# getreu/stringsext

Hardware: AMD Instinct MI355X
Metric: GiB/s scanned (higher is better)
Workload: dtype u8

## Files before the change

stringsext_amd/csrc/sx_api.cpp:

```cpp
#include "sx_ctx.hpp"
#include "sx_print_core.hpp"
#include "sx_select_core.hpp"
#include "sx_selset_build.hpp"
#include "sx_selset_core.hpp"
#include "sx_selre_build.hpp"
#include "sx_selre_core.hpp"
#include "sx_extract_build.hpp"
#include "sx_extract_core.hpp"
#include "sx_seltally_build.hpp"
#include "sx_seltally_core.hpp"
#include "sx_label_build.hpp"
#include "sx_label_core.hpp"

using namespace sx;

struct sx_select_set {
    int device = 0;
    uint8_t* mem = nullptr;
    SelsetDevice dev{};
    sx_select_set_info info{};
};

struct sx_select_regex {
    int device = 0;
    uint8_t* mem = nullptr;
    SelreDevice dev{};
    sx_select_regex_info info{};
};

struct sx_extract_regex {
    int device = 0;
    uint8_t* mem = nullptr;
    ExtractDevice dev{};
    sx_extract_regex_info info{};
};

struct sx_tally_set {
    int device = 0;
    uint8_t* mem = nullptr;
    SeltallyDevice dev{};
    const uint32_t* d_unique_of_pattern = nullptr;
    std::vector<uint32_t> unique_of_pattern;
    sx_tally_set_info info{};
};

struct sx_label_set {
    int device = 0;
    uint8_t* mem = nullptr;
    LabelDevice dev{};
    sx_label_set_info info{};
};

struct sx_labels {
    struct Seg {
        const uint64_t* d = nullptr;
        const void* recs = nullptr;
        uint64_t n = 0;
        std::shared_ptr<std::atomic<uint64_t>> epoch_ref;
        uint64_t epoch = 0;
    };
    int device = 0;
    uint8_t* mem = nullptr;
    std::vector<Seg> segs;
};

namespace sx {
PinnedPool::Block PinnedPool::take(size_t bytes) {
    {
        std::lock_guard<std::mutex> g(mu);
        size_t best = free_blocks.size();
        for (size_t i = 0; i < free_blocks.size(); i++)
            if (free_blocks[i].cap >= bytes && (best == free_blocks.size() || free_blocks[i].cap < free_blocks[best].cap)) best = i;
        if (best < free_blocks.size() && free_blocks[best].cap <= 4 * bytes + (4u << 20)) {
            Block b = free_blocks[best];
            free_blocks.erase(free_blocks.begin() + (long)best);
            return b;
        }
    }
    Block b;
    const size_t cap = bytes + bytes / 8 + (1u << 20);
    if (hipHostMalloc(&b.p, cap, hipHostMallocNonCoherent) != hipSuccess) { b.p = nullptr; return b; }
    b.cap = cap;
    return b;
}
void PinnedPool::give(Block b) {
    if (!b.p) return;
    std::lock_guard<std::mutex> g(mu);
    free_blocks.push_back(b);
    if (free_blocks.size() > 40) {
        size_t m = 0;
        for (size_t i = 1; i < free_blocks.size(); i++) if (free_blocks[i].cap < free_blocks[m].cap) m = i;
        (void)hipHostFree(free_blocks[m].p);
        free_blocks.erase(free_blocks.begin() + (long)m);
    }
}
PinnedPool::~PinnedPool() { for (Block& b : free_blocks) (void)hipHostFree(b.p); }
}

namespace {
std::string g_create_error;
}

namespace sx {

double g_tl_t0 = 0;
int g_tl_on = 0;

double now_ms() {
    using namespace std::chrono;
    return duration<double, std::milli>(steady_clock::now().time_since_epoch()).count();
}


int ensure_pinned(sx_ctx* ctx, uint64_t bytes) {
    if (ctx->h_pin_cap >= bytes) return SX_OK;
    if (ctx->h_pin) HIP_TRY(ctx, hipHostFree(ctx->h_pin));
    ctx->h_pin = nullptr; ctx->h_pin_cap = 0;
    bytes += bytes / 4 + (1u << 20);
    unsigned flags = hipHostMallocNonCoherent;
    if (ctx->sw.pin_flags >= 0) flags = (unsigned)ctx->sw.pin_flags;
    HIP_TRY(ctx, hipHostMalloc((void**)&ctx->h_pin, bytes, flags));
    ctx->h_pin_cap = bytes;
    return SX_OK;
}
int read_back_async(sx_ctx* ctx, hipStream_t s, void* pinned_dst, const void* dev_src, size_t bytes) {
    if (ctx->sw.small_copy && bytes <= (1u << 20) && ((((uintptr_t)pinned_dst | (uintptr_t)dev_src | bytes) & 3) == 0))
        HIP_TRY(ctx, launch_small_copy(pinned_dst, dev_src, bytes, s));
    else HIP_TRY(ctx, hipMemcpyAsync(pinned_dst, dev_src, bytes, hipMemcpyDeviceToHost, s));
    return SX_OK;
}
int read_back_sync(sx_ctx* ctx, MissionDev& d, hipStream_t s, void* host_dst, const void* dev_src, size_t bytes) {
    if (!ctx->sw.small_copy || bytes > kSmallReadBytes || ((((uintptr_t)dev_src | bytes) & 3) != 0)) {
        HIP_TRY(ctx, hipMemcpyAsync(host_dst, dev_src, bytes, hipMemcpyDeviceToHost, s));
        HIP_TRY(ctx, hipStreamSynchronize(s));
        return SX_OK;
    }
    if (!d.h_small) HIP_TRY(ctx, hipHostMalloc((void**)&d.h_small, kSmallReadBytes, hipHostMallocDefault));
    HIP_TRY(ctx, launch_small_copy(d.h_small, dev_src, bytes, s));
    HIP_TRY(ctx, hipStreamSynchronize(s));
    memcpy(host_dst, d.h_small, bytes);
    return SX_OK;
}
int ensure_pinned2(sx_ctx* ctx, uint64_t bytes) {
    if (ctx->h_pin2_cap >= bytes) return SX_OK;
    if (ctx->h_pin2) HIP_TRY(ctx, hipHostFree(ctx->h_pin2));
    ctx->h_pin2 = nullptr; ctx->h_pin2_cap = 0;
    bytes += bytes / 4 + (1u << 20);
    HIP_TRY(ctx, hipHostMalloc((void**)&ctx->h_pin2, bytes, hipHostMallocNonCoherent));
    ctx->h_pin2_cap = bytes;
    return SX_OK;
}
int ensure_scratch(sx_ctx* ctx, uint64_t bytes) {
    std::lock_guard<std::recursive_mutex> g(ctx->grow_mu);
    if (ctx->d_scratch_cap >= bytes) return SX_OK;
    if (ctx->merge_async) { const int rc = merge_drain(ctx); if (rc != SX_OK) return rc; }
    if (ctx->d_scratch) HIP_TRY(ctx, hipFree(ctx->d_scratch));
    ctx->d_scratch = nullptr; ctx->d_scratch_cap = 0;
    bytes += bytes / 4 + (1u << 20);
    HIP_TRY(ctx, hipMalloc((void**)&ctx->d_scratch, bytes));
    ctx->d_scratch_cap = bytes;
    return SX_OK;
}

int ensure_capacity(sx_ctx* ctx, ScanSlot& s, uint32_t cap) {
    if (s.capacity >= cap) return SX_OK;
    if (s.d_recs) HIP_TRY(ctx, hipFree(s.d_recs));
    s.d_recs = nullptr; s.capacity = 0;
    HIP_TRY(ctx, hipMalloc((void**)&s.d_recs, (size_t)cap * sizeof(DevRun)));
    s.capacity = cap;
    return SX_OK;
}

int ensure_cache(sx_ctx* ctx, uint64_t bytes) {
    if (ctx->d_cache_cap >= bytes) return SX_OK;
    if (ctx->d_cache) HIP_TRY(ctx, hipFree(ctx->d_cache));
    ctx->d_cache = nullptr; ctx->d_cache_cap = 0;
    HIP_TRY(ctx, hipMalloc((void**)&ctx->d_cache, bytes));
    ctx->d_cache_cap = bytes;
    return SX_OK;
}
int ensure_rp(sx_ctx* ctx, MissionDev& d, int slot, uint64_t bytes) {
    if (d.d_rp_cap[slot] >= bytes) return SX_OK;
    std::lock_guard<std::recursive_mutex> g(ctx->grow_mu);
    if (ctx->merge_async) { const int rc = merge_drain(ctx); if (rc != SX_OK) return rc; }
    if (d.d_rp[slot]) HIP_TRY(ctx, hipFree(d.d_rp[slot]));
    d.d_rp[slot] = nullptr; d.d_rp_cap[slot] = 0;
    bytes += bytes / 4 + 4096;
    HIP_TRY(ctx, hipMalloc(&d.d_rp[slot], bytes));
    d.d_rp_cap[slot] = bytes;
    return SX_OK;
}


unsigned usable_cpus() {
    unsigned n = std::thread::hardware_concurrency();
    if (n < 1) n = 1;
    if (FILE* f = fopen("/sys/fs/cgroup/cpu.max", "r")) {
        char a[64] = { 0 };
        unsigned long long period = 0;
        if (fscanf(f, "%63s %llu", a, &period) == 2 && strcmp(a, "max") != 0 && period > 0) {
            const unsigned long long quota = strtoull(a, nullptr, 10);
            const unsigned q = (unsigned)((quota + period - 1) / period);
            if (q >= 1 && q < n) n = q;
        }
        fclose(f);
    }
    return n;
}

unsigned replay_threads(const sx_ctx* ctx) {
    unsigned n = ctx->opt.replay_threads ? ctx->opt.replay_threads
                                         : std::min(std::thread::hardware_concurrency(), 4 * usable_cpus());
    if (ctx->sw.replay_threads) n = (unsigned)ctx->sw.replay_threads;
    if (n < 1) n = 1;
    return n > 256 ? 256 : n;
}


void begin_call(sx_ctx* ctx) {
    memset(&ctx->stats, 0, sizeof ctx->stats);
    ctx->err.clear();
    ctx->sharded_call = false;
    ctx->dev_epoch->fetch_add(1);
}

static int fetch_to_host(sx_result* r, MissionFindings& s) {
    if (!s.dev_only) return SX_OK;
    if (!s.keep_on_device || !s.dev_epoch_ref || s.dev_epoch_ref->load() != s.dev_epoch) return SX_E_STATE;
    const size_t bytes = s.ext_nf * s.rec_size() + s.ext_na;
    PinnedPool::Block blk = r->r.pool ? r->r.pool->take(bytes + 64) : PinnedPool::Block{};
    if (!blk.p) return SX_E_NOMEM;
    if (hipMemcpy(blk.p, s.dev_copy, bytes, hipMemcpyDeviceToHost) != hipSuccess) { r->r.pool->give(blk); return SX_E_HIP; }
    s.ext = blk; s.dev_only = false;
    return SX_OK;
}
static int fetch_all_to_host(const sx_result* r) {
    sx_result* w = const_cast<sx_result*>(r);
    for (auto& s : w->r.segs) { const int rc = fetch_to_host(w, s); if (rc != SX_OK) return rc; }
    return SX_OK;
}


}

extern "C" {

int sx_abi_version(void) { return SX_ABI_VERSION; }

const uint16_t* sx_decoder_table(uint32_t encoding, uint64_t* n_words) {
    size_t n = 0;
    const uint16_t* t = decoder_table((int)encoding, &n);
    if (n_words) *n_words = n;
    return t;
}

const uint32_t* sx_wave_pair_codes(const sx_mission* mission, uint32_t* out8192) {
    if (!mission || !out8192) return nullptr;
    Mission m;
    std::string err;
    if (Mission::from_c(*mission, false, Switches{}.wave_same, &m, &err) != SX_OK || m.wave_pairs.size() != 8192) return nullptr;
    memcpy(out8192, m.wave_pairs.data(), 8192 * 4);
    return out8192;
}

const uint32_t* sx_wave_pair_codes2(const sx_mission* mission, uint32_t* out4096) {
    if (!mission || !out4096) return nullptr;
    Mission m;
    std::string err;
    if (Mission::from_c(*mission, false, Switches{}.wave_same, &m, &err) != SX_OK || m.wave_pairs2.size() != 4096) return nullptr;
    memcpy(out4096, m.wave_pairs2.data(), 4096 * 4);
    return out4096;
}

int sx_wave_swar(const sx_mission* mission, uint32_t* out26) {
    if (!mission || !out26) return SX_E_INVALID;
    Mission m;
    std::string err;
    const int rc = Mission::from_c(*mission, false, Switches{}.wave_same, &m, &err);
    if (rc != SX_OK) return rc;
    static_assert(sizeof(WvSwar) == 26 * 4, "sx_wave_swar hands the struct out as 26 words");
    memcpy(out26, &m.wave_swar, sizeof(WvSwar));
    return m.wave_ok && m.wave_swar.cls ? 1 : 0;
}

int sx_scan_classifier(const sx_mission* mission, int generic, uint32_t* out20) {
    if (!mission || !out20) return SX_E_INVALID;
    Mission m;
    std::string err;
    const int rc = Mission::from_c(*mission, generic != 0, Switches{}.wave_same, &m, &err);
    if (rc != SX_OK) return rc;
    const ScanParams& p = m.proto;
    const uint32_t head[7] = { p.a_lo, p.a_hi, p.u_lo, p.u_hi, p.l3_lo, p.l3_hi, p.n_ranges };
    memcpy(out20, head, sizeof head);
    memcpy(out20 + 7, p.rng_c1, 6 * sizeof(uint32_t));
    memcpy(out20 + 13, p.rng_c2, 6 * sizeof(uint32_t));
    out20[19] = 0;
    return (int)m.kind;
}

int sx_wave_classes(const sx_mission* mission, uint8_t* classes) {
    if (!mission || !classes) return SX_E_INVALID;
    Mission m;
    std::string err;
    const int rc = Mission::from_c(*mission, false, Switches{}.wave_same, &m, &err);
    if (rc != SX_OK) return rc;
    if (!m.wave_ok || m.wave_lead_check || (m.wave_lut.size() != 256 && !(m.wave_family == 2 && m.wave_lut.size() == 512))) return 0;
    memcpy(classes, m.wave_lut.data(), m.wave_lut.size());
    return 1 + (int)m.wave_family;
}

int sx_create(sx_ctx** out, const sx_mission* missions, int n_missions, int hip_device, const sx_options* opt) {
    if (!out || !missions || n_missions <= 0 || n_missions > 26) { g_create_error = "bad arguments"; return SX_E_INVALID; }
    sx_ctx* ctx = new sx_ctx();
    ctx->sw = Switches::from_env();
    if (opt) ctx->opt = *opt;
    if (ctx->sw.result_on_device) ctx->opt.flags |= SX_OPT_RESULT_ON_DEVICE;
    ctx->missions.resize((size_t)n_missions);
    ctx->states.resize((size_t)n_missions);
    for (int k = 0; k < n_missions; k++) {
        std::string err;
        int rc = Mission::from_c(missions[k], (ctx->opt.flags & SX_OPT_GENERIC_KERNELS) != 0, ctx->sw.wave_same, &ctx->missions[(size_t)k], &err);
        if (rc != SX_OK) { g_create_error = "mission " + std::to_string(k) + ": " + err; delete ctx; return rc; }
        ctx->states[(size_t)k].reset(ctx->missions[(size_t)k]);
    }
    if (hip_device == SX_HOST_ONLY) { ctx->host_only = true; *out = ctx; return SX_OK; }

    int n_dev = 0;
    hipError_t e = hipGetDeviceCount(&n_dev);
    if (e != hipSuccess || n_dev <= 0 || hip_device < 0 || hip_device >= n_dev) {
        g_create_error = std::string("no usable HIP device (hipGetDeviceCount: ")
                         + (e == hipSuccess ? "ok" : hipGetErrorString(e)) + ", devices=" + std::to_string(n_dev)
                         + ", requested=" + std::to_string(hip_device) + "); the scan only runs on the GPU";
        delete ctx;
        return SX_E_NO_DEVICE;
    }
    ctx->device = hip_device;
    auto fail = [&](const char* what, hipError_t err) {
        g_create_error = std::string(what) + ": " + hipGetErrorString(err);
        sx_destroy(ctx);
        return SX_E_HIP;
    };
    if ((e = hipSetDevice(hip_device)) != hipSuccess) return fail("hipSetDevice", e);
    ctx->dev.resize((size_t)n_missions);
    const uint32_t cap = ctx->opt.record_capacity ? ctx->opt.record_capacity : (1u << 20);
    {
        int cus = 0;
        if (hipDeviceGetAttribute(&cus, hipDeviceAttributeMultiprocessorCount, hip_device) == hipSuccess && cus > 0) ctx->n_cus = (unsigned)cus;
        if (ctx->sw.scan_blocks_per_cu >= 0) ctx->scan_blocks_per_cu = (unsigned)ctx->sw.scan_blocks_per_cu;
        if (ctx->sw.region_cap >= 0) ctx->region_cap = (uint32_t)ctx->sw.region_cap;
        if (ctx->sw.scan_cus) ctx->n_cus = (unsigned)ctx->sw.scan_cus;
    }
    int prio_lo = 0, prio_hi = 0;
    (void)hipDeviceGetStreamPriorityRange(&prio_lo, &prio_hi);
    if (ctx->sw.prio_n >= 0) {
        if (ctx->sw.prio_n >= 1) prio_lo = ctx->sw.prio_scan;
        if (ctx->sw.prio_n >= 2) prio_hi = ctx->sw.prio_post;
        fprintf(stderr, "[sx] stream priorities: scan %d, post %d\n", prio_lo, prio_hi);
    }
    const bool per_mission = (ctx->opt.flags & SX_OPT_MISSION_STREAMS) || ctx->sw.mission_streams;
    if ((e = hipStreamCreateWithPriority(&ctx->post_stream, hipStreamNonBlocking, prio_hi)) != hipSuccess) return fail("hipStreamCreate", e);
    if (!per_mission && (e = hipStreamCreateWithPriority(&ctx->scan_stream, hipStreamNonBlocking, prio_lo)) != hipSuccess)
        return fail("hipStreamCreate", e);
    for (auto& d : ctx->dev) {
        d.stream_b = ctx->post_stream;
        if (per_mission) {
            if ((e = hipStreamCreateWithPriority(&d.stream, hipStreamNonBlocking, prio_lo)) != hipSuccess) return fail("hipStreamCreate", e);
        } else d.stream = ctx->scan_stream;
        for (ScanSlot& s : d.slot) {
            if ((e = hipEventCreate(&s.ev0)) != hipSuccess) return fail("hipEventCreate", e);
            if ((e = hipEventCreate(&s.ev1)) != hipSuccess) return fail("hipEventCreate", e);
            if ((e = hipEventCreateWithFlags(&s.ev_free, hipEventDisableTiming)) != hipSuccess) return fail("hipEventCreate", e);
            if ((e = hipMalloc((void**)&s.d_counters, kCounterWords * sizeof(uint32_t))) != hipSuccess) return fail("hipMalloc", e);
            if ((e = hipMalloc((void**)&s.d_recs, (size_t)cap * sizeof(DevRun))) != hipSuccess) return fail("hipMalloc", e);
            s.capacity = cap;
        }
    }
    for (size_t k = 0; k < ctx->dev.size(); k++) {
        size_t n_words = 0;
        if (const uint16_t* t = decoder_table(ctx->missions[k].c.encoding, &n_words)) {
            if ((e = hipMalloc((void**)&ctx->dev[k].d_table, n_words * 2)) != hipSuccess) return fail("hipMalloc", e);
            if ((e = hipMemcpy(ctx->dev[k].d_table, t, n_words * 2, hipMemcpyHostToDevice)) != hipSuccess) return fail("hipMemcpy", e);
        }
        const std::vector<uint32_t>& pl = ctx->missions[k].pair_lut;
        if (!pl.empty()) {
            if ((e = hipMalloc((void**)&ctx->dev[k].d_pair_lut, pl.size() * 4)) != hipSuccess) return fail("hipMalloc", e);
            if ((e = hipMemcpy(ctx->dev[k].d_pair_lut, pl.data(), pl.size() * 4, hipMemcpyHostToDevice)) != hipSuccess) return fail("hipMemcpy", e);
        }
    }
    *out = ctx;
    return SX_OK;
}

void sx_destroy(sx_ctx* ctx) {
    if (!ctx) return;
    ctx->dev_epoch->fetch_add(1);
    for (auto& e : ctx->select_epoch) e->fetch_add(1);
    if (!ctx->host_only && ctx->device >= 0) {
        (void)hipSetDevice(ctx->device);
        for (auto& d : ctx->dev) {
            if (d.stream) (void)hipStreamSynchronize(d.stream);
            if (d.stream_b) (void)hipStreamSynchronize(d.stream_b);
            for (ScanSlot& s : d.slot) {
                if (s.d_recs) (void)hipFree(s.d_recs);
                if (s.d_cnt) (void)hipFree(s.d_cnt);
                if (s.d_grid) (void)hipFree(s.d_grid);
                if (s.d_packed) (void)hipFree(s.d_packed);
                if (s.d_counters) (void)hipFree(s.d_counters);
                if (s.ev0) (void)hipEventDestroy(s.ev0);
                if (s.ev1) (void)hipEventDestroy(s.ev1);
                if (s.ev_free) (void)hipEventDestroy(s.ev_free);
            }
            if (d.d_table) (void)hipFree(d.d_table);
            if (d.d_pair_lut) (void)hipFree(d.d_pair_lut);
            if (d.d_wave_lut) (void)hipFree(d.d_wave_lut);
            if (d.d_wave_pairs) (void)hipFree(d.d_wave_pairs);
            if (d.d_wave_pairs2) (void)hipFree(d.d_wave_pairs2);
            for (void* q : d.d_rp) if (q) (void)hipFree(q);
            if (d.h_runs) (void)hipHostFree(d.h_runs);
            if (d.ev_runs) (void)hipEventDestroy(d.ev_runs);
            if (d.stream_w) (void)hipStreamDestroy(d.stream_w);
            if (d.h_tot) (void)hipHostFree(d.h_tot);
            if (d.h_small) (void)hipHostFree(d.h_small);
            for (hipEvent_t e : d.wave_ev) if (e) (void)hipEventDestroy(e);
            if (d.stream && d.stream != ctx->scan_stream) (void)hipStreamDestroy(d.stream);
        }
        for (int i = 0; i < 2; i++) {
            if (ctx->ing_pin[i]) (void)hipHostFree(ctx->ing_pin[i]);
            if (ctx->ing_dev[i]) (void)hipFree(ctx->ing_dev[i]);
        }
        if (ctx->copy_stream) (void)hipStreamDestroy(ctx->copy_stream);
        if (ctx->d2h_stream) (void)hipStreamDestroy(ctx->d2h_stream);
        if (ctx->scan_stream) (void)hipStreamDestroy(ctx->scan_stream);
        if (ctx->d_cache) (void)hipFree(ctx->d_cache);
        if (ctx->post_stream) (void)hipStreamDestroy(ctx->post_stream);
        if (ctx->merge_copy_stream) (void)hipStreamDestroy(ctx->merge_copy_stream);
        if (ctx->d_merge) (void)hipFree(ctx->d_merge);
        if (ctx->d_result) (void)hipFree(ctx->d_result);
        if (ctx->d_result_up) (void)hipFree(ctx->d_result_up);
        if (ctx->d_text) (void)hipFree(ctx->d_text);
        if (ctx->d_print_scratch) (void)hipFree(ctx->d_print_scratch);
        if (ctx->d_print_missions) (void)hipFree(ctx->d_print_missions);
        for (uint8_t* p : ctx->d_select) if (p) (void)hipFree(p);
        if (ctx->d_select_scratch) (void)hipFree(ctx->d_select_scratch);
        if (ctx->d_select_scratch2) (void)hipFree(ctx->d_select_scratch2);
        for (hipEvent_t e : ctx->merge_ev) if (e) (void)hipEventDestroy(e);
        for (hipEvent_t e : ctx->slab_ev) if (e) (void)hipEventDestroy(e);
        if (ctx->ev_interleaved) (void)hipEventDestroy(ctx->ev_interleaved);
        if (ctx->d_input) (void)hipFree(ctx->d_input);
        if (ctx->d_scratch) (void)hipFree(ctx->d_scratch);
        if (ctx->h_pin) (void)hipHostFree(ctx->h_pin);
        if (ctx->h_pin2) (void)hipHostFree(ctx->h_pin2);
    }
    delete ctx;
}

const char* sx_last_error(const sx_ctx* ctx) { return ctx ? ctx->err.c_str() : g_create_error.c_str(); }

int sx_reset(sx_ctx* ctx) {
    if (!ctx) return SX_E_INVALID;
    for (size_t k = 0; k < ctx->missions.size(); k++) ctx->states[k].reset(ctx->missions[k]);
    ctx->shard_runs_valid = false;
    return SX_OK;
}


int sx_device_runs(sx_ctx* ctx, int mission_index, const void* device_bytes, uint64_t len, int stream_parity,
                   uint64_t min_chars, sx_run** runs, uint64_t* n_runs) {
    if (!ctx || !runs || !n_runs || mission_index < 0 || (size_t)mission_index >= ctx->missions.size()) return SX_E_INVALID;
    begin_call(ctx);
    ctx->sw.scan_warm = Switches::from_env().scan_warm;
    if (ctx->host_only) { ctx->err = "host-only context: no device scan"; return SX_E_STATE; }
    if ((uintptr_t)device_bytes & 15) { ctx->err = "device_bytes must be 16-byte aligned"; return SX_E_INVALID; }
    if (ctx->missions[(size_t)mission_index].host_sequential()) { ctx->err = "an ISO-2022-JP mission has no stage A (one sequential pass on the host)"; return SX_E_INVALID; }
    HIP_TRY(ctx, hipSetDevice(ctx->device));
    std::vector<RunList> out;
    ctx->shard_runs_valid = false;
    int rc = device_runs(ctx, { mission_index }, (const uint8_t*)device_bytes, len, { (uint32_t)(stream_parity & 1) },
                         { min_chars }, &out);
    if (rc != SX_OK) return rc;
    HIP_TRY(ctx, out[0].wait());
    *n_runs = out[0].size();
    *runs = (sx_run*)malloc(sizeof(sx_run) * (out[0].size() ? out[0].size() : 1));
    if (!*runs) return SX_E_NOMEM;
    memcpy(*runs, out[0].data(), sizeof(sx_run) * out[0].size());
    return SX_OK;
}

int sx_device_runs_multi(sx_ctx* ctx, const int* mission_indices, int n, const void* device_bytes, uint64_t len, int stream_parity,
                         const uint64_t* min_chars, sx_run** runs, uint64_t* n_runs) {
    if (!ctx || !mission_indices || n <= 0 || !min_chars || !runs || !n_runs) return SX_E_INVALID;
    begin_call(ctx);
    if (ctx->host_only) { ctx->err = "host-only context: no device scan"; return SX_E_STATE; }
    if ((uintptr_t)device_bytes & 15) { ctx->err = "device_bytes must be 16-byte aligned"; return SX_E_INVALID; }
    std::vector<int> which; std::vector<uint32_t> par; std::vector<uint64_t> mc;
    for (int i = 0; i < n; i++) {
        const int k = mission_indices[i];
        if (k < 0 || (size_t)k >= ctx->missions.size() || std::find(which.begin(), which.end(), k) != which.end()) { ctx->err = "bad mission index"; return SX_E_INVALID; }
        if (ctx->missions[(size_t)k].host_sequential()) { ctx->err = "an ISO-2022-JP mission has no stage A (one sequential pass on the host)"; return SX_E_INVALID; }
        which.push_back(k); par.push_back((uint32_t)(stream_parity & 1)); mc.push_back(min_chars[i]);
        runs[i] = nullptr; n_runs[i] = 0;
    }
    HIP_TRY(ctx, hipSetDevice(ctx->device));
    std::vector<RunList> out;
    ctx->shard_runs_valid = false;
    int rc = device_runs(ctx, which, (const uint8_t*)device_bytes, len, par, mc, &out);
    if (rc != SX_OK) return rc;
    for (int i = 0; i < n; i++) {
        if (!out[(size_t)i].own.empty()) out[(size_t)i].use_own();
        HIP_TRY(ctx, out[(size_t)i].wait());
        n_runs[i] = out[(size_t)i].size();
        runs[i] = (sx_run*)malloc(sizeof(sx_run) * (n_runs[i] ? n_runs[i] : 1));
        if (!runs[i]) { for (int j = 0; j < i; j++) { free(runs[j]); runs[j] = nullptr; } return SX_E_NOMEM; }
        memcpy(runs[i], out[(size_t)i].data(), sizeof(sx_run) * n_runs[i]);
    }
    return SX_OK;
}

int sx_replay_runs(sx_ctx* ctx, const uint8_t* bytes, uint64_t len, int input_file_id, int is_last_input_buffer,
                   const sx_run* const* runs, const uint64_t* n_runs, sx_result** out) {
    if (!ctx || !out || (!bytes && len) || !runs || !n_runs) return SX_E_INVALID;
    begin_call(ctx);
    std::vector<RunList> r(ctx->missions.size());
    for (size_t k = 0; k < r.size(); k++) r[k].assign(runs[k], runs[k] + n_runs[k]);
    HostBytes view(bytes ? bytes : (const uint8_t*)"");
    ResultHolder res;
    std::vector<uint32_t> entry;
    int rc = set_entry_params(ctx, true, bytes, nullptr, len, 0, &entry);
    if (rc != SX_OK) return rc;
    rc = replay_all(ctx, view, whole_chunk_job(ctx, len, input_file_id, is_last_input_buffer != 0), r, &res.r->r, nullptr);
    if (rc == SX_OK) *out = res.release();
    return rc;
}


int sx_scan_shard_device(sx_ctx* ctx, const void* device_bytes, uint64_t buf_off, uint64_t buf_len, uint64_t own_lo,
                         uint64_t own_hi, const uint64_t* start_at, uint64_t file_stream_off, int input_file_id,
                         int reuse_runs, sx_result** out, uint64_t* end_pos) {
    if (!ctx || (!device_bytes && buf_len)) return SX_E_INVALID;
    begin_call(ctx);
    if (ctx->host_only) { ctx->err = "host-only context: no device scan"; return SX_E_STATE; }
    if ((uintptr_t)device_bytes & 15) { ctx->err = "device_bytes must be 16-byte aligned"; return SX_E_INVALID; }
    HIP_TRY(ctx, hipSetDevice(ctx->device));
    return shard_common(ctx, nullptr, (const uint8_t*)device_bytes, nullptr, nullptr, buf_off, buf_len, own_lo, own_hi, start_at,
                        file_stream_off, input_file_id, reuse_runs, out, end_pos);
}

int sx_scan_shard(sx_ctx* ctx, const uint8_t* bytes, uint64_t buf_off, uint64_t buf_len, uint64_t own_lo, uint64_t own_hi,
                  const uint64_t* start_at, uint64_t file_stream_off, int input_file_id, int reuse_runs, sx_result** out,
                  uint64_t* end_pos) {
    if (!ctx || (!bytes && buf_len)) return SX_E_INVALID;
    begin_call(ctx);
    if (ctx->host_only) { ctx->err = "host-only context: no device scan"; return SX_E_STATE; }
    HIP_TRY(ctx, hipSetDevice(ctx->device));
    if (!(reuse_runs && ctx->shard_runs_valid && ctx->shard_runs_off == buf_off && ctx->shard_runs_len == buf_len && ctx->shard_runs_ptr == (const void*)ctx->d_input)) {
        if (buf_len > ctx->d_input_cap) {
            if (ctx->d_input) HIP_TRY(ctx, hipFree(ctx->d_input));
            ctx->d_input = nullptr; ctx->d_input_cap = 0;
            HIP_TRY(ctx, hipMalloc((void**)&ctx->d_input, buf_len));
            ctx->d_input_cap = buf_len;
        }
        if (buf_len) HIP_TRY(ctx, hipMemcpy(ctx->d_input, bytes, buf_len, hipMemcpyHostToDevice));
    }
    return shard_common(ctx, bytes ? bytes : (const uint8_t*)"", ctx->d_input, nullptr, nullptr, buf_off, buf_len, own_lo, own_hi,
                        start_at, file_stream_off, input_file_id, reuse_runs, out, end_pos);
}

int sx_replay_shard_runs(sx_ctx* ctx, const uint8_t* bytes, uint64_t buf_off, uint64_t buf_len, uint64_t own_lo,
                         uint64_t own_hi, const uint64_t* start_at, uint64_t file_stream_off, int input_file_id,
                         const sx_run* const* runs, const uint64_t* n_runs, sx_result** out, uint64_t* end_pos) {
    if (!ctx || (!bytes && buf_len) || !runs || !n_runs) return SX_E_INVALID;
    begin_call(ctx);
    return shard_common(ctx, bytes ? bytes : (const uint8_t*)"", nullptr, runs, n_runs, buf_off, buf_len, own_lo, own_hi, start_at,
                        file_stream_off, input_file_id, 0, out, end_pos);
}

uint64_t sx_result_count(const sx_result* r) { return r ? r->r.count() : 0; }
uint64_t sx_result_segments(const sx_result* r) { return r ? r->r.segs.size() : 0; }
int sx_result_segment(const sx_result* r, uint64_t i, const sx_finding** findings, uint64_t* n_findings,
                      const uint8_t** arena, uint64_t* arena_len) {
    if (!r || i >= r->r.segs.size()) return SX_E_INVALID;
    { const int rc = fetch_to_host(const_cast<sx_result*>(r), const_cast<sx_result*>(r)->r.segs[(size_t)i]); if (rc != SX_OK) return rc; }
    const MissionFindings& s = r->r.segs[(size_t)i];
    if (findings) *findings = s.data();
    if (n_findings) *n_findings = s.count();
    if (arena) *arena = (const uint8_t*)s.strings();
    if (arena_len) *arena_len = s.strings_len();
    return SX_OK;
}
int sx_result_segment_packed(const sx_result* r, uint64_t i, const void** findings, uint64_t* n_findings, const uint8_t** arena,
                             uint64_t* arena_len, int* packed, sx_segment_info* info) {
    if (!r || i >= r->r.segs.size()) return SX_E_INVALID;
    { const int rc = fetch_to_host(const_cast<sx_result*>(r), const_cast<sx_result*>(r)->r.segs[(size_t)i]); if (rc != SX_OK) return rc; }
    const MissionFindings& s = r->r.segs[(size_t)i];
    if (findings) *findings = s.packed ? (const void*)s.data16() : (const void*)s.data();
    if (n_findings) *n_findings = s.count();
    if (arena) *arena = (const uint8_t*)s.strings();
    if (arena_len) *arena_len = s.strings_len();
    if (packed) *packed = s.packed ? 1 : 0;
    if (info) {
        memset(info, 0, sizeof *info);
        info->packed = s.packed ? 1 : 0;
        info->input_file_id = -1;
        if (s.packed && s.info) {
            info->input_file_id = s.info->file_id; info->slice_base = s.info->slice_base;
            memcpy(info->position0, s.info->pos0, sizeof info->position0);
        }
    }
    return SX_OK;
}
int sx_result_segment_device(const sx_result* r, uint64_t i, const void** d_records, uint64_t* n_findings, const uint8_t** d_arena,
                             uint64_t* arena_len, int* packed, sx_segment_info* info) {
    if (!r || i >= r->r.segs.size()) return SX_E_INVALID;
    const MissionFindings& s = r->r.segs[(size_t)i];
    if (d_records) *d_records = nullptr;
    if (d_arena) *d_arena = nullptr;
    if (n_findings) *n_findings = s.count();
    if (arena_len) *arena_len = s.strings_len();
    if (packed) *packed = s.packed ? 1 : 0;
    if (info) {
        memset(info, 0, sizeof *info);
        info->packed = s.packed ? 1 : 0;
        info->input_file_id = -1;
        if (s.packed && s.info) {
            info->input_file_id = s.info->file_id; info->slice_base = s.info->slice_base;
            memcpy(info->position0, s.info->pos0, sizeof info->position0);
        }
    }
    if (!s.dev_only) return SX_OK;
    if (!s.keep_on_device || !s.dev_epoch_ref || s.dev_epoch_ref->load() != s.dev_epoch) return SX_E_STATE;
    if (d_records) *d_records = s.dev_copy;
    if (d_arena) *d_arena = (const uint8_t*)s.dev_copy + s.ext_nf * s.rec_size();
    return SX_OK;
}
const sx_finding* sx_result_findings(const sx_result* r) {
    if (!r || fetch_all_to_host(r) != SX_OK || !const_cast<sx_result*>(r)->r.flatten(nullptr) || r->r.segs.empty()) return nullptr;
    return r->r.segs[0].data();
}
const uint8_t* sx_result_arena(const sx_result* r, uint64_t* len) {
    if (len) *len = 0;
    if (!r || fetch_all_to_host(r) != SX_OK || !const_cast<sx_result*>(r)->r.flatten(nullptr) || r->r.segs.empty()) return nullptr;
    if (len) *len = r->r.segs[0].strings_len();
    return (const uint8_t*)r->r.segs[0].strings();
}
void sx_result_free(sx_result* r) { delete r; }

int sx_print_findings(const sx_ctx* ctx, const sx_result* r, int n_inputs, int radix, int no_metadata, uint8_t** out,
                      uint64_t* out_len) {
    if (!ctx || !r || !out || !out_len) return SX_E_INVALID;
    if (radix != 0 && radix != 'x' && radix != 'd' && radix != 'o') return SX_E_INVALID;
    { const int rc = fetch_all_to_host(r); if (rc != SX_OK) return rc; }
    std::string s;
    print_findings(ctx->missions, r->r, n_inputs, radix, no_metadata != 0, &s);
    *out = (uint8_t*)malloc(s.size() ? s.size() : 1);
    if (!*out) return SX_E_NOMEM;
    memcpy(*out, s.data(), s.size());
    *out_len = s.size();
    return SX_OK;
}

static int result_on_device(sx_ctx* ctx, const sx_result* r, const char* host_call) {
    const std::string in_host = std::string("the result is in host memory: ") + host_call;
    if (r->r.segs.empty()) { ctx->set_err(in_host); return SX_E_STATE; }
    for (const MissionFindings& s : r->r.segs) {
        if (!s.dev_only || !s.keep_on_device || s.ext_nf == 0) { ctx->set_err(in_host); return SX_E_STATE; }
        const bool ours = s.dev_epoch_ref && (s.dev_epoch_ref == ctx->dev_epoch || s.dev_epoch_ref == ctx->select_epoch[0] || s.dev_epoch_ref == ctx->select_epoch[1]);
        if (!ours || s.dev_epoch_ref->load() != s.dev_epoch) {
            ctx->set_err("a later scan or selection has reused the result's device memory");
            return SX_E_STATE;
        }
    }
    return SX_OK;
}

int sx_print_findings_device(sx_ctx* ctx, const sx_result* r, int n_inputs, int radix, int no_metadata, const uint8_t** d_text,
                             uint64_t* text_len) {
    if (d_text) *d_text = nullptr;
    if (text_len) *text_len = 0;
    if (!ctx || !r || !d_text || !text_len) return SX_E_INVALID;
    if (radix != 0 && radix != 'x' && radix != 'd' && radix != 'o') { ctx->set_err("radix must be 0, 'x', 'd' or 'o'"); return SX_E_INVALID; }
    if (ctx->host_only) { ctx->set_err("host-only context: no device print"); return SX_E_STATE; }
    { const int rc = result_on_device(ctx, r, "sx_print_findings"); if (rc != SX_OK) return rc; }
    HIP_TRY(ctx, hipSetDevice(ctx->device));
    hipStream_t st = ctx->post_stream;
    if (!ctx->d_print_missions) {
        std::vector<PrintMission> tab(256);
        memset(tab.data(), 0, tab.size() * sizeof(PrintMission));
        for (size_t k = ctx->missions.size(); k-- > 0;) {
            const Mission& m = ctx->missions[k];
            const char* name = m.c.print_encoding_as_ascii ? "ascii" : m.encoding_name();
            const std::string label = name ? name : "";
            PrintMission& t = tab[m.c.mission_id];
            if (label.size() > sizeof t.label) { ctx->set_err("encoding label longer than 14 bytes"); return SX_E_STATE; }
            t.present = 1; t.len = (uint8_t)label.size();
            memcpy(t.label, label.data(), label.size());
        }
        uint8_t* p = nullptr;
        if (hipMalloc((void**)&p, tab.size() * sizeof(PrintMission)) != hipSuccess) { (void)hipGetLastError(); ctx->set_err("device print: no memory for the Mission table"); return SX_E_NOMEM; }
        const hipError_t e = hipMemcpy(p, tab.data(), tab.size() * sizeof(PrintMission), hipMemcpyHostToDevice);
        if (e != hipSuccess) { (void)hipFree(p); ctx->set_err(std::string("hipMemcpy: ") + hipGetErrorString(e)); return SX_E_HIP; }
        ctx->d_print_missions = p;
    }
    const size_t ns = r->r.segs.size();
    uint64_t scratch = 0;
    for (const MissionFindings& s : r->r.segs) scratch += print_scratch_bytes(s.ext_nf);
    if (scratch > ctx->d_print_scratch_cap) {
        if (ctx->d_print_scratch) (void)hipFree(ctx->d_print_scratch);
        ctx->d_print_scratch = nullptr; ctx->d_print_scratch_cap = 0;
        if (hipMalloc((void**)&ctx->d_print_scratch, scratch) != hipSuccess) { (void)hipGetLastError(); ctx->d_print_scratch = nullptr; ctx->set_err("device print: no memory for the offsets"); return SX_E_NOMEM; }
        ctx->d_print_scratch_cap = scratch;
    }
    std::vector<PrintParams> P(ns);
    std::vector<const uint64_t*> d_total(ns);
    uint64_t at = 0;
    for (size_t i = 0; i < ns; i++) {
        const MissionFindings& s = r->r.segs[i];
        PrintParams& p = P[i];
        memset(&p, 0, sizeof p);
        p.recs = s.dev_copy; p.arena = (const uint8_t*)s.dev_copy + s.ext_nf * s.rec_size(); p.n = s.ext_nf; p.packed = s.packed ? 1u : 0u;
        p.file_id = s.packed && s.info ? s.info->file_id : -1;
        p.several_inputs = n_inputs > 1; p.radix = (uint32_t)radix; p.no_metadata = no_metadata != 0; p.several_missions = ctx->missions.size() > 1;
        p.missions = (const PrintMission*)ctx->d_print_missions;
        const size_t bytes = print_scratch_bytes(s.ext_nf);
        HIP_TRY(ctx, print_measure(p, ctx->d_print_scratch + at, bytes, st, &p.wbase, &d_total[i]));
        at += bytes;
    }
    HIP_TRY(ctx, hipStreamSynchronize(st));
    uint64_t total = 0;
    for (size_t i = 0; i < ns; i++) {
        uint64_t t = 0;
        HIP_TRY(ctx, hipMemcpy(&t, d_total[i], sizeof t, hipMemcpyDeviceToHost));
        P[i].base = total;
        total += t;
    }
    if (total > ctx->d_text_cap) {
        if (ctx->d_text) (void)hipFree(ctx->d_text);
        ctx->d_text = nullptr; ctx->d_text_cap = 0;
        if (hipMalloc((void**)&ctx->d_text, total) != hipSuccess) {
            (void)hipGetLastError();
            ctx->d_text = nullptr;
            ctx->set_err("device print: no memory for " + std::to_string(total) + " bytes of text");
            return SX_E_NOMEM;
        }
        ctx->d_text_cap = total;
    }
    for (size_t i = 0; i < ns; i++) {
        P[i].text = ctx->d_text;
        HIP_TRY(ctx, print_write(P[i], st));
    }
    HIP_TRY(ctx, hipStreamSynchronize(st));
    *d_text = ctx->d_text;
    *text_len = total;
    return SX_OK;
}

static int grow_device(sx_ctx* ctx, uint8_t** p, uint64_t* cap, uint64_t bytes, const char* what) {
    if (bytes <= *cap) return SX_OK;
    if (*p) (void)hipFree(*p);
    *p = nullptr; *cap = 0;
    if (hipMalloc((void**)p, bytes) != hipSuccess) {
        (void)hipGetLastError();
        *p = nullptr;
        ctx->set_err(std::string("device select: no memory for ") + std::to_string(bytes) + " bytes of " + what);
        return SX_E_NOMEM;
    }
    *cap = bytes;
    return SX_OK;
}

static int select_on_device(sx_ctx* ctx, const sx_result* r, const sx_pattern* patterns, int n_patterns, const SelsetDevice* set, const SelreDevice* re, const ExtractDevice* ex, uint32_t flags, sx_result** out,
                            const sx_labels* labels = nullptr, const uint64_t* masks = nullptr) {
    if (ctx->host_only) { ctx->set_err("host-only context: no device selection"); return SX_E_STATE; }
    { const int rc = result_on_device(ctx, r, "filter on the host"); if (rc != SX_OK) return rc; }
    if (labels) {
        bool same = labels->segs.size() == r->r.segs.size();
        for (size_t i = 0; same && i < labels->segs.size(); i++) {
            const sx_labels::Seg& l = labels->segs[i];
            const MissionFindings& s = r->r.segs[i];
            same = l.recs == s.dev_copy && l.n == s.ext_nf && l.epoch_ref == s.dev_epoch_ref && l.epoch == s.dev_epoch;
        }
        if (!same) { ctx->set_err("the labels were not made from this result"); return SX_E_INVALID; }
    }
    const int slot = (int)(ctx->select_calls & 1u);
    for (const MissionFindings& s : r->r.segs)
        if (s.dev_epoch_ref == ctx->select_epoch[slot]) { ctx->set_err("this selection reuses the source's device memory: it was selected two calls ago"); return SX_E_STATE; }
    HIP_TRY(ctx, hipSetDevice(ctx->device));
    hipStream_t st = ctx->post_stream;
    const size_t ns = r->r.segs.size();
    uint64_t scratch = 0;
    for (const MissionFindings& s : r->r.segs) scratch += ex ? extract_scratch_bytes(s.ext_nf) : select_scratch_bytes(s.ext_nf);
    { const int rc = grow_device(ctx, &ctx->d_select_scratch, &ctx->d_select_scratch_cap, scratch, "wavefront tables"); if (rc != SX_OK) return rc; }
    std::vector<SelectParams> P(ex ? 0 : ns);
    std::vector<ExtractParams> X(ex ? ns : 0);
    std::vector<const uint32_t*> d_count(ns);
    std::vector<const uint64_t*> d_count64(ns), d_bytes(ns);
    uint64_t at = 0;
    for (size_t i = 0; i < ns; i++) {
        const MissionFindings& s = r->r.segs[i];
        if (ex) {
            ExtractParams& x = X[i];
            memset(&x, 0, sizeof x);
            x.recs = s.dev_copy; x.arena = (const uint8_t*)s.dev_copy + s.ext_nf * s.rec_size(); x.n = s.ext_nf; x.packed = s.packed ? 1u : 0u;
            x.ex = *ex;
            const size_t bytes = extract_scratch_bytes(s.ext_nf);
            HIP_TRY(ctx, extract_measure(&x, ctx->d_select_scratch + at, bytes, st, &d_count64[i], &d_bytes[i]));
            at += bytes;
            continue;
        }
        SelectParams& p = P[i];
        memset(&p, 0, sizeof p);
        p.recs = s.dev_copy; p.arena = (const uint8_t*)s.dev_copy + s.ext_nf * s.rec_size(); p.n = s.ext_nf; p.packed = s.packed ? 1u : 0u;
        if (set || re) p.pat.invert = (flags & SX_SELECT_INVERT) ? 1u : 0u;
        else select_fill_patterns(&p.pat, patterns, n_patterns, flags);
        const size_t bytes = select_scratch_bytes(s.ext_nf);
        LabelPick pick{ nullptr, 0, 0, 0 };
        if (labels) pick = LabelPick{ labels->segs[i].d, masks[0], masks[1], masks[2] };
        HIP_TRY(ctx, select_measure(&p, set, re, ctx->d_select_scratch + at, bytes, st, &d_count[i], &d_bytes[i], labels ? &pick : nullptr));
        at += bytes;
    }
    HIP_TRY(ctx, hipStreamSynchronize(st));
    std::vector<uint64_t> n_sel(ns), b_sel(ns), base(ns);
    uint64_t block = 0, scratch2 = 0;
    for (size_t i = 0; i < ns; i++) {
        uint64_t c = 0;
        if (ex) HIP_TRY(ctx, hipMemcpy(&c, d_count64[i], sizeof c, hipMemcpyDeviceToHost));
        else { uint32_t c32 = 0; HIP_TRY(ctx, hipMemcpy(&c32, d_count[i], sizeof c32, hipMemcpyDeviceToHost)); c = c32; }
        HIP_TRY(ctx, hipMemcpy(&b_sel[i], d_bytes[i], sizeof(uint64_t), hipMemcpyDeviceToHost));
        if (c >= 0xFFFFFFFFull) {
            ctx->set_err("segment " + std::to_string(i) + " has " + std::to_string(c) + " matches: more than the 32-bit counters of a segment hold");
            return SX_E_INVALID;
        }
        n_sel[i] = c;
        if (!c) continue;
        base[i] = block;
        block += (c * r->r.segs[i].rec_size() + b_sel[i] + 255) / 256 * 256;
        scratch2 = std::max<uint64_t>(scratch2, ex ? extract_place_scratch_bytes(c) : select_place_scratch_bytes(c));
    }
    ctx->select_epoch[slot]->fetch_add(1);
    ctx->select_calls++;
    ResultHolder res;
    res.r->r.pool = ctx->pool;
    if (block) {
        { const int rc = grow_device(ctx, &ctx->d_select[slot], &ctx->d_select_cap[slot], block, "selected findings"); if (rc != SX_OK) return rc; }
        { const int rc = grow_device(ctx, &ctx->d_select_scratch2, &ctx->d_select_scratch2_cap, scratch2, "string offsets"); if (rc != SX_OK) return rc; }
        for (size_t i = 0; i < ns; i++) {
            if (!n_sel[i]) continue;
            const MissionFindings& s = r->r.segs[i];
            uint8_t* recs = ctx->d_select[slot] + base[i];
            if (ex) HIP_TRY(ctx, extract_place(X[i], recs, n_sel[i], recs + n_sel[i] * s.rec_size(), ctx->d_select_scratch2, extract_place_scratch_bytes(n_sel[i]), st));
            else HIP_TRY(ctx, select_place(P[i], recs, n_sel[i], recs + n_sel[i] * s.rec_size(), ctx->d_select_scratch2, select_place_scratch_bytes(n_sel[i]), st));
            MissionFindings o;
            o.ext_nf = n_sel[i]; o.ext_na = b_sel[i]; o.dev_copy = recs; o.dev_only = true; o.keep_on_device = true;
            o.dev_epoch_ref = ctx->select_epoch[slot]; o.dev_epoch = ctx->select_epoch[slot]->load();
            o.packed = s.packed; o.info = s.info;
            res.r->r.segs.push_back(std::move(o));
        }
        HIP_TRY(ctx, hipStreamSynchronize(st));
    }
    *out = res.release();
    return SX_OK;
}

int sx_result_select_device(sx_ctx* ctx, const sx_result* r, const sx_pattern* patterns, int n_patterns, uint32_t flags, sx_result** out) {
    if (out) *out = nullptr;
    if (!ctx || !r || !patterns || !out) return SX_E_INVALID;
    if (n_patterns < 1 || n_patterns > SX_SELECT_MAX_PATTERNS) { ctx->set_err("n_patterns must be 1..16"); return SX_E_INVALID; }
    if (flags & ~(uint32_t)(SX_SELECT_ASCII_NOCASE | SX_SELECT_INVERT)) { ctx->set_err("unknown selection flags"); return SX_E_INVALID; }
    for (int p = 0; p < n_patterns; p++)
        if (!patterns[p].bytes || patterns[p].len < 1 || patterns[p].len > SX_SELECT_MAX_PATTERN_BYTES) { ctx->set_err("a pattern must have 1..64 bytes"); return SX_E_INVALID; }
    return select_on_device(ctx, r, patterns, n_patterns, nullptr, nullptr, nullptr, flags, out);
}

int sx_select_set_create(sx_ctx* ctx, const sx_pattern* patterns, uint32_t n_patterns, uint32_t flags, sx_select_set** out) {
    if (out) *out = nullptr;
    if (!ctx || !patterns || !out) return SX_E_INVALID;
    SelsetTable T;
    std::string err;
    { const int rc = selset_build(patterns, n_patterns, flags, &T, &err); if (rc != SX_OK) { ctx->set_err("pattern set: " + err); return rc; } }
    if (ctx->host_only) { ctx->set_err("host-only context: no device for the pattern set"); return SX_E_STATE; }
    HIP_TRY(ctx, hipSetDevice(ctx->device));
    const size_t table = (T.next.size() + 15) / 16 * 16;
    uint8_t* mem = nullptr;
    if (hipMalloc((void**)&mem, sizeof T.map + table) != hipSuccess) {
        (void)hipGetLastError();
        ctx->set_err("pattern set: no device memory for " + std::to_string(sizeof T.map + table) + " bytes of table");
        return SX_E_NOMEM;
    }
    hipError_t e = hipMemcpy(mem, T.map, sizeof T.map, hipMemcpyHostToDevice);
    if (e == hipSuccess) e = hipMemcpy(mem + sizeof T.map, T.next.data(), T.next.size(), hipMemcpyHostToDevice);
    if (e != hipSuccess) { (void)hipFree(mem); ctx->set_err(std::string("hipMemcpy: ") + hipGetErrorString(e)); return SX_E_HIP; }
    sx_select_set* set = new (std::nothrow) sx_select_set;
    if (!set) { (void)hipFree(mem); return SX_E_NOMEM; }
    set->device = ctx->device; set->mem = mem;
    set->dev = SelsetDevice{ mem, mem + sizeof T.map, T.states, T.classes, T.lds_states, T.matched, T.entry_bytes, 0 };
    set->info = sx_select_set_info{ T.n_patterns, T.states, T.classes, T.nocase, (uint64_t)T.next.size(), T.lds_states, 0 };
    *out = set;
    return SX_OK;
}

int sx_select_set_info_get(const sx_select_set* set, sx_select_set_info* out) {
    if (!set || !out) return SX_E_INVALID;
    *out = set->info;
    return SX_OK;
}

void sx_select_set_free(sx_select_set* set) {
    if (!set) return;
    (void)hipFree(set->mem);
    delete set;
}

int sx_result_select_set_device(sx_ctx* ctx, const sx_result* r, const sx_select_set* set, uint32_t flags, sx_result** out) {
    if (out) *out = nullptr;
    if (!ctx || !r || !set || !out) return SX_E_INVALID;
    if (flags & ~(uint32_t)SX_SELECT_INVERT) { ctx->set_err("a pattern set is selected with SX_SELECT_INVERT or no flag: the fold is compiled into the set"); return SX_E_INVALID; }
    if (ctx->host_only) { ctx->set_err("host-only context: no device selection"); return SX_E_STATE; }
    if (set->device != ctx->device) { ctx->set_err("the pattern set lies on another device"); return SX_E_INVALID; }
    return select_on_device(ctx, r, nullptr, 0, &set->dev, nullptr, nullptr, flags, out);
}

int sx_select_regex_create(sx_ctx* ctx, const sx_pattern* patterns, uint32_t n_patterns, uint32_t flags, sx_select_regex** out) {
    if (out) *out = nullptr;
    if (!ctx || !patterns || !out) return SX_E_INVALID;
    SelreTable T;
    std::string err;
    { const int rc = selre_build(patterns, n_patterns, flags, &T, &err); if (rc != SX_OK) { ctx->set_err("regex set: " + err); return rc; } }
    if (ctx->host_only) { ctx->set_err("host-only context: no device for the regex set"); return SX_E_STATE; }
    HIP_TRY(ctx, hipSetDevice(ctx->device));
    const size_t bytes = T.next.size() * sizeof(uint16_t), table = (bytes + 15) / 16 * 16;
    uint8_t* mem = nullptr;
    if (hipMalloc((void**)&mem, sizeof T.map + table) != hipSuccess) {
        (void)hipGetLastError();
        ctx->set_err("regex set: no device memory for " + std::to_string(sizeof T.map + table) + " bytes of table");
        return SX_E_NOMEM;
    }
    hipError_t e = hipMemcpy(mem, T.map, sizeof T.map, hipMemcpyHostToDevice);
    if (e == hipSuccess) e = hipMemcpy(mem + sizeof T.map, T.next.data(), bytes, hipMemcpyHostToDevice);
    if (e != hipSuccess) { (void)hipFree(mem); ctx->set_err(std::string("hipMemcpy: ") + hipGetErrorString(e)); return SX_E_HIP; }
    sx_select_regex* re = new (std::nothrow) sx_select_regex;
    if (!re) { (void)hipFree(mem); return SX_E_NOMEM; }
    re->device = ctx->device; re->mem = mem;
    re->dev = SelreDevice{ mem, (const uint16_t*)(mem + sizeof T.map), T.states, T.classes, T.lds_states, T.end_first, T.stop_first, T.matched, T.root_end, 0 };
    re->info = sx_select_regex_info{ T.n_patterns, T.states, T.classes, T.nocase, (uint64_t)bytes, T.lds_states, T.end_states };
    *out = re;
    return SX_OK;
}

int sx_select_regex_info_get(const sx_select_regex* re, sx_select_regex_info* out) {
    if (!re || !out) return SX_E_INVALID;
    *out = re->info;
    return SX_OK;
}

void sx_select_regex_free(sx_select_regex* re) {
    if (!re) return;
    (void)hipFree(re->mem);
    delete re;
}

int sx_result_select_regex_device(sx_ctx* ctx, const sx_result* r, const sx_select_regex* re, uint32_t flags, sx_result** out) {
    if (out) *out = nullptr;
    if (!ctx || !r || !re || !out) return SX_E_INVALID;
    if (flags & ~(uint32_t)SX_SELECT_INVERT) { ctx->set_err("a regex set is selected with SX_SELECT_INVERT or no flag: the fold is compiled into the set"); return SX_E_INVALID; }
    if (ctx->host_only) { ctx->set_err("host-only context: no device selection"); return SX_E_STATE; }
    if (re->device != ctx->device) { ctx->set_err("the regex set lies on another device"); return SX_E_INVALID; }
    return select_on_device(ctx, r, nullptr, 0, nullptr, &re->dev, nullptr, flags, out);
}

int sx_extract_regex_create(sx_ctx* ctx, const sx_pattern* patterns, uint32_t n_patterns, uint32_t flags, sx_extract_regex** out) {
    if (out) *out = nullptr;
    if (!ctx || !patterns || !out) return SX_E_INVALID;
    ExtractTable T;
    std::string err;
    { const int rc = extract_build(patterns, n_patterns, flags, &T, &err); if (rc != SX_OK) { ctx->set_err("extract set: " + err); return rc; } }
    if (ctx->host_only) { ctx->set_err("host-only context: no device for the extract set"); return SX_E_STATE; }
    HIP_TRY(ctx, hipSetDevice(ctx->device));
    const size_t bytes = T.next.size() * sizeof(uint16_t), table = (bytes + 15) / 16 * 16;
    uint8_t* mem = nullptr;
    if (hipMalloc((void**)&mem, sizeof T.map + table) != hipSuccess) {
        (void)hipGetLastError();
        ctx->set_err("extract set: no device memory for " + std::to_string(sizeof T.map + table) + " bytes of table");
        return SX_E_NOMEM;
    }
    hipError_t e = hipMemcpy(mem, T.map, sizeof T.map, hipMemcpyHostToDevice);
    if (e == hipSuccess) e = hipMemcpy(mem + sizeof T.map, T.next.data(), bytes, hipMemcpyHostToDevice);
    if (e != hipSuccess) { (void)hipFree(mem); ctx->set_err(std::string("hipMemcpy: ") + hipGetErrorString(e)); return SX_E_HIP; }
    sx_extract_regex* ex = new (std::nothrow) sx_extract_regex;
    if (!ex) { (void)hipFree(mem); return SX_E_NOMEM; }
    ex->device = ctx->device; ex->mem = mem;
    ex->dev = ExtractDevice{ mem, (const uint16_t*)(mem + sizeof T.map), T.states, T.classes, T.lds_states, T.end_first, T.here_first, T.dead_first, T.start0, T.start1 };
    ex->info = sx_extract_regex_info{ T.n_patterns, T.states, T.classes, T.nocase, (uint64_t)bytes, T.lds_states, 0 };
    *out = ex;
    return SX_OK;
}

int sx_extract_regex_info_get(const sx_extract_regex* ex, sx_extract_regex_info* out) {
    if (!ex || !out) return SX_E_INVALID;
    *out = ex->info;
    return SX_OK;
}

void sx_extract_regex_free(sx_extract_regex* ex) {
    if (!ex) return;
    (void)hipFree(ex->mem);
    delete ex;
}

int sx_result_extract_regex_device(sx_ctx* ctx, const sx_result* r, const sx_extract_regex* ex, uint32_t flags, sx_result** out) {
    if (out) *out = nullptr;
    if (!ctx || !r || !ex || !out) return SX_E_INVALID;
    if (flags) { ctx->set_err("an extraction takes no flag: the fold is compiled into the set"); return SX_E_INVALID; }
    if (ctx->host_only) { ctx->set_err("host-only context: no device extraction"); return SX_E_STATE; }
    if (ex->device != ctx->device) { ctx->set_err("the extract set lies on another device"); return SX_E_INVALID; }
    return select_on_device(ctx, r, nullptr, 0, nullptr, nullptr, &ex->dev, flags, out);
}

int sx_tally_set_reset(sx_tally_set* set) {
    if (!set) return SX_E_INVALID;
    if (hipSetDevice(set->device) != hipSuccess) { (void)hipGetLastError(); return SX_E_HIP; }
    hipError_t e = hipMemset(set->dev.hits, 0, (size_t)set->dev.unique * sizeof(uint64_t));
    if (e == hipSuccess) e = hipMemset(set->dev.first, 0xFF, (size_t)set->dev.unique * sizeof(uint64_t));
    if (e == hipSuccess) e = hipStreamSynchronize(nullptr);
    if (e != hipSuccess) { (void)hipGetLastError(); return SX_E_HIP; }
    return SX_OK;
}

int sx_tally_set_create(sx_ctx* ctx, const sx_pattern* patterns, uint32_t n_patterns, uint32_t flags, sx_tally_set** out) {
    if (out) *out = nullptr;
    if (!ctx || !patterns || !out) return SX_E_INVALID;
    SeltallyTable T;
    std::string err;
    { const int rc = seltally_build(patterns, n_patterns, flags, &T, &err); if (rc != SX_OK) { ctx->set_err("tally set: " + err); return rc; } }
    if (ctx->host_only) { ctx->set_err("host-only context: no device for the tally set"); return SX_E_STATE; }
    HIP_TRY(ctx, hipSetDevice(ctx->device));
    const size_t table = (T.next.size() + 15) / 16 * 16;
    const size_t per_state = (size_t)T.states * sizeof(uint32_t), map_words = (((size_t)T.n_patterns + 1) & ~(size_t)1) * sizeof(uint32_t);
    const size_t counters = (size_t)T.unique * sizeof(uint64_t);
    const size_t at_own = sizeof T.map + table, at_dict = at_own + per_state, at_map = at_dict + per_state;
    const size_t at_hits = (at_map + map_words + 7) / 8 * 8, bytes = at_hits + 2 * counters;
    uint8_t* mem = nullptr;
    if (hipMalloc((void**)&mem, bytes) != hipSuccess) {
        (void)hipGetLastError();
        ctx->set_err("tally set: no device memory for " + std::to_string(bytes) + " bytes of tables and counters");
        return SX_E_NOMEM;
    }
    hipError_t e = hipMemcpy(mem, T.map, sizeof T.map, hipMemcpyHostToDevice);
    if (e == hipSuccess) e = hipMemcpy(mem + sizeof T.map, T.next.data(), T.next.size(), hipMemcpyHostToDevice);
    if (e == hipSuccess) e = hipMemcpy(mem + at_own, T.own.data(), per_state, hipMemcpyHostToDevice);
    if (e == hipSuccess) e = hipMemcpy(mem + at_dict, T.dict.data(), per_state, hipMemcpyHostToDevice);
    if (e == hipSuccess) e = hipMemcpy(mem + at_map, T.unique_of_pattern.data(), (size_t)T.n_patterns * sizeof(uint32_t), hipMemcpyHostToDevice);
    if (e != hipSuccess) { (void)hipFree(mem); ctx->set_err(std::string("hipMemcpy: ") + hipGetErrorString(e)); return SX_E_HIP; }
    sx_tally_set* set = new (std::nothrow) sx_tally_set;
    if (!set) { (void)hipFree(mem); return SX_E_NOMEM; }
    set->device = ctx->device; set->mem = mem;
    set->dev = SeltallyDevice{ mem, mem + sizeof T.map, (const uint32_t*)(mem + at_own), (const uint32_t*)(mem + at_dict),
                               (uint64_t*)(mem + at_hits), (uint64_t*)(mem + at_hits + counters),
                               T.states, T.classes, T.lds_states, T.entry_bytes, T.unique, T.unique < kSeltallyLdsIds ? T.unique : kSeltallyLdsIds };
    set->d_unique_of_pattern = (const uint32_t*)(mem + at_map);
    set->info = sx_tally_set_info{ T.n_patterns, T.unique, T.states, T.classes, T.nocase, T.entry_bytes,
                                   (uint64_t)(sizeof T.map + T.next.size() + 2 * per_state + (size_t)T.n_patterns * sizeof(uint32_t)), T.lds_states, 0 };
    set->unique_of_pattern = std::move(T.unique_of_pattern);
    if (sx_tally_set_reset(set) != SX_OK) { ctx->set_err("tally set: the counters could not be reset"); sx_tally_set_free(set); return SX_E_HIP; }
    *out = set;
    return SX_OK;
}

int sx_tally_set_info_get(const sx_tally_set* set, sx_tally_set_info* out) {
    if (!set || !out) return SX_E_INVALID;
    *out = set->info;
    return SX_OK;
}

void sx_tally_set_free(sx_tally_set* set) {
    if (!set) return;
    (void)hipFree(set->mem);
    delete set;
}

int sx_result_tally_device(sx_ctx* ctx, const sx_result* r, sx_tally_set* set, uint64_t ordinal_base, uint64_t* n_findings) {
    if (n_findings) *n_findings = 0;
    if (!ctx || !r || !set) return SX_E_INVALID;
    if (ctx->host_only) { ctx->set_err("host-only context: no device tally"); return SX_E_STATE; }
    if (set->device != ctx->device) { ctx->set_err("the tally set lies on another device"); return SX_E_INVALID; }
    { const int rc = result_on_device(ctx, r, "count on the host"); if (rc != SX_OK) return rc; }
    HIP_TRY(ctx, hipSetDevice(ctx->device));
    hipStream_t st = ctx->post_stream;
    uint64_t walked = 0;
    for (const MissionFindings& s : r->r.segs) {
        SeltallyParams p;
        memset(&p, 0, sizeof p);
        p.recs = s.dev_copy; p.arena = (const uint8_t*)s.dev_copy + s.ext_nf * s.rec_size(); p.n = s.ext_nf; p.packed = s.packed ? 1u : 0u;
        p.ordinal = ordinal_base + walked;
        p.set = set->dev;
        HIP_TRY(ctx, seltally_launch(p, st));
        walked += s.ext_nf;
    }
    HIP_TRY(ctx, hipStreamSynchronize(st));
    if (n_findings) *n_findings = walked;
    return SX_OK;
}

int sx_tally_set_read(const sx_tally_set* set, uint64_t* hits, uint64_t* first, uint32_t n_patterns) {
    if (!set || n_patterns != set->info.n_patterns) return SX_E_INVALID;
    if (hipSetDevice(set->device) != hipSuccess) { (void)hipGetLastError(); return SX_E_HIP; }
    std::vector<uint64_t> u(set->dev.unique);
    for (int k = 0; k < 2; k++) {
        uint64_t* out = k ? first : hits;
        if (!out) continue;
        if (hipMemcpy(u.data(), k ? set->dev.first : set->dev.hits, u.size() * sizeof(uint64_t), hipMemcpyDeviceToHost) != hipSuccess) { (void)hipGetLastError(); return SX_E_HIP; }
        for (uint32_t p = 0; p < n_patterns; p++) out[p] = u[set->unique_of_pattern[p]];
    }
    return SX_OK;
}

int sx_tally_set_counters_device(const sx_tally_set* set, const uint64_t** d_hits, const uint64_t** d_first,
                                 const uint32_t** d_unique_of_pattern, uint32_t* unique) {
    if (!set) return SX_E_INVALID;
    if (d_hits) *d_hits = set->dev.hits;
    if (d_first) *d_first = set->dev.first;
    if (d_unique_of_pattern) *d_unique_of_pattern = set->d_unique_of_pattern;
    if (unique) *unique = set->dev.unique;
    return SX_OK;
}

int sx_label_set_reset(sx_label_set* set) {
    if (!set) return SX_E_INVALID;
    if (hipSetDevice(set->device) != hipSuccess) { (void)hipGetLastError(); return SX_E_HIP; }
    hipError_t e = hipMemset(set->dev.findings, 0, kLabelBits * sizeof(uint64_t));
    if (e == hipSuccess) e = hipMemset(set->dev.first, 0xFF, kLabelBits * sizeof(uint64_t));
    if (e == hipSuccess) e = hipStreamSynchronize(nullptr);
    if (e != hipSuccess) { (void)hipGetLastError(); return SX_E_HIP; }
    return SX_OK;
}

int sx_label_set_create(sx_ctx* ctx, const sx_pattern* patterns, uint32_t n_patterns, uint32_t flags, sx_label_set** out) {
    if (out) *out = nullptr;
    if (!ctx || !patterns || !out) return SX_E_INVALID;
    LabelTable T;
    std::string err;
    { const int rc = label_build(patterns, n_patterns, flags, &T, &err); if (rc != SX_OK) { ctx->set_err("label set: " + err); return rc; } }
    if (ctx->host_only) { ctx->set_err("host-only context: no device for the label set"); return SX_E_STATE; }
    HIP_TRY(ctx, hipSetDevice(ctx->device));
    const size_t next_bytes = T.next.size() * sizeof(uint16_t), table = (next_bytes + 15) / 16 * 16;
    const size_t here_bytes = T.here.size() * sizeof(uint64_t), end_bytes = T.end.size() * sizeof(uint64_t), counters = kLabelBits * sizeof(uint64_t);
    const size_t at_here = sizeof T.map + table, at_end = at_here + here_bytes, at_findings = at_end + end_bytes, bytes = at_findings + 2 * counters;
    uint8_t* mem = nullptr;
    if (hipMalloc((void**)&mem, bytes) != hipSuccess) {
        (void)hipGetLastError();
        ctx->set_err("label set: no device memory for " + std::to_string(bytes) + " bytes of tables and counters");
        return SX_E_NOMEM;
    }
    hipError_t e = hipMemcpy(mem, T.map, sizeof T.map, hipMemcpyHostToDevice);
    if (e == hipSuccess) e = hipMemcpy(mem + sizeof T.map, T.next.data(), next_bytes, hipMemcpyHostToDevice);
    if (e == hipSuccess && here_bytes) e = hipMemcpy(mem + at_here, T.here.data(), here_bytes, hipMemcpyHostToDevice);
    if (e == hipSuccess) e = hipMemcpy(mem + at_end, T.end.data(), end_bytes, hipMemcpyHostToDevice);
    if (e != hipSuccess) { (void)hipFree(mem); ctx->set_err(std::string("hipMemcpy: ") + hipGetErrorString(e)); return SX_E_HIP; }
    sx_label_set* set = new (std::nothrow) sx_label_set;
    if (!set) { (void)hipFree(mem); return SX_E_NOMEM; }
    set->device = ctx->device; set->mem = mem;
    set->dev = LabelDevice{ mem, (const uint16_t*)(mem + sizeof T.map), (const uint64_t*)(mem + at_here), (const uint64_t*)(mem + at_end),
                            (uint64_t*)(mem + at_findings), (uint64_t*)(mem + at_findings + counters), T.root_here, T.all,
                            T.states, T.classes, T.lds_states, T.here_first, T.dead, T.n_patterns };
    set->info = sx_label_set_info{ T.n_patterns, T.states, T.classes, T.nocase, (uint64_t)(sizeof T.map + next_bytes + here_bytes + end_bytes), T.lds_states, (uint32_t)T.here.size() };
    if (sx_label_set_reset(set) != SX_OK) { ctx->set_err("label set: the counters could not be reset"); sx_label_set_free(set); return SX_E_HIP; }
    *out = set;
    return SX_OK;
}

int sx_label_set_info_get(const sx_label_set* set, sx_label_set_info* out) {
    if (!set || !out) return SX_E_INVALID;
    *out = set->info;
    return SX_OK;
}

void sx_label_set_free(sx_label_set* set) {
    if (!set) return;
    (void)hipFree(set->mem);
    delete set;
}

int sx_label_set_read(const sx_label_set* set, uint64_t* findings, uint64_t* first, uint32_t n_patterns) {
    if (!set || n_patterns != set->info.n_patterns) return SX_E_INVALID;
    if (hipSetDevice(set->device) != hipSuccess) { (void)hipGetLastError(); return SX_E_HIP; }
    for (int k = 0; k < 2; k++) {
        uint64_t* out = k ? first : findings;
        if (!out) continue;
        if (hipMemcpy(out, k ? set->dev.first : set->dev.findings, (size_t)n_patterns * sizeof(uint64_t), hipMemcpyDeviceToHost) != hipSuccess) { (void)hipGetLastError(); return SX_E_HIP; }
    }
    return SX_OK;
}

int sx_label_set_counters_device(const sx_label_set* set, const uint64_t** d_findings, const uint64_t** d_first) {
    if (!set) return SX_E_INVALID;
    if (d_findings) *d_findings = set->dev.findings;
    if (d_first) *d_first = set->dev.first;
    return SX_OK;
}

int sx_result_label_device(sx_ctx* ctx, const sx_result* r, sx_label_set* set, uint64_t ordinal_base, sx_labels** out) {
    if (out) *out = nullptr;
    if (!ctx || !r || !set || !out) return SX_E_INVALID;
    if (ctx->host_only) { ctx->set_err("host-only context: no device labels"); return SX_E_STATE; }
    if (set->device != ctx->device) { ctx->set_err("the label set lies on another device"); return SX_E_INVALID; }
    { const int rc = result_on_device(ctx, r, "label on the host"); if (rc != SX_OK) return rc; }
    HIP_TRY(ctx, hipSetDevice(ctx->device));
    hipStream_t st = ctx->post_stream;
    sx_labels* lab = new (std::nothrow) sx_labels;
    if (!lab) return SX_E_NOMEM;
    lab->device = ctx->device;
    uint64_t bytes = 0;
    for (const MissionFindings& s : r->r.segs) bytes += ((uint64_t)s.ext_nf * sizeof(uint64_t) + 255) / 256 * 256;
    if (hipMalloc((void**)&lab->mem, bytes ? bytes : 256) != hipSuccess) {
        (void)hipGetLastError();
        delete lab;
        ctx->set_err("device labels: no memory for " + std::to_string(bytes) + " bytes of labels");
        return SX_E_NOMEM;
    }
    uint64_t walked = 0, at = 0;
    hipError_t e = hipSuccess;
    for (const MissionFindings& s : r->r.segs) {
        sx_labels::Seg seg;
        seg.d = (const uint64_t*)(lab->mem + at); seg.recs = s.dev_copy; seg.n = s.ext_nf; seg.epoch_ref = s.dev_epoch_ref; seg.epoch = s.dev_epoch;
        lab->segs.push_back(seg);
        LabelParams p;
        memset(&p, 0, sizeof p);
        p.recs = s.dev_copy; p.arena = (const uint8_t*)s.dev_copy + s.ext_nf * s.rec_size(); p.n = s.ext_nf; p.packed = s.packed ? 1u : 0u;
        p.ordinal = ordinal_base + walked;
        p.labels = (uint64_t*)(lab->mem + at);
        p.set = set->dev;
        e = label_launch(p, st);
        if (e != hipSuccess) break;
        walked += s.ext_nf;
        at += ((uint64_t)s.ext_nf * sizeof(uint64_t) + 255) / 256 * 256;
    }
    const hipError_t e2 = hipStreamSynchronize(st);
    if (e == hipSuccess) e = e2;
    if (e != hipSuccess) {
        sx_labels_free(lab);
        ctx->set_err(std::string("device labels: ") + hipGetErrorString(e));
        return SX_E_HIP;
    }
    *out = lab;
    return SX_OK;
}

uint64_t sx_labels_segments(const sx_labels* labels) { return labels ? labels->segs.size() : 0; }

int sx_labels_segment_device(const sx_labels* labels, uint64_t segment, const uint64_t** d_labels, uint64_t* n_findings) {
    if (d_labels) *d_labels = nullptr;
    if (n_findings) *n_findings = 0;
    if (!labels || segment >= labels->segs.size()) return SX_E_INVALID;
    if (d_labels) *d_labels = labels->segs[segment].d;
    if (n_findings) *n_findings = labels->segs[segment].n;
    return SX_OK;
}

void sx_labels_free(sx_labels* labels) {
    if (!labels) return;
    (void)hipFree(labels->mem);
    delete labels;
}

int sx_result_select_labels_device(sx_ctx* ctx, const sx_result* r, const sx_labels* labels, uint64_t any, uint64_t all, uint64_t none, sx_result** out) {
    if (out) *out = nullptr;
    if (!ctx || !r || !labels || !out) return SX_E_INVALID;
    if (ctx->host_only) { ctx->set_err("host-only context: no device selection"); return SX_E_STATE; }
    if (labels->device != ctx->device) { ctx->set_err("the labels lie on another device"); return SX_E_INVALID; }
    const uint64_t masks[3] = { any, all, none };
    return select_on_device(ctx, r, nullptr, 0, nullptr, nullptr, nullptr, 0, out, labels, masks);
}

int sx_get_stats(const sx_ctx* ctx, sx_stats* out) {
    if (!ctx || !out) return SX_E_INVALID;
    *out = ctx->stats;
    return SX_OK;
}

void sx_free(void* p) { free(p); }

int sx_fill_background_device(sx_ctx* ctx, void* device_bytes, uint64_t first_byte_index, uint64_t len, uint64_t seed) {
    if (!ctx || ctx->host_only) return SX_E_STATE;
    HIP_TRY(ctx, hipSetDevice(ctx->device));
    HIP_TRY(ctx, launch_fill_background((uint8_t*)device_bytes, first_byte_index, len, seed, ctx->dev[0].stream_b));
    HIP_TRY(ctx, hipStreamSynchronize(ctx->dev[0].stream_b));
    return SX_OK;
}

int sx_device_alloc(sx_ctx* ctx, uint64_t bytes, void** device_ptr) {
    if (!ctx || ctx->host_only || !device_ptr) return SX_E_STATE;
    HIP_TRY(ctx, hipSetDevice(ctx->device));
    HIP_TRY(ctx, hipMalloc(device_ptr, bytes ? bytes : 1));
    return SX_OK;
}
int sx_device_free(sx_ctx* ctx, void* device_ptr) {
    if (!ctx || ctx->host_only) return SX_E_STATE;
    HIP_TRY(ctx, hipFree(device_ptr));
    return SX_OK;
}
int sx_device_upload(sx_ctx* ctx, void* device_dst, const void* host_src, uint64_t bytes) {
    if (!ctx || ctx->host_only) return SX_E_STATE;
    HIP_TRY(ctx, hipSetDevice(ctx->device));
    HIP_TRY(ctx, hipMemcpy(device_dst, host_src, bytes, hipMemcpyHostToDevice));
    return SX_OK;
}
int sx_device_download(sx_ctx* ctx, void* host_dst, const void* device_src, uint64_t bytes) {
    if (!ctx || ctx->host_only) return SX_E_STATE;
    HIP_TRY(ctx, hipSetDevice(ctx->device));
    HIP_TRY(ctx, hipMemcpy(host_dst, device_src, bytes, hipMemcpyDeviceToHost));
    return SX_OK;
}

int sx_device_read_bandwidth(sx_ctx* ctx, const void* device_bytes, uint64_t len, int repeats, double* gbytes_per_s) {
    if (!ctx || ctx->host_only || !gbytes_per_s || repeats == 0) return SX_E_STATE;
    HIP_TRY(ctx, hipSetDevice(ctx->device));
    MissionDev& d = ctx->dev[0];
    uint64_t* d_out = nullptr;
    HIP_TRY(ctx, hipMalloc((void**)&d_out, 8));
    HIP_TRY(ctx, hipMemsetAsync(d_out, 0, 8, d.stream));
    const uint32_t sub = repeats < 0 ? (ctx->opt.subchunk_bytes ? ctx->opt.subchunk_bytes : 256u * 1024u) : 0u;
    if (repeats < 0) repeats = -repeats;
    HIP_TRY(ctx, launch_read_sum((const uint8_t*)device_bytes, len, d_out, d.stream, sub, ctx->sw.probe_rot));
    float best = 1e30f;
    for (int i = 0; i < repeats; i++) {
        HIP_TRY(ctx, hipEventRecord(d.slot[0].ev0, d.stream));
        HIP_TRY(ctx, launch_read_sum((const uint8_t*)device_bytes, len, d_out, d.stream, sub, ctx->sw.probe_rot));
        HIP_TRY(ctx, hipEventRecord(d.slot[0].ev1, d.stream));
        HIP_TRY(ctx, hipStreamSynchronize(d.stream));
        float ms = 0;
        HIP_TRY(ctx, hipEventElapsedTime(&ms, d.slot[0].ev0, d.slot[0].ev1));
        if (ms < best) best = ms;
    }
    (void)hipFree(d_out);
    *gbytes_per_s = (double)(len / 16 * 16) / (best * 1e-3) / 1e9;
    return SX_OK;
}

}
```

stringsext_amd/csrc/sx_ctx.hpp:

```cpp
#pragma once
#include <hip/hip_runtime_api.h>
#include <stdio.h>
#include <stdlib.h>
#include <string.h>
#include <errno.h>
#include <fcntl.h>
#include <sys/mman.h>
#include <sys/stat.h>
#include <unistd.h>

#include <algorithm>
#include <atomic>
#include <chrono>
#include <condition_variable>
#include <deque>
#include <functional>
#include <mutex>
#include <string>
#include <thread>
#include <unordered_map>
#include <vector>

#include "sx_host.hpp"
#include "sx_switches.hpp"

namespace sx {

double now_ms();
constexpr size_t kSmallReadBytes = 4096;
extern double g_tl_t0;
extern int g_tl_on;
#define SX_TL(...) do { if (sx::g_tl_on) { fprintf(stderr, "[tl %+8.3f] ", sx::now_ms() - sx::g_tl_t0); fprintf(stderr, __VA_ARGS__); fputc('\n', stderr); } } while (0)

struct RunList {
    std::vector<sx_run> own;
    const sx_run* p = nullptr;
    size_t n = 0;
    bool on_device = false;
    bool skipped = false;
    const sx_run* dev_ptr = nullptr;
    const void* dev_src = nullptr; size_t copy_bytes = 0;
    hipStream_t copy_stream = nullptr; hipEvent_t ready = nullptr;
    mutable bool issued = false;
    hipError_t start_copy() const {
        if (!dev_src || issued || !copy_bytes) return hipSuccess;
        hipError_t e = hipMemcpyAsync(const_cast<sx_run*>(p), dev_src, copy_bytes, hipMemcpyDeviceToHost, copy_stream);
        if (e == hipSuccess) e = hipEventRecord(ready, copy_stream);
        issued = true;
        return e;
    }
    mutable bool complete = false, edges_done = false;
    bool full() const { return !dev_src || !copy_bytes || complete; }
    hipError_t fetch_edges(size_t edge) const {
        if (full() || issued) return wait();
        if (n <= 2 * edge) return wait();
        if (edges_done) return hipSuccess;
        edges_done = true;
        hipError_t e = hipMemcpyAsync(const_cast<sx_run*>(p), dev_src, edge * sizeof(sx_run), hipMemcpyDeviceToHost, copy_stream);
        if (e == hipSuccess)
            e = hipMemcpyAsync(const_cast<sx_run*>(p) + (n - edge), (const sx_run*)dev_src + (n - edge), edge * sizeof(sx_run),
                               hipMemcpyDeviceToHost, copy_stream);
        if (e == hipSuccess) e = hipStreamSynchronize(copy_stream);
        return e;
    }
    hipError_t wait() const {
        hipError_t e = start_copy();
        if (e == hipSuccess && dev_src && copy_bytes) e = hipEventSynchronize(ready);
        if (e == hipSuccess) complete = true;
        return e;
    }
    void use_own() { p = own.data(); n = own.size(); on_device = false; dev_src = nullptr; copy_bytes = 0; complete = true; }
    void assign(const sx_run* b, const sx_run* e) { own.assign(b, e); use_own(); }
    const sx_run* data() const { return p; }
    size_t size() const { return n; }
    const sx_run& operator[](size_t i) const { return p[i]; }
};

struct ScanSlot {
    DevRun* d_recs = nullptr;
    uint32_t capacity = 0;
    uint32_t* d_counters = nullptr;
    hipEvent_t ev0 = nullptr, ev1 = nullptr;
    hipEvent_t ev_free = nullptr;
    bool free_pending = false;
    uint32_t* d_cnt = nullptr;  uint64_t cnt_cap = 0;
    uint32_t* d_grid = nullptr; uint64_t grid_cap = 0;
    DevRun* d_packed = nullptr; uint64_t packed_cap = 0;
    uint32_t region_cap = 0;
    uint64_t n_regions = 0;
    bool fused = false, fused_first = false;
};
struct MissionDev {
    hipStream_t stream = nullptr;
    hipStream_t stream_b = nullptr;
    ScanSlot slot[2];
    uint16_t* d_table = nullptr;
    uint32_t* d_pair_lut = nullptr;
    uint32_t* d_wave_pairs = nullptr;
    uint32_t* d_wave_pairs2 = nullptr;
    uint8_t* d_wave_lut = nullptr;
    sx_run* h_runs = nullptr; uint64_t h_runs_cap = 0;
    hipEvent_t ev_runs = nullptr;
    void* d_rp[12] = { nullptr, nullptr, nullptr, nullptr, nullptr, nullptr, nullptr, nullptr, nullptr, nullptr, nullptr, nullptr };
    uint64_t d_rp_cap[12] = { 0, 0, 0, 0, 0, 0, 0, 0, 0, 0, 0, 0 };
    hipStream_t stream_w = nullptr;
    uint64_t* h_tot = nullptr;
    const uint32_t* grid_of_scan = nullptr; uint32_t grid_sub = 0; const uint8_t* grid_data = nullptr; uint64_t grid_len = 0;
    uint8_t* h_small = nullptr;
    std::vector<hipEvent_t> wave_ev;
    uint64_t last_out_runs = 0, last_out_bytes = 0;
};


}

struct sx_result {
    sx::Result r;
};

struct sx_ctx {
    std::shared_ptr<sx::PinnedPool> pool = std::make_shared<sx::PinnedPool>();
    std::shared_ptr<std::atomic<uint64_t>> dev_epoch = std::make_shared<std::atomic<uint64_t>>(0);
    std::vector<sx::Mission> missions;
    std::vector<sx::ScannerState> states;
    std::vector<sx::MissionDev> dev;
    bool host_only = false;
    bool sharded_call = false, single_piece = true;
    int device = -1;
    sx_options opt{};
    sx::Switches sw;
    std::string err;
    sx_stats stats{};
    hipStream_t scan_stream = nullptr, post_stream = nullptr;
    uint8_t* d_cache = nullptr;
    uint64_t d_cache_cap = 0;
    hipStream_t merge_copy_stream = nullptr;
    hipEvent_t merge_ev[3] = { nullptr, nullptr, nullptr };
    hipEvent_t slab_ev[3] = { nullptr, nullptr, nullptr };
    std::atomic<bool> slab_copy_pending{ false };
    uint8_t* d_merge = nullptr; uint64_t d_merge_cap = 0, merge_out_room = 0, merge_n_out = 0;
    uint8_t* d_result = nullptr; uint64_t d_result_cap = 0;
    uint8_t* d_result_up = nullptr; uint64_t d_result_up_cap = 0;
    uint8_t* d_text = nullptr; uint64_t d_text_cap = 0;
    uint8_t* d_print_scratch = nullptr; uint64_t d_print_scratch_cap = 0;
    uint8_t* d_print_missions = nullptr;
    uint8_t* d_select[2] = { nullptr, nullptr }; uint64_t d_select_cap[2] = { 0, 0 };
    std::shared_ptr<std::atomic<uint64_t>> select_epoch[2] = { std::make_shared<std::atomic<uint64_t>>(0), std::make_shared<std::atomic<uint64_t>>(0) };
    uint64_t select_calls = 0;
    uint8_t* d_select_scratch = nullptr; uint64_t d_select_scratch_cap = 0;
    uint8_t* d_select_scratch2 = nullptr; uint64_t d_select_scratch2_cap = 0;
    bool merge_async = false;
    bool merge_copy_pending[2] = { false, false };
    uint64_t merge_parts = 0;
    uint64_t merged_out_bytes = 0;
    double out_density = 0;
    hipEvent_t ev_interleaved = nullptr;
    std::atomic<bool> interleave_pending{ false };
    std::mutex mu;
    std::mutex err_mu;
    std::recursive_mutex grow_mu;
    void set_err(std::string text) { std::lock_guard<std::mutex> g(err_mu); err = std::move(text); }
    unsigned n_cus = 256, scan_blocks_per_cu = 8;
    hipStream_t copy_stream = nullptr;
    hipStream_t d2h_stream = nullptr;
    uint8_t* ing_pin[2] = { nullptr, nullptr };
    uint8_t* ing_dev[2] = { nullptr, nullptr };
    uint64_t ing_cap = 0, ing_dev_cap = 0;
    uint32_t region_cap = 64;
    std::vector<uint32_t> dense;
    uint8_t* d_input = nullptr;
    uint64_t d_input_cap = 0;
    uint64_t ondemand_fetches = 0;
    std::vector<uint64_t> last_runs;
    std::vector<char> wave_pred;
    std::vector<double> wave_density;
    std::vector<char> wave_off;
    std::vector<sx::RunList> shard_runs;
    bool shard_runs_valid = false;
    uint64_t shard_runs_off = 0, shard_runs_len = 0;
    const void* shard_runs_ptr = nullptr;
    uint8_t* h_pin = nullptr;   uint64_t h_pin_cap = 0;
    uint8_t* h_pin2 = nullptr;  uint64_t h_pin2_cap = 0;
    uint8_t* d_scratch = nullptr; uint64_t d_scratch_cap = 0;
};

#define HIP_TRY(ctx, expr)                                                                     \
    do {                                                                                       \
        hipError_t e_ = (expr);                                                                \
        if (e_ != hipSuccess) {                                                                \
            (ctx)->set_err(std::string(#expr) + ": " + hipGetErrorString(e_));                 \
            return SX_E_HIP;                                                                   \
        }                                                                                      \
    } while (0)

namespace sx {

class SparseDeviceBytes : public ByteView {
public:
    SparseDeviceBytes(sx_ctx* ctx, const uint8_t* d_base, uint64_t len = 0) : ctx_(ctx), d_base_(d_base), len_(len) {}
    void add(uint64_t lo, uint64_t hi, const uint8_t* p) { segs_.push_back({ lo, hi, p }); }
    void add_copy(uint64_t lo, uint64_t hi, const uint8_t* p) {
        owned_.emplace_back(p, p + (hi - lo));
        segs_.push_back({ lo, hi, owned_.back().data() });
    }
    bool empty() const { return segs_.empty(); }
    const uint8_t* span(uint64_t off, size_t n, size_t* hint) override {
        size_t a = *hint < segs_.size() ? *hint : 0;
        if (!(a < segs_.size() && segs_[a].lo <= off)) a = 0;
        size_t steps = 0;
        while (a < segs_.size() && segs_[a].hi <= off && steps < 8) { a++; steps++; }
        if (!(a < segs_.size() && segs_[a].lo <= off && off < segs_[a].hi)) {
            size_t lo = 0, hi = segs_.size();
            while (lo < hi) {
                size_t mid = (lo + hi) / 2;
                if (segs_[mid].hi <= off) lo = mid + 1; else hi = mid;
            }
            a = lo;
        }
        if (a < segs_.size() && segs_[a].lo <= off && off + n <= segs_[a].hi) { *hint = a; return segs_[a].p + (off - segs_[a].lo); }
        std::lock_guard<std::mutex> g(mu_);
        if (len_) {
            const uint64_t b = off / kBlock;
            if (off + n <= std::min<uint64_t>(len_, (b + 1) * kBlock)) {
                auto it = blocks_.find(b);
                if (it == blocks_.end()) {
                    const uint64_t lo = b * kBlock, hi = std::min<uint64_t>(len_, lo + kBlock);
                    std::vector<uint8_t> v((size_t)(hi - lo));
                    if (hipMemcpy(v.data(), d_base_ + lo, (size_t)(hi - lo), hipMemcpyDeviceToHost) != hipSuccess) memset(v.data(), 0, v.size());
                    ctx_->ondemand_fetches++;
                    it = blocks_.emplace(b, std::move(v)).first;
                }
                return it->second.data() + (off - b * kBlock);
            }
        }
        extra_.emplace_back(n);
        if (hipMemcpy(extra_.back().data(), d_base_ + off, n, hipMemcpyDeviceToHost) != hipSuccess)
            memset(extra_.back().data(), 0, n);
        ctx_->ondemand_fetches++;
        return extra_.back().data();
    }

private:
    struct Seg { uint64_t lo, hi; const uint8_t* p; };
    sx_ctx* ctx_;
    const uint8_t* d_base_;
    uint64_t len_ = 0;
    static constexpr uint64_t kBlock = 65536;
    std::unordered_map<uint64_t, std::vector<uint8_t>> blocks_;
    std::vector<Seg> segs_;
    std::deque<std::vector<uint8_t>> extra_, owned_;
    std::mutex mu_;
};

int ensure_pinned(sx_ctx* ctx, uint64_t bytes);
int ensure_pinned2(sx_ctx* ctx, uint64_t bytes);
int read_back_sync(sx_ctx* ctx, sx::MissionDev& d, hipStream_t s, void* host_dst, const void* dev_src, size_t bytes);
int read_back_async(sx_ctx* ctx, hipStream_t s, void* pinned_dst, const void* dev_src, size_t bytes);
int ensure_scratch(sx_ctx* ctx, uint64_t bytes);
int ensure_capacity(sx_ctx* ctx, ScanSlot& s, uint32_t cap);
int ensure_rp(sx_ctx* ctx, MissionDev& d, int slot, uint64_t bytes);
int ensure_cache(sx_ctx* ctx, uint64_t bytes);
unsigned usable_cpus();
unsigned replay_threads(const sx_ctx* ctx);
void begin_call(sx_ctx* ctx);

ScanParams scan_params(const sx_ctx* ctx, int mission, const ScanSlot& s, const uint8_t* d_bytes, uint64_t len,
                       uint32_t parity, uint64_t min_chars);
int stage_a_launch(sx_ctx* ctx, const std::vector<int>& which, const uint8_t* d_bytes, uint64_t len,
                   const std::vector<uint32_t>& parity, const std::vector<uint64_t>& min_chars, int si);
struct ReplayJob;
int ensure_copy_stream(sx_ctx* ctx);
bool result_stays_on_device(const sx_ctx* ctx, const ReplayJob& job);
int merge_drain(sx_ctx* ctx);
int slab_copy_drain(sx_ctx* ctx);
int stage_a_finish(sx_ctx* ctx, const std::vector<int>& which, const uint8_t* d_bytes, uint64_t len,
                   const std::vector<uint32_t>& parity, const std::vector<uint64_t>& min_chars, int si,
                   std::vector<RunList>* out, bool cut_into_pieces = false, const ReplayJob* wave_job = nullptr);
int device_runs(sx_ctx* ctx, const std::vector<int>& which, const uint8_t* d_bytes, uint64_t len,
                const std::vector<uint32_t>& parity, const std::vector<uint64_t>& min_chars,
                std::vector<RunList>* out);

struct ReplayJob {
    uint64_t len = 0;
    int file_id = -1;
    bool is_last = false;
    std::vector<uint64_t> lo;
    uint64_t hi = 0;
    std::vector<char> entry_exact;
    std::vector<uint64_t> consumed0, stream0;
    bool commit_state = true;
    uint32_t slice_base = 0;
    const uint8_t* d_bytes = nullptr;
};




struct PreReplayed {
    std::vector<char> done;
    std::vector<MissionFindings> per;
    std::vector<uint64_t> ends;
    explicit PreReplayed(size_t nm) : done(nm, 0), per(nm), ends(nm, 0) {}
};


constexpr int SX_WAVE_FALLBACK = 1001;
constexpr int SX_NEED_RUNS = 1002;
bool wave_replay_wanted(const sx_ctx* ctx, const ReplayJob& job, size_t k, size_t n_runs, uint64_t heavy_tiles = 0);
int wave_replay_mission(sx_ctx* ctx, size_t k, ByteView& view, const ReplayJob& job, MissionFindings* out, uint64_t* end_pos,
                        uint64_t defer_min_bytes, bool own_stream = false);
bool device_replay_wanted(const sx_ctx* ctx, const ReplayJob& job, size_t k, size_t n_runs);
int device_replay_mission(sx_ctx* ctx, size_t k, ByteView& view, const ReplayJob& job, const RunList& runs,
                          MissionFindings* out, uint64_t* end_pos, uint64_t defer_min_bytes);
int replay_all(sx_ctx* ctx, ByteView& bytes, const ReplayJob& job, const std::vector<RunList>& runs,
               Result* into, uint64_t* end_pos, PreReplayed* pre = nullptr);
ReplayJob whole_chunk_job(sx_ctx* ctx, uint64_t len, int file_id, bool is_last);
int download_for_replay(sx_ctx* ctx, const uint8_t* d_bytes, uint64_t len,
                        const std::vector<RunList>* runs_opt, SparseDeviceBytes* view,
                        const ReplayJob& job, const std::vector<char>* skip = nullptr,
                        bool* used_base = nullptr);

struct ResultHolder {
    sx_result* r = new sx_result();
    ~ResultHolder() { delete r; }
    sx_result* release() { sx_result* x = r; r = nullptr; return x; }
};

int set_entry_params(sx_ctx* ctx, bool carried_state_is_entry, const uint8_t* host_bytes, const uint8_t* d_bytes, uint64_t len,
                     uint64_t stream_off, std::vector<uint32_t>* parity);
int scan_common(sx_ctx* ctx, const uint8_t* host_bytes, const uint8_t* d_bytes, uint64_t len, int file_id,
                int is_last, sx_result** out, uint32_t slice_base0 = 0, sx_result* append_to = nullptr);
int shard_common(sx_ctx* ctx, const uint8_t* host_bytes, const uint8_t* d_bytes,
                 const sx_run* const* given_runs, const uint64_t* given_n, uint64_t buf_off, uint64_t buf_len,
                 uint64_t own_lo, uint64_t own_hi, const uint64_t* start_at, uint64_t file_stream_off, int file_id,
                 int reuse_runs, sx_result** out, uint64_t* end_pos);
int stream_core(sx_ctx* ctx, sx_read_fn read, void* read_user, uint64_t chunk_bytes, int input_file_id,
                sx_result_fn sink, void* sink_user, sx_result* accumulate, int is_last_at_eof,
                const uint8_t* direct = nullptr, uint64_t direct_len = 0);

}
```

stringsext_amd/csrc/sx_replay_core.hpp:

```cpp
#pragma once
#include <stdint.h>

#include "sx_device.hpp"
#include "sx_codec_core.hpp"

namespace sx {


constexpr u32 kSliceLen = 4096;

SXD u64 win_start(u64 p, u32 W) { const u64 s = p / kSliceLen * kSliceLen; return s + (p - s) / W * W; }
SXD u64 next_win_start(u64 p, u32 W) {
    const u64 s = p / kSliceLen * kSliceLen;
    const u64 e = s + (p - s) / W * W + W;
    return e < s + kSliceLen ? e : s + kSliceLen;
}

SXD bool regions_may_touch(const ReplayParams& P) { return P.grep_char < 0; }
SXD bool run_is_chained(const ReplayParams& P, u64 i, u64 want) {
    if (i == 0) return false;
    return regions_may_touch(P) ? want < P.runs[i - 1].end : want <= next_win_start(P.runs[i - 1].end - 1, P.W);
}

struct NearBytes {
    const u8* p = nullptr;
    u64 lo = 0, hi = 0;
};
struct ByteReader {
    const u8* far;
    NearBytes nr;
    SXD u8 operator[](u64 pos) const { return pos - nr.lo < nr.hi - nr.lo ? nr.p[pos - nr.lo] : far[pos]; }
    SXD const u8* span(u64 pos, u64 n) const { return (pos >= nr.lo && pos + n <= nr.hi) ? nr.p + (pos - nr.lo) : far + pos; }
};

template <int ENC>
SXD u64 call_start_before(const ReplayParams& P, u64 p, u64 rs, NearBytes nr = NearBytes{}) {
    const ByteReader bytes{ P.data, nr };
    u64 b = rs;
    if (ENC == 1) {
        while (b > p) {
            const u8 x = bytes[b - 1];
            if (x < 0x80) { b--; continue; }
            if (x >= 0xC0) break;
            u32 k = 1;
            u64 j = b - 1;
            bool found = false;
            while (j > p && k <= 3) {
                j--;
                const u8 y = bytes[j];
                if ((y & 0xC0) == 0x80) { k++; continue; }
                found = true;
                break;
            }
            if (!found) break;
            const u8 lead = bytes[j];
            u32 need = 0;
            u8 lo = 0x80, hi = 0xBF;
            if (lead >= 0xC2 && lead <= 0xDF) need = 1;
            else if (lead >= 0xE0 && lead <= 0xEF) { need = 2; if (lead == 0xE0) lo = 0xA0; if (lead == 0xED) hi = 0x9F; }
            else if (lead >= 0xF0 && lead <= 0xF4) { need = 3; if (lead == 0xF0) lo = 0x90; if (lead == 0xF4) hi = 0x8F; }
            if (need != k) break;
            const u8 second = bytes[j + 1];
            if (second < lo || second > hi) break;
            b = j;
        }
        return b;
    }
    if (ENC == 2 || ENC == 3) {
        constexpr bool be = ENC == 3;
        if ((rs - p) & 1) return p;
        while (b >= p + 2) {
            const u32 u = be ? ((u32)bytes[b - 2] << 8) | bytes[b - 1] : ((u32)bytes[b - 1] << 8) | bytes[b - 2];
            if ((u & 0xF800) != 0xD800) { b -= 2; continue; }
            if ((u & 0xFC00) == 0xDC00) {
                if (b >= p + 4) {
                    const u32 h = be ? ((u32)bytes[b - 4] << 8) | bytes[b - 3] : ((u32)bytes[b - 3] << 8) | bytes[b - 4];
                    if ((h & 0xFC00) == 0xD800) { b -= 4; continue; }
                }
                break;
            }
            b -= 2;
            break;
        }
        return b;
    }
    if (ENC == 4 || ENC == 5) {
        DDecoder dd;
        ddec_reset(dd, (int)P.encoding, P.table);
        u8 sink[48];
        u64 at = p, vs = p;
        while (at < rs) {
            const u32 n = (u32)(rs - at < 12 ? rs - at : 12);
            const DStep r = ddecode<ENC>(dd, P.data + at, n, sink, sizeof sink, false);
            at += r.read;
            if (r.result == RES_MALFORMED && dd.rq_n == 0) vs = at;
        }
        return vs;
    }
    if (!P.table) return p;
    while (b > p) {
        const u8 x = bytes[b - 1];
        if (x >= 0x80 && P.table[x - 0x80] == 0) break;
        b--;
    }
    return b;
}

constexpr u64 kPieceCont = 1ull << 63;

SXD bool mission_splittable(const ReplayParams& P) {
    return P.grep_char < 0 && !P.same_block && P.chars_min_nb >= 1 && P.chars_min_nb <= P.q;
}
SXD u64 win_starts_below(u64 x, u32 W) { const u64 wps = (kSliceLen + W - 1) / W; return x / kSliceLen * wps + (x % kSliceLen + W - 1) / W; }
SXD u64 win_start_no(u64 idx, u32 W) { const u64 wps = (kSliceLen + W - 1) / W; return idx / wps * kSliceLen + idx % wps * W; }

template <int ENC>
SXD bool valid_char_before(const ReplayParams& P, u64 rs) {
    const u8* bytes = P.data;
    if (rs == 0) return false;
    const u8 x = bytes[rs - 1];
    if (ENC == 1) {
        if (x < 0x80) return true;
        if (x >= 0xC0) return false;
        u32 k = 1;
        u64 j = rs - 1;
        bool found = false;
        while (j > 0 && k <= 3) {
            j--;
            if ((bytes[j] & 0xC0) == 0x80) { k++; continue; }
            found = true;
            break;
        }
        if (!found) return false;
        const u8 lead = bytes[j];
        u32 need = 0;
        u8 lo = 0x80, hi = 0xBF;
        if (lead >= 0xC2 && lead <= 0xDF) need = 1;
        else if (lead >= 0xE0 && lead <= 0xEF) { need = 2; if (lead == 0xE0) lo = 0xA0; if (lead == 0xED) hi = 0x9F; }
        else if (lead >= 0xF0 && lead <= 0xF4) { need = 3; if (lead == 0xF0) lo = 0x90; if (lead == 0xF4) hi = 0x8F; }
        if (need != k) return false;
        const u8 second = bytes[j + 1];
        return second >= lo && second <= hi;
    }
    if (ENC == 2 || ENC == 3) {
        constexpr bool be = ENC == 3;
        if (rs < 2) return false;
        const u32 u = be ? ((u32)bytes[rs - 2] << 8) | bytes[rs - 1] : ((u32)bytes[rs - 1] << 8) | bytes[rs - 2];
        if ((u & 0xF800) != 0xD800) return true;
        if ((u & 0xFC00) != 0xDC00 || rs < 4) return false;
        const u32 h = be ? ((u32)bytes[rs - 4] << 8) | bytes[rs - 3] : ((u32)bytes[rs - 3] << 8) | bytes[rs - 4];
        return (h & 0xFC00) == 0xD800;
    }
    if (ENC == 4 || ENC == 5) return x < 0x80;
    return x < 0x80 || !P.table || P.table[x - 0x80] != 0;
}

template <int ENC>
SXD u32 char_len_at(const ReplayParams& P, u64 rs) {
    const u8* b = P.data + rs;
    if (ENC == 1) return b[0] < 0x80 ? 1u : b[0] < 0xE0 ? 2u : b[0] < 0xF0 ? 3u : 4u;
    if (ENC == 2) return (b[1] & 0xFC) == 0xD8 ? 4u : 2u;
    if (ENC == 3) return (b[0] & 0xFC) == 0xD8 ? 4u : 2u;
    if (ENC == 4 || ENC == 5) return dbcs_token_len<(ENC == 4 || ENC == 5) ? ENC : 4>(b, P.len - rs, (int)P.encoding);
    return 1;
}

constexpr u64 kGbVerifyMax = 2048;
SXD bool gb_run_is_exact(const ReplayParams& P, u64 rs, u64 re) {
    if (rs == 0 || re - rs > kGbVerifyMax) return false;
    const u8 x = P.data[rs - 1];
    if (x >= 0x80 || gb_digit(x)) return false;
    DDecoder d;
    ddec_reset(d, (int)P.encoding, P.table);
    u8 sink[48];
    u64 at = rs;
    while (at < re) {
        const u32 n = (u32)(re - at < 12 ? re - at : 12);
        const DStep r = ddec_gb18030(d, P.data + at, n, sink, sizeof sink, false);
        if (r.result != RES_INPUT_EMPTY) return false;
        for (u32 w = 0; w < r.written;) {
            const u8 lead = sink[w];
            if (!pass_lead(P, lead)) return false;
            w += lead < 0x80 ? 1 : lead < 0xE0 ? 2 : lead < 0xF0 ? 3 : 4;
        }
        at += r.read;
    }
    return d.dlead == 0 && d.gb2 == 0 && d.rq_n == 0;
}

template <int ENC>
SXD u64 split_count(const ReplayParams& P, u64 i) {
    if (!mission_splittable(P)) return 1;
    const u64 rs = P.runs[i].start, re = P.runs[i].end;
    const u64 inside = win_starts_below(re, P.W) - win_starts_below(rs + 1, P.W);
    if (inside == 0) return 1;
    const u64 fe = rs + char_len_at<ENC>(P, rs) - 1;
    if (fe >= re || win_start(fe, P.W) >= rs) return 1;
    if (ENC == 4 && enc_is_gb((int)P.encoding)) return gb_run_is_exact(P, rs, re) ? inside + 1 : 1;
    return valid_char_before<ENC>(P, rs) ? inside + 1 : 1;
}
SXD sx_run split_piece(const ReplayParams& P, u64 i, u64 k, u64 count) {
    const sx_run r = P.runs[i];
    if (count <= 1) return r;
    const u64 first = win_starts_below(r.start + 1, P.W);
    sx_run o;
    o.start = k == 0 ? r.start : win_start_no(first + k - 1, P.W);
    o.end = k + 1 == count ? r.end : win_start_no(first + k, P.W);
    o.chars = k == 0 ? r.chars : (kPieceCont | (o.start - r.start));
    return o;
}
template <int ENC> SXD bool run_is_piece(const sx_run& r) { return (r.chars & kPieceCont) != 0; }

template <int ENC>
SXD u32 derive_in_run(u32 q, u32 encoding, const uint16_t* table, const u8* from, u32 delta, DDecoder& dec, u8* ob, u32 ob_cap,
                      bool* cut_pending) {
    ddec_reset(dec, (int)encoding, table);
    u32 w = 0, k = 0;
    while (k < delta) {
        const DStep r = ddecode<ENC>(dec, from + k, delta - k, ob + w, ob_cap - w, false);
        k += r.read; w += r.written;
        if (r.result != RES_MALFORMED) break;
    }
    u32 chars = 0;
    for (u32 t = 0; t < w; t++) chars += (ob[t] & 0xC0) != 0x80;
    *cut_pending = chars >= q;
    return chars >= q ? 0u : w;
}

template <int ENC>
SXD u64 dbcs_sync_before(const u8* bytes, u64 len, u64 at, u64 floor, u32 skip0, u64 lim, int enc, const u32* grid = nullptr, u32 grid_sub = 0) {
    if (grid && grid_sub) {
        const u64 sub = lim / grid_sub, s0 = sub * grid_sub;
        if (s0 > floor) { const u32 v = grid[sub]; if (v & 1u) { floor = s0; skip0 = (v >> 1) & 3u; } }
    }
    u64 r = lim;
    while (r >= floor + 4) {
        u32 x;
        __builtin_memcpy(&x, bytes + r - 4, 4);
        if (!dbcs_may_be_pending_after<ENC>((u8)(x >> 24), enc)) break;
        if (!dbcs_may_be_pending_after<ENC>((u8)(x >> 16), enc)) { r -= 1; break; }
        if (!dbcs_may_be_pending_after<ENC>((u8)(x >> 8), enc)) { r -= 2; break; }
        if (!dbcs_may_be_pending_after<ENC>((u8)x, enc)) { r -= 3; break; }
        r -= 4;
    }
    while (r > floor && dbcs_may_be_pending_after<ENC>(bytes[r - 1], enc)) r--;
    if (r == floor) r += skip0;
    while (r < lim) r += dbcs_token_len<ENC>(bytes + r, len - r, enc);
    return r < at ? r : at;
}

template <int ENC>
SXD_NOINLINE u32 derive_at(const ReplayParams& P, u64 at, u64 floor, DDecoder& dec, u8* ob, NearBytes nr = NearBytes{}) {
    const u8* bytes = P.data;
    const ByteReader rd{ P.data, nr };
    ddec_reset(dec, (int)P.encoding, P.table);
    const u64 back = P.same_block ? 4ull * P.long_run + 8 : 8;
    u64 p = at >= back ? at - back : 0;
    if ((ENC == 2 || ENC == 3) && ((P.stream0 + p) & 1)) p = p ? p - 1 : p + 1;
    if (p < floor) p = floor;
    if (p > at) p = at;
    if (ENC == 4 || ENC == 5) p = dbcs_sync_before<ENC>(bytes, P.len, at, floor, floor == 0 ? P.entry_skip : 0u, p, (int)P.encoding, P.grid_flags, P.grid_sub);
    u8 sink[40], last[4], mb[4];
    u32 last_len = 0, mb_len = 0;
    while (p < at) {
        const u32 n = (u32)(at - p < 12 ? at - p : 12);
        const u8* src = rd.span(p, n);
        u32 k = 0;
        for (;;) {
            const DStep r = ddecode<ENC>(dec, src + k, n - k, sink, sizeof sink, false);
            k += r.read;
            for (u32 w = 0; w < r.written;) {
                const u8 lead = sink[w];
                const u32 cl = lead < 0x80 ? 1 : lead < 0xE0 ? 2 : lead < 0xF0 ? 3 : 4;
                if (pass_lead(P, lead)) {
                    for (u32 t = 0; t < cl; t++) last[t] = sink[w + t];
                    last_len = cl;
                    if (cl > 1) { for (u32 t = 0; t < cl; t++) mb[t] = sink[w + t]; mb_len = cl; }
                } else { last_len = 0; mb_len = 0; }
                w += cl;
            }
            if (r.result == RES_INPUT_EMPTY) break;
            if (r.result == RES_MALFORMED) { last_len = 0; mb_len = 0; }
        }
        p += n;
    }
    u32 out = 0;
    if (last_len) {
        if (P.same_block && mb_len && last_len == 1) { for (u32 t = 0; t < mb_len; t++) ob[out++] = mb[t]; }
        for (u32 t = 0; t < last_len; t++) ob[out++] = last[t];
    }
    return out;
}

constexpr u32 kObCap = 4 * 64 + 3 * 128 + 16;
constexpr u32 kMaxWindow = 128;
constexpr u32 kObCapBig = 4 * 255 + 3 * 510 + 16, kMaxWindowBig = 512;
constexpr u32 kBackBytes = 16;

SXD void stage_window(const u8* src, u32 n, u8* win) {
    u32 k = 0;
    if (((uintptr_t)src & 15) == 0) {
        for (; k + 16 <= n; k += 16) *(uint4*)(win + k) = *(const uint4*)(src + k);
    } else if (((uintptr_t)src & 3) == 0) {
        for (; k + 4 <= n; k += 4) *(u32*)(win + k) = *(const u32*)(src + k);
    }
    for (; k < n; k++) win[k] = src[k];
}

SXD void stage_window_words(const u8* src, u32 n, u8* win) {
    u32 k = 0;
    if (((uintptr_t)src & 15) == 0) {
        for (; k + 16 <= n; k += 16) {
            const uint4 v = *(const uint4*)(src + k);
            u32* w = (u32*)(win + k);
            w[0] = v.x; w[1] = v.y; w[2] = v.z; w[3] = v.w;
        }
    } else if (((uintptr_t)src & 3) == 0) {
        for (; k + 4 <= n; k += 4) *(u32*)(win + k) = *(const u32*)(src + k);
    }
    for (; k < n; k++) win[k] = src[k];
}

struct CacheGeom { u32 slot_bytes, cap_f, cap_b; };
SXD CacheGeom cache_geom(u64 arena_bytes, u64 n_heads) {
    u64 sb = n_heads ? arena_bytes / n_heads : 4096;
    if (sb > 4096) sb = 4096;
    if (sb < 160) sb = 160;
    sb &= ~15ull;
    CacheGeom g;
    g.slot_bytes = (u32)sb;
    g.cap_f = (u32)(sb / 96);
    if (g.cap_f < 2) g.cap_f = 2;
    g.cap_b = g.slot_bytes - g.cap_f * (u32)sizeof(sx_finding);
    return g;
}
template <int MODE, int ENC, bool EXT_WIN = false, bool QBIG = false>
SXD void replay_region(const ReplayParams& P, u64 i, ReplayRegionOut& o, sx_finding* fout, u8* aout, u64 abase,
                       u32 cap_f = 0, u32 cap_b = 0, u8* win_ext = nullptr) {
    const u8* bytes = P.data;
    const u64 len = P.len;
    const u32 W = P.W;
    const u64 want = win_start(P.runs[i].start, W);
    constexpr u32 kOb = QBIG ? kObCapBig : kObCap, kWinMax = QBIG ? kMaxWindowBig : kMaxWindow;
    u8 ob[kOb];
    alignas(16) u8 win_own[EXT_WIN ? 16 : kWinMax + kBackBytes];
    u8* const row = EXT_WIN ? win_ext : win_own;
    u8* const win = row + kBackBytes;
    u64 staged = ~0ull;
    NearBytes near;
    DDecoder dec;

    if (want >= kBackBytes) {
        if (EXT_WIN) stage_window_words(bytes + want - kBackBytes, kBackBytes, row);
        else stage_window(bytes + want - kBackBytes, kBackBytes, row);
        near.p = row; near.lo = want - kBackBytes; near.hi = want;
    }
    u32 leftover_len;
    bool maybe_cut = false;
    if (P.runs[i].chars & kPieceCont) {
        const u64 delta = P.runs[i].chars & ~kPieceCont;
        if (delta < 4ull * P.q) leftover_len = derive_in_run<ENC>(P.q, P.encoding, P.table, bytes + (want - delta), (u32)delta, dec, ob, kOb, &maybe_cut);
        else { (void)derive_at<ENC>(P, want, 0, dec, ob, near); leftover_len = 0; maybe_cut = true; }
    } else leftover_len = derive_at<ENC>(P, want, 0, dec, ob, near);

    u64 ri = i;
    u32 n_find = 0, n_bytes = 0, windows = 0;
    u32 status = kRegionOk;
    u64 pos = want;
    bool cached = MODE == 2;

    const u64 n_look = P.n_look ? P.n_look : P.n_runs;
    auto piece_at = [&](u64 p) -> bool {
        while (ri < n_look && P.runs[ri].end <= p) ri++;
        return ri < n_look && P.runs[ri].start == p && (P.runs[ri].chars & kPieceCont);
    };
    auto region_over = [&](u64 p) -> bool {
        while (ri < n_look && P.runs[ri].end <= p) ri++;
        if (ri < n_look && (regions_may_touch(P) ? P.runs[ri].start < p : win_start(P.runs[ri].start, W) <= p)) return false;
        return true;
    };
    auto may_drop = [&](const u8* lo, u32 n) -> bool {
        if (n == 0) return true;
        if (n < P.long_run) return true;
        u32 chars = 0;
        for (u32 k = 0; k < n; k++) chars += (lo[k] & 0xC0) != 0x80;
        return chars < P.long_run;
    };

    bool done = false;
    while (!done && pos < len) {
        const u64 soff = pos / kSliceLen * kSliceLen;
        const u32 slen = (u32)(len - soff < kSliceLen ? len - soff : kSliceLen);
        const u64 consumed = P.consumed0 + soff;
        const u32 slice_index = (u32)(soff / kSliceLen) + P.slice_base;
        u32 din = (u32)(pos - soff);
        bool is_last_window = false;
        while (din < slen) {
            u32 dend;
            if (din + W < slen) dend = din + W; else { is_last_window = true; dend = slen; }
            if (++windows > P.max_windows) { status = kRegionTooLong; done = true; break; }
            const u32 wb = din;
            u32 dout = leftover_len;
            for (;;) {
                if (staged != soff + wb) {
                    if (EXT_WIN) stage_window_words(bytes + soff + wb, dend - wb, win);
                    else stage_window(bytes + soff + wb, dend - wb, win);
                    staged = soff + wb;
                    if (near.p == row && staged == want) near.hi = soff + dend;
                    else { near.p = win; near.lo = staged; near.hi = soff + dend; }
                }
                if (P.skip && leftover_len == 0 && !maybe_cut && din < dend && ddec_idle<ENC>(dec)) {
                    const u64 p = soff + din, wend = soff + dend;
                    while (ri < n_look && P.runs[ri].end <= p) ri++;
                    const u64 rs = ri < n_look ? P.runs[ri].start : ~0ull;
                    if (rs >= wend) {
                        if (regions_may_touch(P) || (P.long_run > 1 && (ri >= n_look || win_start(rs, W) > wend))) {
                            leftover_len = 0; dout = 0; din = dend;
                            ddec_reset(dec, (int)P.encoding, P.table);
                            break;
                        }
                        leftover_len = derive_at<ENC>(P, wend, p, dec, ob, near);
                        dout = leftover_len;
                        din = dend;
                        break;
                    }
                    if (rs > p) {
                        const u64 vs = call_start_before<ENC>(P, p, rs, near);
                        if (vs > p) din = (u32)(vs - soff);
                    }
                }
                const DStep r = ddecode<ENC>(dec, win + (din - wb), dend - din, ob + dout, kOb - dout, false);
                if (r.result == RES_OUTPUT_FULL) { status = kRegionTooLong; done = true; break; }
                u8 precision = SX_PRECISION_EXACT;
                if (r.written > 0 && din == 0 && (ob[dout] & 0x80)) {
                    DDecoder fresh;
                    ddec_reset(fresh, (int)P.encoding, P.table);
                    u8 probe[8] = { 0, 0, 0, 0, 0, 0, 0, 0 };
                    const u32 pn = slen < 32 ? slen : 32;
                    const DStep pr = ddecode<ENC>(fresh, bytes + soff, pn, probe, 8, true);
                    const u32 filled = dout + r.written < 8 ? dout + r.written : 8;
                    bool same = pr.written != 0;
                    for (u32 t = 0; t < pr.written && same; t++) same = (t < filled ? ob[t] : 0) == probe[t];
                    if (!same) precision = SX_PRECISION_BEFORE;
                }
                u32 split_start = dout;
                const u32 split_end = dout + r.written;
                if (leftover_len > 0) { split_start -= leftover_len; leftover_len = 0; precision = SX_PRECISION_BEFORE; }
                const bool invalid_after = r.result == RES_MALFORMED;
                const bool continue_str = maybe_cut;
                maybe_cut = false;
                const bool may_yield = continue_str || !invalid_after || split_end - split_start >= P.chars_min_nb;
                if (split_end > split_start && may_yield) {
                    DSplit it{ ob + split_start, ob + split_end, ob + split_start, continue_str, invalid_after };
                    DChunk ch;
                    while (dsplit_next(P, it, ch)) {
                        if (!ch.again) {
                            bool put = MODE != 0;
                            if (MODE == 2) { put = n_find < cap_f && n_bytes + ch.len <= cap_b; cached = cached && put; }
                            if (put) {
                                sx_finding f;
                                f.position = consumed + din;
                                f.str_off = (u32)(abase + n_bytes);
                                f.str_len = ch.len;
                                f.precision = precision;
                                f.completes_previous = ch.completes ? 1 : 0;
                                f.mission_id = (u8)P.mission_id;
                                f.reserved = 0;
                                f.input_file_id = (int16_t)P.file_id;
                                f.reserved2 = 0;
                                f.slice_index = slice_index;
                                fout[n_find] = f;
                                for (u32 t = 0; t < ch.len; t++) aout[n_bytes + t] = ch.s[t];
                            }
                            n_find++; n_bytes += ch.len;
                            leftover_len = 0;
                            maybe_cut = ch.maybe_cut;
                        } else {
                            leftover_len = ch.len;
                            maybe_cut = false;
                        }
                        precision = SX_PRECISION_AFTER;
                    }
                }
                dout += r.written;
                din += r.read;
                if (r.result == RES_INPUT_EMPTY) break;
            }
            if (done) break;
            if (leftover_len) {
                const u32 from = dout - leftover_len;
                if (from) for (u32 t = 0; t < leftover_len; t++) ob[t] = ob[from + t];
            }
            const bool digit_pending = (ENC == 4) && enc_is_gb((int)P.encoding) && dec.gb2 != 0;
            if (piece_at(soff + din) || (!maybe_cut && !digit_pending && may_drop(ob, leftover_len) && region_over(soff + din))) { done = true; break; }
        }
        pos = soff + din;
        (void)is_last_window;
    }
    o.end = pos;
    o.n_find = n_find;
    o.n_bytes = n_bytes;
    o.status = status;
    o.pad = cached ? 1u : 0u;
}

template <int MODE>
SXD void replay_region_any(const ReplayParams& P, u64 i, ReplayRegionOut& o, sx_finding* fout, u8* aout, u64 abase,
                           u32 cap_f = 0, u32 cap_b = 0) {
#define SX_RR(E)                                                                                  \
    do {                                                                                          \
        if (P.q > 64) replay_region<MODE, E, false, true>(P, i, o, fout, aout, abase, cap_f, cap_b); \
        else replay_region<MODE, E>(P, i, o, fout, aout, abase, cap_f, cap_b);                     \
    } while (0)
    switch (enc_family(P.encoding)) {
        case 1: SX_RR(1); break;
        case 2: SX_RR(2); break;
        case 3: SX_RR(3); break;
        case 4: SX_RR(4); break;
        case 5: SX_RR(5); break;
        default: SX_RR(0); break;
    }
#undef SX_RR
}


}
```

stringsext_amd/csrc/sx_sort.hip:

```cpp
#include <hip/hip_runtime.h>
#include <cstring>
#include <cstdio>
#include <cstdlib>
#include <ctime>
#include <rocprim/device/device_radix_sort.hpp>
#include <rocprim/device/device_scan.hpp>
#include <rocprim/iterator/counting_iterator.hpp>
#include <rocprim/iterator/transform_iterator.hpp>

#include "sx_device.hpp"

namespace sx {

__global__ __launch_bounds__(256) void split_records_kernel(const DevRun* recs, uint32_t n, uint64_t* keys, uint64_t* vals) {
    const uint32_t i = blockIdx.x * 256u + threadIdx.x;
    if (i >= n) return;
    const DevRun r = recs[i];
    const bool invalid = r.len == kRecInvalidLen && r.chars_flags == kRecInvalidFlags;
    keys[i] = invalid ? ~0ull : r.start;
    vals[i] = ((uint64_t)r.chars_flags << 32) | r.len;
}
__global__ __launch_bounds__(256) void join_records_kernel(const uint64_t* keys, const uint64_t* vals, uint32_t n, DevRun* out) {
    const uint32_t i = blockIdx.x * 256u + threadIdx.x;
    if (i >= n) return;
    DevRun r;
    r.start = keys[i]; r.len = (uint32_t)vals[i]; r.chars_flags = (uint32_t)(vals[i] >> 32);
    out[i] = r;
}

size_t sort_scratch_bytes(uint32_t n) {
    size_t tmp = 0;
    uint64_t* nul = nullptr;
    (void)rocprim::radix_sort_pairs(nullptr, tmp, nul, nul, nul, nul, (size_t)n, 0, 64, (hipStream_t)0);
    return (size_t)n * 8 * 4 + tmp + 1024;
}

hipError_t sort_records(DevRun* recs, uint32_t n, uint64_t max_key, void* scratch, size_t scratch_bytes, hipStream_t stream, bool dbg) {
    if (n == 0) return hipSuccess;
    uint64_t* k0 = (uint64_t*)scratch;
    uint64_t* v0 = k0 + n;
    uint64_t* k1 = v0 + n;
    uint64_t* v1 = k1 + n;
    uint8_t* tmp = (uint8_t*)(((uintptr_t)(v1 + n) + 255) & ~(uintptr_t)255);
    size_t tmp_bytes = scratch_bytes - (size_t)(tmp - (uint8_t*)scratch);
    const unsigned blocks = (n + 255) / 256;
    auto stamp = [&](const char* what) {
        if (!dbg) return;
        (void)hipStreamSynchronize(stream);
        timespec ts; clock_gettime(CLOCK_MONOTONIC, &ts);
        fprintf(stderr, "[sx]     %s at %.3f ms\n", what, ts.tv_sec * 1e3 + ts.tv_nsec * 1e-6);
    };
    stamp("sort: begin");
    hipLaunchKernelGGL(split_records_kernel, dim3(blocks), dim3(256), 0, stream, recs, n, k0, v0);
    stamp("sort: split done");
    unsigned end_bit = 1;
    while (end_bit < 63 && (max_key >> end_bit)) end_bit++;
    end_bit++;
    hipError_t e = rocprim::radix_sort_pairs(tmp, tmp_bytes, k0, k1, v0, v1, (size_t)n, 0, end_bit, stream);
    if (e != hipSuccess) return e;
    stamp("sort: radix done");
    hipLaunchKernelGGL(join_records_kernel, dim3(blocks), dim3(256), 0, stream, k1, v1, n, recs);
    return hipGetLastError();
}


constexpr uint32_t kScanPerBlock = 1024;
__global__ __launch_bounds__(256) void region_block_scan_kernel(const uint32_t* counts, uint64_t n, uint32_t* local_off,
                                                                uint32_t* block_sum) {
    __shared__ uint32_t wsum[4];
    const uint64_t i0 = ((uint64_t)blockIdx.x * 256 + threadIdx.x) * 4;
    uint32_t c[4], t = 0;
    for (int j = 0; j < 4; j++) { c[j] = i0 + j < n ? counts[i0 + j] : 0u; t += c[j]; }
    uint32_t inc = t;
    const uint32_t lane = threadIdx.x & 63;
    for (int o = 1; o < 64; o <<= 1) { const uint32_t v = __shfl_up(inc, o); if ((int)lane >= o) inc += v; }
    if (lane == 63) wsum[threadIdx.x >> 6] = inc;
    __syncthreads();
    uint32_t before = 0;
    for (uint32_t w = 0; w < (threadIdx.x >> 6); w++) before += wsum[w];
    uint32_t run = before + inc - t;
    for (int j = 0; j < 4; j++) { if (i0 + j < n) local_off[i0 + j] = run; run += c[j]; }
    if (threadIdx.x == 255) block_sum[blockIdx.x] = before + inc;
}
__global__ __launch_bounds__(256) void region_sum_scan_kernel(uint32_t* block_sum, uint32_t n_blocks, uint32_t* total) {
    __shared__ uint32_t wsum[4];
    __shared__ uint32_t carry_s;
    if (threadIdx.x == 0) carry_s = 0;
    __syncthreads();
    for (uint32_t base = 0; base < n_blocks; base += 256) {
        const uint32_t i = base + threadIdx.x;
        const uint32_t v = i < n_blocks ? block_sum[i] : 0u;
        uint32_t inc = v;
        const uint32_t lane = threadIdx.x & 63;
        for (int o = 1; o < 64; o <<= 1) { const uint32_t u = __shfl_up(inc, o); if ((int)lane >= o) inc += u; }
        if (lane == 63) wsum[threadIdx.x >> 6] = inc;
        __syncthreads();
        uint32_t before = carry_s;
        for (uint32_t w = 0; w < (threadIdx.x >> 6); w++) before += wsum[w];
        if (i < n_blocks) block_sum[i] = before + inc - v;
        __syncthreads();
        if (threadIdx.x == 255) carry_s = before + inc;
        __syncthreads();
    }
    if (threadIdx.x == 0) *total = carry_s;
}
constexpr uint32_t kPackLanes = 16;
__global__ __launch_bounds__(256) void region_pack_kernel(const DevRun* recs, const uint32_t* counts, const uint32_t* local_off,
                                                          const uint32_t* block_off, uint64_t n_regions, uint32_t region_cap,
                                                          DevRun* out) {
    const uint64_t t = (uint64_t)blockIdx.x * 256 + threadIdx.x;
    const uint64_t w = t / kPackLanes;
    if (w >= n_regions) return;
    const uint32_t n = counts[w];
    const DevRun* reg = recs + w * region_cap;
    const uint64_t base = (uint64_t)block_off[w / kScanPerBlock] + local_off[w];
    for (uint32_t j = (uint32_t)(t % kPackLanes); j < n; j += kPackLanes) {
        const DevRun r = reg[j];
        uint32_t rank = 0;
        for (uint32_t i = 0; i < n; i++) rank += reg[i].start < r.start ? 1u : 0u;
        out[base + rank] = r;
    }
}
__global__ __launch_bounds__(256) void region_invalidate_kernel(DevRun* recs, const uint32_t* counts, uint64_t n_regions,
                                                                uint32_t region_cap) {
    const uint64_t s = (uint64_t)blockIdx.x * 256 + threadIdx.x;
    const uint64_t w = s / region_cap;
    if (w >= n_regions) return;
    if ((uint32_t)(s - w * region_cap) >= counts[w]) {
        DevRun r; r.start = 0; r.len = kRecInvalidLen; r.chars_flags = kRecInvalidFlags;
        recs[s] = r;
    }
}
hipError_t invalidate_region_slack(DevRun* recs, const uint32_t* counts, uint64_t n_regions, uint32_t region_cap, hipStream_t stream) {
    const uint64_t slots = n_regions * region_cap;
    if (slots == 0) return hipSuccess;
    hipLaunchKernelGGL(region_invalidate_kernel, dim3((unsigned)((slots + 255) / 256)), dim3(256), 0, stream, recs, counts, n_regions,
                       region_cap);
    return hipGetLastError();
}
size_t compact_scratch_bytes(uint64_t n_regions) {
    return n_regions * 4 + ((n_regions + kScanPerBlock - 1) / kScanPerBlock) * 4 + 1024;
}
hipError_t compact_regions(const DevRun* recs, const uint32_t* counts, uint64_t n_regions, uint32_t region_cap, DevRun* out,
                           uint32_t* total, void* scratch, size_t scratch_bytes, hipStream_t stream) {
    if (n_regions == 0) return hipMemsetAsync(total, 0, 4, stream);
    const uint32_t n_blocks = (uint32_t)((n_regions + kScanPerBlock - 1) / kScanPerBlock);
    if (scratch_bytes < compact_scratch_bytes(n_regions)) return hipErrorInvalidValue;
    uint32_t* local_off = (uint32_t*)scratch;
    uint32_t* block_sum = local_off + n_regions;
    hipLaunchKernelGGL(region_block_scan_kernel, dim3(n_blocks), dim3(256), 0, stream, counts, n_regions, local_off, block_sum);
    hipLaunchKernelGGL(region_sum_scan_kernel, dim3(1), dim3(256), 0, stream, block_sum, n_blocks, total);
    const uint64_t threads = n_regions * kPackLanes;
    hipLaunchKernelGGL(region_pack_kernel, dim3((unsigned)((threads + 255) / 256)), dim3(256), 0, stream, recs, counts, local_off,
                       block_sum, n_regions, region_cap, out);
    return hipGetLastError();
}

struct RecIsHead {
    const DevRun* v;
    __device__ uint32_t operator()(uint32_t i) const {
        const DevRun r = v[i];
        if (r.start == ~0ull) return 0u;
        if (i == 0 || !(r.chars_flags & kRecStartOpen)) return 1u;
        const DevRun p = v[i - 1];
        return ((p.chars_flags & kRecEndOpen) && p.start + p.len == r.start) ? 0u : 1u;
    }
};
__global__ __launch_bounds__(256) void accumulate_runs_kernel(const DevRun* v, uint32_t n, const uint32_t* rid, sx_run* tmp) {
    const uint32_t i = blockIdx.x * 256u + threadIdx.x;
    if (i >= n) return;
    const DevRun r = v[i];
    if (r.start == ~0ull) return;
    const uint32_t id = rid[i] - 1u;
    const bool head = i == 0 || rid[i - 1] != rid[i];
    const bool tail = i + 1 >= n || rid[i + 1] != rid[i] || v[i + 1].start == ~0ull;
    const unsigned long long chars = r.chars_flags & kRecCharsMask, end = r.start + r.len;
    if (head && tail) { sx_run o; o.start = r.start; o.end = end; o.chars = chars; tmp[id] = o; return; }
    if (head) tmp[id].start = r.start;
    atomicAdd((unsigned long long*)&tmp[id].chars, chars);
    atomicMax((unsigned long long*)&tmp[id].end, end);
}

struct RunLongFlag {
    const sx_run* t; uint64_t min_chars;
    __device__ uint32_t operator()(uint32_t i) const { return t[i].chars >= min_chars ? 1u : 0u; }
};
__global__ __launch_bounds__(256) void scatter_long_runs_kernel(const sx_run* tmp, uint32_t n, uint64_t min_chars, const uint32_t* pos,
                                                                sx_run* out, uint32_t* out_count) {
    const uint32_t i = blockIdx.x * 256u + threadIdx.x;
    if (i >= n) return;
    const sx_run r = tmp[i];
    const bool keep = r.chars >= min_chars;
    if (keep) out[pos[i]] = r;
    if (i == n - 1) *out_count = pos[i] + (keep ? 1u : 0u);
}
static size_t merge_tmp_bytes(uint32_t n) {
    size_t a = 0, b = 0;
    auto heads = rocprim::make_transform_iterator(rocprim::counting_iterator<uint32_t>(0), RecIsHead{ nullptr });
    (void)rocprim::inclusive_scan(nullptr, a, heads, (uint32_t*)nullptr, (size_t)n, rocprim::plus<uint32_t>(), (hipStream_t)0);
    auto flags = rocprim::make_transform_iterator(rocprim::counting_iterator<uint32_t>(0), RunLongFlag{ nullptr, 1 });
    (void)rocprim::exclusive_scan(nullptr, b, flags, (uint32_t*)nullptr, 0u, (size_t)n, rocprim::plus<uint32_t>(), (hipStream_t)0);
    return (a > b ? a : b) + 256;
}
size_t merge_scratch_bytes(uint32_t n) {
    return ((size_t)n * 4 + 255) / 256 * 256 + ((size_t)n * sizeof(sx_run) + 511) / 256 * 256 + merge_tmp_bytes(n);
}

hipError_t merge_sorted_records(const DevRun* recs, uint32_t n, uint64_t min_chars, void* scratch, size_t scratch_bytes,
                                sx_run* out, uint32_t* out_count, hipStream_t stream) {
    if (n == 0) return hipMemsetAsync(out_count, 0, 4, stream);
    uint8_t* base = (uint8_t*)scratch;
    uint32_t* rid = (uint32_t*)base;
    const size_t rid_bytes = ((size_t)n * 4 + 255) / 256 * 256;
    sx_run* tmp = (sx_run*)(base + rid_bytes);
    const size_t run_bytes = ((size_t)n * sizeof(sx_run) + 511) / 256 * 256;
    void* rp_tmp = base + rid_bytes + run_bytes;
    size_t rp_bytes = scratch_bytes - rid_bytes - run_bytes;
    auto heads = rocprim::make_transform_iterator(rocprim::counting_iterator<uint32_t>(0), RecIsHead{ recs });
    hipError_t e = rocprim::inclusive_scan(rp_tmp, rp_bytes, heads, rid, (size_t)n, rocprim::plus<uint32_t>(), stream);
    if (e != hipSuccess) return e;
    e = hipMemsetAsync(tmp, 0, (size_t)n * sizeof(sx_run), stream);
    if (e != hipSuccess) return e;
    hipLaunchKernelGGL(accumulate_runs_kernel, dim3((n + 255) / 256), dim3(256), 0, stream, recs, n, rid, tmp);
    const uint64_t minc = min_chars ? min_chars : 1;
    auto flags = rocprim::make_transform_iterator(rocprim::counting_iterator<uint32_t>(0), RunLongFlag{ tmp, minc });
    rp_bytes = scratch_bytes - rid_bytes - run_bytes;
    uint32_t* pos = rid;
    e = rocprim::exclusive_scan(rp_tmp, rp_bytes, flags, pos, 0u, (size_t)n, rocprim::plus<uint32_t>(), stream);
    if (e != hipSuccess) return e;
    hipLaunchKernelGGL(scatter_long_runs_kernel, dim3((n + 255) / 256), dim3(256), 0, stream, tmp, n, minc, pos, out, out_count);
    return hipGetLastError();
}


constexpr int kMergeLists = 16;
struct MergeLists {
    const sx_finding* f[kMergeLists];
    uint64_t nf[kMergeLists];
    uint64_t out_base[kMergeLists];
    uint32_t arena_adj[kMergeLists];
    const uint8_t* a[kMergeLists];
    uint32_t off0[kMergeLists];
    int n;
};
struct MergeRange { uint64_t base; uint32_t shift, pad; };

__global__ void merge_range_kernel(MergeLists L, uint32_t T, MergeRange* out) {
    if (threadIdx.x || blockIdx.x) return;
    uint64_t lo = ~0ull, hi = 0;
    for (int m = 0; m < L.n; m++)
        if (L.nf[m]) {
            const uint64_t a = L.f[m][0].position, b = L.f[m][L.nf[m] - 1].position;
            lo = a < lo ? a : lo; hi = b > hi ? b : hi;
        }
    if (lo > hi) { lo = 0; hi = 0; }
    const uint64_t span = hi - lo;
    uint32_t s = 0;
    while (s < 63 && (span >> s) + 1 > (uint64_t)T) s++;
    out->base = lo; out->shift = s; out->pad = 0;
}
__device__ __forceinline__ uint64_t merge_lower(const sx_finding* f, uint64_t lo, uint64_t hi, uint64_t p) {
    while (lo < hi) {
        const uint64_t mid = lo + (hi - lo) / 2;
        if (f[mid].position < p) lo = mid + 1; else hi = mid;
    }
    return lo;
}
__device__ __forceinline__ uint64_t merge_upper(const sx_finding* f, uint64_t lo, uint64_t hi, uint64_t p) {
    while (lo < hi) {
        const uint64_t mid = lo + (hi - lo) / 2;
        if (f[mid].position <= p) lo = mid + 1; else hi = mid;
    }
    return lo;
}
__global__ __launch_bounds__(256) void merge_bounds_kernel(MergeLists L, uint32_t T, const MergeRange* rg, uint32_t* bounds) {
    const uint64_t i = (uint64_t)blockIdx.x * 256 + threadIdx.x;
    const uint64_t per = (uint64_t)T + 1;
    if (i >= per * (uint64_t)L.n) return;
    const int m = (int)(i / per);
    const uint32_t t = (uint32_t)(i % per);
    uint64_t v;
    if (t == 0) v = 0;
    else if (t == T) v = L.nf[m];
    else v = merge_lower(L.f[m], 0, L.nf[m], rg->base + ((uint64_t)t << rg->shift));
    bounds[i] = (uint32_t)v;
}
__global__ __launch_bounds__(256) void merge_place_kernel(MergeLists L, int m, uint32_t T, const MergeRange* rg, const uint32_t* bounds,
                                                          void* out, int packed, uint64_t* src) {
    const uint64_t i = (uint64_t)blockIdx.x * 256 + threadIdx.x;
    if (i >= L.nf[m]) return;
    sx_finding f = L.f[m][i];
    const uint64_t p = f.position, base = rg->base;
    uint64_t t = p <= base ? 0 : (p - base) >> rg->shift;
    if (t > (uint64_t)T - 1) t = (uint64_t)T - 1;
    uint64_t rank = i;
    for (int o = 0; o < L.n; o++) {
        if (o == m || !L.nf[o]) continue;
        const uint32_t* b = bounds + (uint64_t)o * ((uint64_t)T + 1) + t;
        const uint64_t lo = b[0], hi = b[1];
        rank += o < m ? merge_upper(L.f[o], lo, hi, p) : merge_lower(L.f[o], lo, hi, p);
    }
    if (src) src[rank] = (uint64_t)(uintptr_t)(L.a[m] + (uint32_t)(f.str_off - L.off0[m]));
    f.str_off += L.arena_adj[m];
    if (packed) {
        sx_finding16 p;
        p.position = f.position; p.str_off = f.str_off; p.str_len = (uint16_t)f.str_len;
        p.flags = (uint8_t)((f.precision & 3u) | (f.completes_previous ? 4u : 0u)); p.mission_id = f.mission_id;
        ((sx_finding16*)out)[rank] = p;
    } else ((sx_finding*)out)[rank] = f;
}
static uint32_t merge_tiles(uint64_t n) {
    const uint64_t t = n / 64;
    return (uint32_t)(t < 1 ? 1 : t > (1u << 22) ? (1u << 22) : t);
}

__global__ __launch_bounds__(256) void merge_gather_in_kernel(const sx_finding* src, uint64_t n, uint32_t arena_base, uint64_t out_base,
                                                              sx_finding* all, uint64_t* keys, uint64_t* vals) {
    const uint64_t i = (uint64_t)blockIdx.x * 256 + threadIdx.x;
    if (i >= n) return;
    sx_finding f = src[i];
    f.str_off += arena_base;
    all[out_base + i] = f;
    keys[out_base + i] = f.position;
    vals[out_base + i] = out_base + i;
}
__global__ __launch_bounds__(256) void merge_gather_out_kernel(const sx_finding* all, const uint64_t* order, uint64_t n, sx_finding* out) {
    const uint64_t i = (uint64_t)blockIdx.x * 256 + threadIdx.x;
    if (i < n) out[i] = all[order[i]];
}
static size_t merge_sort_scratch_bytes(uint64_t n) {
    size_t tmp = 0;
    uint64_t* nul = nullptr;
    (void)rocprim::radix_sort_pairs(nullptr, tmp, nul, nul, nul, nul, (size_t)n, 0, 64, (hipStream_t)0);
    return n * sizeof(sx_finding) + 4 * n * 8 + tmp + 2048;
}
bool merge_part_can_pack(uint64_t n, int n_missions) { return n_missions <= kMergeLists && n < 0xFFFFFFFFull; }
static size_t merge_tables_bytes(uint64_t n, int n_missions) { return (256 + ((size_t)merge_tiles(n) + 1) * 4 * (size_t)n_missions + 255) / 256 * 256; }
size_t merge_findings_scratch_bytes(uint64_t n, int n_missions, int ordered) {
    if (n_missions > kMergeLists || n >= 0xFFFFFFFFull) return merge_sort_scratch_bytes(n);
    if (ordered) return 512 + merge_tables_bytes(n, n_missions) + ((size_t)n * 8 + 255) / 256 * 256 + order_strings_scratch_bytes(n);
    return 512 + ((size_t)merge_tiles(n) + 1) * 4 * (size_t)n_missions + 256;
}
hipError_t merge_findings_device_part(const sx_finding* const* f, const uint8_t* const* a, const uint64_t* nf, const uint64_t* nb,
                                      const uint32_t* off0, int n_missions, void* out, void* scratch, size_t scratch_bytes,
                                      hipStream_t stream, int packed, int ordered) {
    uint64_t n = 0;
    for (int m = 0; m < n_missions; m++) n += nf[m];
    if (n == 0) return hipSuccess;
    if (scratch_bytes < merge_findings_scratch_bytes(n, n_missions, ordered)) return hipErrorInvalidValue;
    if (ordered && !(n_missions <= kMergeLists && n < 0xFFFFFFFFull)) return hipErrorInvalidValue;
    uint8_t* base = (uint8_t*)(((uintptr_t)scratch + 255) & ~(uintptr_t)255);
    if (packed && !(n_missions <= kMergeLists && n < 0xFFFFFFFFull)) return hipErrorInvalidValue;
    sx_finding* out_f = (sx_finding*)out;
    uint8_t* out_a = (uint8_t*)out + n * (packed ? sizeof(sx_finding16) : sizeof(sx_finding));
    if (n_missions <= kMergeLists && n < 0xFFFFFFFFull) {
        MergeLists L{};
        L.n = n_missions;
        uint64_t ab = 0;
        for (int m = 0; m < n_missions; m++) {
            L.f[m] = f[m]; L.nf[m] = nf[m]; L.arena_adj[m] = (uint32_t)ab - off0[m];
            L.a[m] = a[m]; L.off0[m] = off0[m];
            if (nf[m] && nb[m] && !ordered) {
                hipError_t e = hipMemcpyAsync(out_a + ab, a[m], nb[m], hipMemcpyDeviceToDevice, stream);
                if (e != hipSuccess) return e;
            }
            ab += nb[m];
        }
        const uint32_t T = merge_tiles(n);
        MergeRange* rg = (MergeRange*)base;
        uint32_t* bounds = (uint32_t*)(base + 256);
        uint64_t* src = ordered ? (uint64_t*)(base + merge_tables_bytes(n, n_missions)) : nullptr;
        hipLaunchKernelGGL(merge_range_kernel, dim3(1), dim3(64), 0, stream, L, T, rg);
        const uint64_t nb_threads = ((uint64_t)T + 1) * (uint64_t)n_missions;
        hipLaunchKernelGGL(merge_bounds_kernel, dim3((unsigned)((nb_threads + 255) / 256)), dim3(256), 0, stream, L, T, rg, bounds);
        for (int m = 0; m < n_missions; m++)
            if (nf[m])
                hipLaunchKernelGGL(merge_place_kernel, dim3((unsigned)((nf[m] + 255) / 256)), dim3(256), 0, stream, L, m, T, rg, bounds, (void*)out_f, packed, src);
        if (ordered) {
            uint8_t* rest = (uint8_t*)src + ((size_t)n * 8 + 255) / 256 * 256;
            return order_part_strings(out, n, packed, src, out_a, rest, scratch_bytes - (size_t)(rest - (uint8_t*)scratch), stream);
        }
        return hipGetLastError();
    }
    sx_finding* all = (sx_finding*)base;
    uint64_t* k0 = (uint64_t*)(base + ((n * sizeof(sx_finding) + 255) & ~(size_t)255));
    uint64_t* v0 = k0 + n;
    uint64_t* k1 = v0 + n;
    uint64_t* v1 = k1 + n;
    uint8_t* tmp = (uint8_t*)(((uintptr_t)(v1 + n) + 255) & ~(uintptr_t)255);
    size_t tmp_bytes = scratch_bytes - (size_t)(tmp - (uint8_t*)scratch);
    uint64_t fb = 0, ab = 0;
    for (int m = 0; m < n_missions; m++) {
        if (nf[m]) {
            hipLaunchKernelGGL(merge_gather_in_kernel, dim3((unsigned)((nf[m] + 255) / 256)), dim3(256), 0, stream, f[m], nf[m],
                               (uint32_t)ab - off0[m], fb, all, k0, v0);
            hipError_t e = hipMemcpyAsync(out_a + ab, a[m], nb[m], hipMemcpyDeviceToDevice, stream);
            if (e != hipSuccess) return e;
        }
        fb += nf[m]; ab += nb[m];
    }
    hipError_t e = rocprim::radix_sort_pairs(tmp, tmp_bytes, k0, k1, v0, v1, (size_t)n, 0, 64, stream);
    if (e != hipSuccess) return e;
    hipLaunchKernelGGL(merge_gather_out_kernel, dim3((unsigned)((n + 255) / 256)), dim3(256), 0, stream, all, v1, n, out_f);
    return hipGetLastError();
}

typedef unsigned int copy_v4u __attribute__((ext_vector_type(4)));
template <bool NT>
__global__ __launch_bounds__(1024) void copy_bytes_kernel(copy_v4u* __restrict__ dst, const copy_v4u* __restrict__ src, uint64_t n16,
                                                          uint8_t* dst_tail, const uint8_t* src_tail, uint32_t n_tail) {
    const uint64_t per = (n16 + gridDim.x - 1) / gridDim.x;
    const uint64_t begin = per * blockIdx.x, end = begin + per < n16 ? begin + per : n16;
    const uint64_t stride = blockDim.x;
    uint64_t i = begin + threadIdx.x;
    n16 = end;
    for (; i + 3 * stride < n16; i += 4 * stride) {
        const copy_v4u a = __builtin_nontemporal_load(src + i), b = __builtin_nontemporal_load(src + i + stride);
        const copy_v4u c = __builtin_nontemporal_load(src + i + 2 * stride), d = __builtin_nontemporal_load(src + i + 3 * stride);
        if (NT) {
            __builtin_nontemporal_store(a, dst + i); __builtin_nontemporal_store(b, dst + i + stride);
            __builtin_nontemporal_store(c, dst + i + 2 * stride); __builtin_nontemporal_store(d, dst + i + 3 * stride);
        } else { dst[i] = a; dst[i + stride] = b; dst[i + 2 * stride] = c; dst[i + 3 * stride] = d; }
    }
    for (; i < n16; i += stride) dst[i] = src[i];
    if (blockIdx.x == 0 && threadIdx.x < n_tail) dst_tail[threadIdx.x] = src_tail[threadIdx.x];
}
__global__ __launch_bounds__(64) void small_copy_kernel(uint32_t* dst, const uint32_t* src, uint32_t n_words) {
    const uint32_t t = blockIdx.x * 64 + threadIdx.x, nt = gridDim.x * 64;
    if ((((uintptr_t)dst | (uintptr_t)src) & 15) == 0) {
        const uint32_t n4 = n_words / 4;
        for (uint32_t i = t; i < n4; i += nt) ((uint4*)dst)[i] = ((const uint4*)src)[i];
        for (uint32_t i = n4 * 4 + t; i < n_words; i += nt) dst[i] = src[i];
    } else for (uint32_t i = t; i < n_words; i += nt) dst[i] = src[i];
}
hipError_t launch_small_copy(void* pinned_dst, const void* dev_src, size_t bytes, hipStream_t stream) {
    if (!bytes) return hipSuccess;
    if ((((uintptr_t)pinned_dst | (uintptr_t)dev_src | bytes) & 3) != 0 || bytes > (1u << 20)) return hipErrorInvalidValue;
    const unsigned blocks = bytes <= 16384 ? 1u : (bytes <= 131072 ? 2u : 4u);
    hipLaunchKernelGGL(small_copy_kernel, dim3(blocks), dim3(64), 0, stream, (uint32_t*)pinned_dst, (const uint32_t*)dev_src, (uint32_t)(bytes / 4));
    return hipGetLastError();
}
hipError_t launch_copy_bytes(void* dst, const void* src, uint64_t bytes, uint32_t workgroups, hipStream_t stream, int threads, bool nt) {
    if (!bytes) return hipSuccess;
    if ((((uintptr_t)dst | (uintptr_t)src) & 15) != 0) return hipErrorInvalidValue;
    const uint64_t n16 = bytes / 16;
    if (nt)
        hipLaunchKernelGGL(copy_bytes_kernel<true>, dim3(workgroups ? workgroups : 2), dim3((unsigned)threads), 0, stream, (copy_v4u*)dst, (const copy_v4u*)src, n16,
                           (uint8_t*)dst + n16 * 16, (const uint8_t*)src + n16 * 16, (uint32_t)(bytes - n16 * 16));
    else
        hipLaunchKernelGGL(copy_bytes_kernel<false>, dim3(workgroups ? workgroups : 2), dim3((unsigned)threads), 0, stream, (copy_v4u*)dst, (const copy_v4u*)src, n16,
                           (uint8_t*)dst + n16 * 16, (const uint8_t*)src + n16 * 16, (uint32_t)(bytes - n16 * 16));
    return hipGetLastError();
}

__global__ __launch_bounds__(64) void merge_cuts_kernel(const sx_finding* f, uint64_t n, uint64_t nb, const uint64_t* cuts, uint32_t n_cuts,
                                                        uint64_t* idx, uint64_t* off) {
    const uint32_t j = blockIdx.x * 64u + threadIdx.x;
    if (j >= n_cuts) return;
    const uint64_t c = cuts[j];
    uint64_t lo = 0, hi = n;
    while (lo < hi) {
        const uint64_t mid = lo + (hi - lo) / 2;
        if (f[mid].position < c) lo = mid + 1; else hi = mid;
    }
    idx[j] = lo;
    off[j] = lo < n ? f[lo].str_off : nb;
}
hipError_t launch_merge_cuts(const sx_finding* f, uint64_t n, uint64_t nb, const uint64_t* cuts, uint32_t n_cuts, uint64_t* idx,
                             uint64_t* off, hipStream_t stream) {
    if (n_cuts == 0) return hipSuccess;
    hipLaunchKernelGGL(merge_cuts_kernel, dim3((n_cuts + 63) / 64), dim3(64), 0, stream, f, n, nb, cuts, n_cuts, idx, off);
    return hipGetLastError();
}

}
```

stringsext_amd/csrc/sx_stage_a.cpp:

```cpp
#include "sx_ctx.hpp"

using namespace sx;

namespace sx {

static bool large_regions_fit(uint64_t len, uint64_t n_regions, uint32_t cap) {
    const uint64_t slots = n_regions * cap;
    return slots < (1ull << 31) && slots * sizeof(DevRun) <= std::max<uint64_t>(256ull << 20, len / 2);
}

static uint32_t subchunk_bytes(const sx_ctx* ctx) {
    const uint32_t sub = ctx->opt.subchunk_bytes ? ctx->opt.subchunk_bytes : 256u * 1024u;
    return std::max<uint32_t>(kTileBytes, sub / kTileBytes * kTileBytes);
}

static bool fusion_allowed(const sx_ctx* ctx) {
    return !(ctx->opt.flags & (SX_OPT_NO_FUSED_SCAN | SX_OPT_MISSION_STREAMS)) && !ctx->sw.mission_streams && ctx->sw.fused && ctx->sw.scan_warm < 0;
}

ScanParams scan_params(const sx_ctx* ctx, int mission, const ScanSlot& s, const uint8_t* d_bytes, uint64_t len,
                       uint32_t parity, uint64_t min_chars) {
    const Mission& m = ctx->missions[(size_t)mission];
    ScanParams p = m.proto;
    p.data = d_bytes; p.len = len; p.subchunk = subchunk_bytes(ctx); p.parity = parity;
    p.pair_lut = ctx->dev[(size_t)mission].d_pair_lut;
    if (p.gb4) {
        p.gb_ranges = ctx->dev[(size_t)mission].d_table ? ctx->dev[(size_t)mission].d_table + kGbN : nullptr;
        p.ubf = m.c.ubf;
        if (!p.gb_ranges) p.gb4 = 0;
    }
    p.wave_prio = ctx->sw.scan_prio;
    p.min_chars = (uint32_t)std::min<uint64_t>(min_chars, kRecCharsMask);
    if (p.min_chars == 0) p.min_chars = 1;
    p.cand_bytes = std::min<uint32_t>(p.min_chars * (m.is_utf16() ? 2u : 1u), 14u);
    {
        uint32_t have = 1;
        for (int i = 0; i < 5; i++) {
            const uint32_t sh = have < p.cand_bytes ? std::min(have, p.cand_bytes - have) : 0;
            p.cand_sh[i] = sh;
            have += sh;
        }
    }
    p.capacity = s.capacity; p.recs = s.d_recs; p.counters = s.d_counters;
    p.region_cap = s.region_cap; p.region_counts = s.d_cnt; p.grid_flags = s.d_grid;
    unsigned occ = ctx->scan_blocks_per_cu;
    p.persistent = (occ >= 1 && occ < 8) ? occ * ctx->n_cus : 0u;
    return p;
}

int stage_a_launch(sx_ctx* ctx, const std::vector<int>& which, const uint8_t* d_bytes, uint64_t len,
                   const std::vector<uint32_t>& parity, const std::vector<uint64_t>& min_chars, int si) {
    if (len == 0) return SX_OK;
    for (size_t k = 0; k < which.size(); k++) {
        MissionDev& d = ctx->dev[(size_t)which[k]];
        ScanSlot& s = d.slot[si];
        if (s.free_pending) { HIP_TRY(ctx, hipStreamWaitEvent(d.stream, s.ev_free, 0)); s.free_pending = false; }
        {
            const uint32_t sub = subchunk_bytes(ctx);
            const uint64_t n_regions = (len + sub - 1) / sub;
            if (ctx->dense.size() != ctx->missions.size()) ctx->dense.assign(ctx->missions.size(), 0);
            s.region_cap = 0; s.n_regions = n_regions;
            const uint32_t dn = ctx->dense[(size_t)which[k]];
            const uint32_t want_cap = dn > 1 ? dn : (dn == 0 ? ctx->region_cap : 0u);
            if (ctx->region_cap && want_cap &&
                (dn > 1 ? large_regions_fit(len, n_regions, want_cap) : n_regions * want_cap < (1ull << 28))) {
                s.region_cap = want_cap;
                int rc = ensure_capacity(ctx, s, (uint32_t)(n_regions * s.region_cap));
                if (rc != SX_OK && dn > 1) {
                    (void)hipGetLastError();
                    ctx->dense[(size_t)which[k]] = 1;
                    s.region_cap = 0;
                    rc = SX_OK;
                }
                if (rc != SX_OK) return rc;
                if (s.region_cap == 0) goto launch;
                if (s.cnt_cap < n_regions) {
                    if (s.d_cnt) HIP_TRY(ctx, hipFree(s.d_cnt));
                    s.d_cnt = nullptr; s.cnt_cap = 0;
                    HIP_TRY(ctx, hipMalloc((void**)&s.d_cnt, (n_regions + n_regions / 4 + 64) * 4));
                    s.cnt_cap = n_regions + n_regions / 4 + 64;
                }
            }
        }
    launch:
        const bool dbcs = ctx->missions[(size_t)which[k]].is_dbcs();
        if (dbcs) {
            const uint32_t sub = subchunk_bytes(ctx);
            const uint64_t n_sub = (len + sub - 1) / sub;
            if (s.grid_cap < n_sub) {
                if (s.d_grid) HIP_TRY(ctx, hipFree(s.d_grid));
                s.d_grid = nullptr; s.grid_cap = 0;
                HIP_TRY(ctx, hipMalloc((void**)&s.d_grid, (n_sub + n_sub / 4 + 64) * 4));
                s.grid_cap = n_sub + n_sub / 4 + 64;
            }
        }
    }
    std::vector<char> fused(which.size(), 0);
    std::vector<ScanParams> params(which.size());
    for (size_t k = 0; k < which.size(); k++)
        params[k] = scan_params(ctx, which[k], ctx->dev[(size_t)which[k]].slot[si], d_bytes, len, parity[k], min_chars[k]);
    if (fusion_allowed(ctx)) {
        FusedParams fp{};
        uint32_t used = 0;
        size_t member[kFusedMax] = { 0, 0, 0 };
        for (size_t k = 0; k < which.size(); k++) {
            if (params[k].persistent) continue;
            const int sl = fused_slot_of(ctx->missions[(size_t)which[k]].kind, params[k]);
            if (sl < 0 || (used >> sl) & 1u) continue;
            if (sl >= 1 && (used & 6u) && ((fp.m[(used & 2u) ? 1 : 2].parity ^ params[k].parity) & 1u)) continue;
            used |= 1u << sl; fp.m[sl] = params[k]; member[sl] = k;
        }
        if (__builtin_popcount(used) >= 2 || used == 1u) {
            hipStream_t st = nullptr;
            for (int sl = 0; sl < kFusedMax; sl++) if ((used >> sl) & 1u) {
                MissionDev& d = ctx->dev[(size_t)which[member[sl]]];
                if (!st) st = d.stream;
                HIP_TRY(ctx, hipMemsetAsync(d.slot[si].d_counters, 0, kCounterWords * sizeof(uint32_t), st));
            }
            for (int sl = 0; sl < kFusedMax; sl++) if ((used >> sl) & 1u) HIP_TRY(ctx, hipEventRecord(ctx->dev[(size_t)which[member[sl]]].slot[si].ev0, st));
            HIP_TRY(ctx, launch_scan_fused(fp, used, st, ctx->sw.fused_prefilter));
            bool first = true;
            for (int sl = 0; sl < kFusedMax; sl++) if ((used >> sl) & 1u) {
                ScanSlot& s = ctx->dev[(size_t)which[member[sl]]].slot[si];
                HIP_TRY(ctx, hipEventRecord(s.ev1, st));
                s.fused = true; s.fused_first = first; first = false;
                fused[member[sl]] = 1;
            }
            ctx->stats.fused_launches++;
        }
    }
    for (size_t k = 0; k < which.size(); k++) {
        if (fused[k]) continue;
        MissionDev& d = ctx->dev[(size_t)which[k]];
        ScanSlot& s = d.slot[si];
        s.fused = false; s.fused_first = false;
        const bool dbcs = ctx->missions[(size_t)which[k]].is_dbcs();
        const ScanParams& p = params[k];
        const uint64_t n_sub = (len + p.subchunk - 1) / p.subchunk;
        for (int w = ctx->sw.scan_warm; w > 0; w--) {
            if (dbcs) HIP_TRY(ctx, hipMemsetAsync(s.d_grid, 0, n_sub * 4, d.stream));
            HIP_TRY(ctx, hipMemsetAsync(s.d_counters, 0, kCounterWords * sizeof(uint32_t), d.stream));
            HIP_TRY(ctx, launch_scan(ctx->missions[(size_t)which[k]].kind, p, d.stream));
        }
        if (dbcs) HIP_TRY(ctx, hipMemsetAsync(s.d_grid, 0, n_sub * 4, d.stream));
        HIP_TRY(ctx, hipMemsetAsync(s.d_counters, 0, kCounterWords * sizeof(uint32_t), d.stream));
        HIP_TRY(ctx, hipEventRecord(s.ev0, d.stream));
        HIP_TRY(ctx, launch_scan(ctx->missions[(size_t)which[k]].kind, p, d.stream));
        HIP_TRY(ctx, hipEventRecord(s.ev1, d.stream));
        if (dbcs) { d.grid_of_scan = s.d_grid; d.grid_sub = p.subchunk; d.grid_data = d_bytes; d.grid_len = len; }
    }
    return SX_OK;
}

int stage_a_finish(sx_ctx* ctx, const std::vector<int>& which, const uint8_t* d_bytes, uint64_t len,
                   const std::vector<uint32_t>& parity, const std::vector<uint64_t>& min_chars, int si,
                   std::vector<RunList>* out, bool cut_into_pieces, const ReplayJob* wave_job) {
    out->assign(which.size(), RunList{});
    if (len == 0) return SX_OK;
    const double t0 = now_ms();
    for (size_t k = 0; k < which.size(); k++) {
        MissionDev& d = ctx->dev[(size_t)which[k]];
        ScanSlot& s = d.slot[si];
        HIP_TRY(ctx, hipEventSynchronize(s.ev1));
        const double t_ev = now_ms();
        SX_TL("mission %d: scan kernel done", which[k]);
        float ms = 0;
        HIP_TRY(ctx, hipEventElapsedTime(&ms, s.ev0, s.ev1));
        if (which[k] < 16) ctx->stats.kernel_ms[which[k]] += ms;
        if (s.fused && s.fused_first) ctx->stats.fused_ms += ms;
        if (which[k] < 64) { if (s.fused) ctx->stats.fused_mask |= 1ull << which[k]; else ctx->stats.fused_mask &= ~(1ull << which[k]); }
        uint32_t counters[4] = { 0, 0, 0, 0 };
        std::vector<uint32_t> hc(kCounterWords);
        bool skip_runs = false;
        for (int round = 0;; round++) {
            { const int rb = read_back_sync(ctx, d, d.stream_b, hc.data(), s.d_counters, kCounterWords * sizeof(uint32_t)); if (rb != SX_OK) return rb; }
            counters[0] = hc[0]; counters[3] = hc[3];
            {
                uint64_t heavy = 0, recs = 0;
                for (uint32_t sh = 0; sh < kStatShards; sh++) { heavy += hc[kStatBase + sh * kStatStride]; recs += hc[kStatBase + sh * kStatStride + 1]; }
                counters[1] = (uint32_t)std::min<uint64_t>(heavy, 0xFFFFFFFFull); counters[2] = (uint32_t)std::min<uint64_t>(recs, 0xFFFFFFFFull);
            }
            if (round == 0 && wave_job) {
                const uint64_t total = s.region_cap ? counters[2] : counters[0];
                if (wave_replay_wanted(ctx, *wave_job, (size_t)which[k], total, counters[1])) {
                    RunList& rl = (*out)[k];
                    rl.n = wave_replay_wanted(ctx, *wave_job, (size_t)which[k], total) ? total : std::max<uint64_t>(total, len / 16);
                    rl.p = nullptr; rl.skipped = true; rl.complete = true;
                    skip_runs = true;
                    break;
                }
            }
            if (s.region_cap) {
                if (counters[0] == 0) break;
                const uint32_t big = (counters[3] + counters[3] / 4 + 127) / 64 * 64;
                if (s.region_cap == ctx->region_cap && counters[3] && large_regions_fit(len, s.n_regions, big) && !ctx->sw.no_large_regions) {
                    ctx->dense[(size_t)which[k]] = big;
                    s.region_cap = big;
                    if (ensure_capacity(ctx, s, (uint32_t)(s.n_regions * big)) != SX_OK) {
                        (void)hipGetLastError();
                        ctx->dense[(size_t)which[k]] = 1;
                        s.region_cap = 0;
                    }
                } else {
                    ctx->dense[(size_t)which[k]] = 1;
                    s.region_cap = 0;
                }
            } else {
                if (counters[0] <= s.capacity) break;
                if (round >= 8) { ctx->err = "device run-record buffer kept overflowing"; return SX_E_NOMEM; }
                int rc = ensure_capacity(ctx, s, counters[0] + counters[0] / 8 + 1024);
                if (rc != SX_OK) return rc;
            }
            const ScanParams p = scan_params(ctx, which[k], s, d_bytes, len, parity[k], min_chars[k]);
            const double tr0 = now_ms();
            if (p.grid_flags) HIP_TRY(ctx, hipMemsetAsync(p.grid_flags, 0, ((len + p.subchunk - 1) / p.subchunk) * 4, d.stream_b));
            HIP_TRY(ctx, hipMemsetAsync(s.d_counters, 0, kCounterWords * sizeof(uint32_t), d.stream_b));
            HIP_TRY(ctx, launch_scan(ctx->missions[(size_t)which[k]].kind, p, d.stream_b));
            if (p.grid_flags) { d.grid_of_scan = p.grid_flags; d.grid_sub = p.subchunk; d.grid_data = d_bytes; d.grid_len = len; }
            HIP_TRY(ctx, hipStreamSynchronize(d.stream_b));
            ctx->stats.rescans++;
            ctx->stats.rescan_ms += now_ms() - tr0;
        }
        const double tc0 = now_ms();
        SX_TL("mission %d: counters read (%u records)", which[k], s.region_cap ? counters[2] : counters[0]);
        if (ctx->sw.timing2) fprintf(stderr, "[sx]   mission %d: kernel done at +%.2f ms, counters at +%.2f ms\n", which[k], t_ev - t0, tc0 - t0);
        if (skip_runs) {
            HIP_TRY(ctx, hipEventRecord(s.ev_free, d.stream_b));
            s.free_pending = true;
            if (ctx->sw.timing) fprintf(stderr, "[sx] mission %d: kernel %.2f ms, %llu records counted: string-dense, every window is replayed\n", which[k], ms, (unsigned long long)(*out)[k].n);
            ctx->stats.run_records += (*out)[k].n;
            ctx->stats.bytes_scanned += len;
            ctx->stats.heavy_tiles += counters[1];
            continue;
        }
        uint32_t nrec = counters[0];
        const DevRun* d_records = s.d_recs;
        const bool large_regions = s.region_cap > ctx->region_cap && ctx->region_cap;
        const bool regions = s.region_cap != 0 && !large_regions;
        if (large_regions) {
            HIP_TRY(ctx, invalidate_region_slack(s.d_recs, s.d_cnt, s.n_regions, s.region_cap, d.stream_b));
            nrec = (uint32_t)(s.n_regions * s.region_cap);
        }
        if (regions) {
            const uint64_t slots = s.n_regions * s.region_cap;
            if (s.packed_cap < slots) {
                if (s.d_packed) HIP_TRY(ctx, hipFree(s.d_packed));
                s.d_packed = nullptr; s.packed_cap = 0;
                HIP_TRY(ctx, hipMalloc((void**)&s.d_packed, (slots + slots / 8 + 64) * sizeof(DevRun)));
                s.packed_cap = slots + slots / 8 + 64;
            }
            int rc = ensure_scratch(ctx, compact_scratch_bytes(s.n_regions)); if (rc != SX_OK) return rc;
            HIP_TRY(ctx, compact_regions(s.d_recs, s.d_cnt, s.n_regions, s.region_cap, s.d_packed, s.d_counters + 1, ctx->d_scratch,
                                         ctx->d_scratch_cap, d.stream_b));
            { const int rb = read_back_sync(ctx, d, d.stream_b, &nrec, s.d_counters + 1, 4); if (rb != SX_OK) return rb; }
            d_records = s.d_packed;
            SX_TL("mission %d: regions packed (%u)", which[k], nrec);
        } else if (ctx->region_cap && !large_regions && nrec < s.n_regions * ctx->region_cap / 4)
            ctx->dense[(size_t)which[k]] = 0;
        const uint32_t join_min = ctx->sw.device_join_min;
        const bool dev_sorted = nrec >= join_min && nrec > 0;
        double tc1 = tc0;
        RunList& rl = (*out)[k];
        if (dev_sorted) {
            const size_t sb = std::max(sort_scratch_bytes(nrec), merge_scratch_bytes(nrec));
            int rc = ensure_scratch(ctx, sb); if (rc != SX_OK) return rc;
            if (d.ev_runs) HIP_TRY(ctx, hipEventSynchronize(d.ev_runs));
            rc = ensure_rp(ctx, d, 0, (uint64_t)nrec * sizeof(sx_run)); if (rc != SX_OK) return rc;
            if (!regions) HIP_TRY(ctx, sort_records(s.d_recs, nrec, len, ctx->d_scratch, ctx->d_scratch_cap, d.stream_b, ctx->sw.timing2));
            if (ctx->sw.timing2) { HIP_TRY(ctx, hipStreamSynchronize(d.stream_b)); fprintf(stderr, "[sx]   sort done +%.2f ms\n", now_ms() - tc0); }
            HIP_TRY(ctx, merge_sorted_records(d_records, nrec, min_chars[k], ctx->d_scratch, ctx->d_scratch_cap,
                                              (sx_run*)d.d_rp[0], s.d_counters + 2, d.stream_b));
            HIP_TRY(ctx, hipEventRecord(s.ev_free, d.stream_b));
            s.free_pending = true;
            if (ctx->sw.timing2) { HIP_TRY(ctx, hipStreamSynchronize(d.stream_b)); fprintf(stderr, "[sx]   join done +%.2f ms\n", now_ms() - tc0); }
            uint32_t nruns32 = 0;
            { const int rb = read_back_sync(ctx, d, d.stream_b, &nruns32, s.d_counters + 2, 4); if (rb != SX_OK) return rb; }
            uint64_t nruns = nruns32;
            SX_TL("mission %d: joined (%u runs)", which[k], nruns32);
            const sx_run* d_list = (const sx_run*)d.d_rp[0];
            const Mission& mm = ctx->missions[(size_t)which[k]];
            if (cut_into_pieces && nruns && !ctx->sw.no_pieces && mm.c.grep_char < 0 && !mm.c.require_same_unicode_block
                && mm.c.chars_min_nb >= 1 && mm.c.chars_min_nb <= mm.q && mm.q <= 255) {
                ReplayParams SP{};
                SP.data = d_bytes; SP.len = len; SP.runs = d_list; SP.n_runs = nruns; SP.encoding = mm.c.encoding; SP.table = d.d_table;
                SP.chars_min_nb = mm.c.chars_min_nb; SP.same_block = 0; SP.q = (uint32_t)mm.q; SP.W = (uint32_t)mm.window; SP.grep_char = -1;
                rc = ensure_scratch(ctx, split_scratch_bytes(nruns) + 64); if (rc != SX_OK) return rc;
                uint64_t* d_total = (uint64_t*)ctx->d_scratch;
                HIP_TRY(ctx, launch_split_count(SP, ctx->d_scratch + 64, ctx->d_scratch_cap - 64, d_total, d.stream_b));
                uint64_t total = 0;
                { const int rb = read_back_sync(ctx, d, d.stream_b, &total, d_total, 8); if (rb != SX_OK) return rb; }
                if (total > nruns && total < (1ull << 32) && ensure_rp(ctx, d, 9, total * sizeof(sx_run)) == SX_OK) {
                    HIP_TRY(ctx, launch_split_write(SP, ctx->d_scratch + 64, total, (sx_run*)d.d_rp[9], d.stream_b));
                    HIP_TRY(ctx, hipStreamSynchronize(d.stream_b));
                    d_list = (const sx_run*)d.d_rp[9];
                    nruns = total;
                } else (void)hipGetLastError();
            }
            tc1 = now_ms();
            SX_TL("mission %d: cut into pieces (%llu)", which[k], (unsigned long long)nruns);
            if ((uint64_t)nruns * sizeof(sx_run) > d.h_runs_cap) {
                if (d.h_runs) HIP_TRY(ctx, hipHostFree(d.h_runs));
                d.h_runs = nullptr; d.h_runs_cap = 0;
                const uint64_t cap = (uint64_t)nruns * sizeof(sx_run) * 5 / 4 + 4096;
                HIP_TRY(ctx, hipHostMalloc((void**)&d.h_runs, cap, hipHostMallocNonCoherent));
                d.h_runs_cap = cap;
            }
            rl.p = d.h_runs; rl.n = nruns; rl.on_device = true; rl.dev_ptr = d_list;
            if (large_regions && nruns < s.n_regions * ctx->region_cap / 4) ctx->dense[(size_t)which[k]] = 0;
            if (nruns) {
                if (!ctx->d2h_stream) HIP_TRY(ctx, hipStreamCreateWithFlags(&ctx->d2h_stream, hipStreamNonBlocking));
                if (!d.ev_runs) HIP_TRY(ctx, hipEventCreateWithFlags(&d.ev_runs, hipEventDisableTiming));
                rl.dev_src = d_list; rl.copy_bytes = (size_t)nruns * sizeof(sx_run);
                rl.copy_stream = ctx->d2h_stream; rl.ready = d.ev_runs; rl.issued = false;
            }
        } else {
            int rc = ensure_pinned(ctx, (uint64_t)nrec * sizeof(DevRun) + 16);
            if (rc != SX_OK) return rc;
            DevRun* recs_p = (DevRun*)ctx->h_pin;
            if (nrec) {
                { const int rb = read_back_async(ctx, d.stream_b, recs_p, d_records, (size_t)nrec * sizeof(DevRun)); if (rb != SX_OK) return rb; }
                HIP_TRY(ctx, hipStreamSynchronize(d.stream_b));
            }
            tc1 = now_ms();
            if (regions) merge_sorted_device_runs(recs_p, nrec, min_chars[k], &rl.own);
            else merge_device_runs(recs_p, nrec, min_chars[k], 64 * 1024, &rl.own);
            rl.use_own();
        }
        if (ctx->sw.timing)
            fprintf(stderr, "[sx] mission %d: kernel %.2f ms, %u %s, %s %.2f ms, %s %.2f ms -> %zu runs\n", which[k], ms, nrec,
                    regions ? "records (regions)" : (large_regions ? "record slots (large regions)" : "record slots (pool)"), dev_sorted ? (regions ? "device pack+join" : "device sort+join") : "d2h",
                    tc1 - tc0, dev_sorted ? "d2h runs" : "host join", now_ms() - tc1, rl.size());
        ctx->stats.run_records += rl.size();
        ctx->stats.bytes_scanned += len;
        ctx->stats.heavy_tiles += counters[1];
    }
    ctx->stats.device_ms += now_ms() - t0;
    return SX_OK;
}

int device_runs(sx_ctx* ctx, const std::vector<int>& which, const uint8_t* d_bytes, uint64_t len,
                const std::vector<uint32_t>& parity, const std::vector<uint64_t>& min_chars,
                std::vector<RunList>* out) {
    int rc = stage_a_launch(ctx, which, d_bytes, len, parity, min_chars, 0);
    if (rc != SX_OK) return rc;
    return stage_a_finish(ctx, which, d_bytes, len, parity, min_chars, 0, out);
}


}
```

stringsext_amd/csrc/sx_switches.cpp:

```cpp
#include "sx_switches.hpp"

#include <stdio.h>
#include <stdlib.h>

#include <algorithm>

namespace sx {

static bool present(const char* name) { return getenv(name) != nullptr; }
static bool on_unless_0(const char* name) { const char* e = getenv(name); return !(e && !atoi(e)); }
static bool on_if_nonzero(const char* name) { const char* e = getenv(name); return e && atoi(e); }
static int int_or(const char* name, int unset) { const char* e = getenv(name); return e ? atoi(e) : unset; }
static int64_t i64_or(const char* name, int64_t unset) { const char* e = getenv(name); return e ? (int64_t)atoll(e) : unset; }
static int clamped_or(const char* name, int lo, int hi, int unset) { const char* e = getenv(name); return e ? std::max(lo, std::min(hi, atoi(e))) : unset; }
static uint64_t u64_at_least(const char* name, uint64_t lo, uint64_t unset) { const char* e = getenv(name); return e ? std::max<uint64_t>(lo, (uint64_t)atoll(e)) : unset; }

Switches Switches::from_env() {
    Switches s;
    if (const char* e = getenv("SX_PIN_FLAGS")) s.pin_flags = (int64_t)(unsigned)strtoul(e, nullptr, 0);
    s.small_copy = on_unless_0("SX_SMALL_COPY");
    if (const char* e = getenv("SX_REPLAY_THREADS")) s.replay_threads = (int)std::max(1u, std::min(256u, (unsigned)atoi(e)));
    s.result_on_device = on_if_nonzero("SX_RESULT_ON_DEVICE");
    s.scan_blocks_per_cu = int_or("SX_SCAN_BLOCKS_PER_CU", s.scan_blocks_per_cu);
    if (const char* e = getenv("SX_REGION_CAP")) s.region_cap = (int64_t)(uint32_t)atoi(e);
    s.scan_cus = clamped_or("SX_SCAN_CUS", 1, INT32_MAX, s.scan_cus);
    if (const char* e = getenv("SX_PRIO")) s.prio_n = std::max(0, sscanf(e, "%d,%d", &s.prio_scan, &s.prio_post));
    s.mission_streams = present("SX_MISSION_STREAMS");
    s.scan_prio = (uint32_t)int_or("SX_SCAN_PRIO", (int)s.scan_prio);
    s.fused = on_unless_0("SX_FUSED");
    s.fused_prefilter = int_or("SX_FUSED_PREFILTER", s.fused_prefilter);
    s.scan_warm = clamped_or("SX_SCAN_WARM", 0, INT32_MAX, s.scan_warm);
    s.no_large_regions = present("SX_NO_LARGE_REGIONS");
    s.device_join_min = (uint32_t)int_or("SX_DEVICE_JOIN_MIN", (int)s.device_join_min);
    s.no_pieces = present("SX_NO_PIECES");
    s.probe_rot = (uint32_t)int_or("SX_PROBE_ROT", (int)s.probe_rot);
    s.host_replay = present("SX_HOST_REPLAY");
    s.device_replay = present("SX_DEVICE_REPLAY");
    s.host_stitch = present("SX_HOST_STITCH");
    s.no_replay_skip = present("SX_NO_REPLAY_SKIP");
    s.no_grid_bound = present("SX_NO_GRID_BOUND");
    s.no_replay_cache = present("SX_NO_REPLAY_CACHE");
    s.max_region_windows = (uint32_t)clamped_or("SX_MAX_REGION_WINDOWS", 1, INT32_MAX, (int)s.max_region_windows);
    s.replay_cache_mib = i64_or("SX_REPLAY_CACHE_MIB", s.replay_cache_mib);
    s.fast_replay = on_unless_0("SX_FAST_REPLAY");
    s.count_waves = int_or("SX_COUNT_WAVES", s.count_waves);
    s.stitch_block = clamped_or("SX_STITCH_BLOCK", 0, INT32_MAX, s.stitch_block);
    s.slabs = clamped_or("SX_SLABS", 1, 64, s.slabs);
    s.replay_copy_wgs = int_or("SX_REPLAY_COPY_WGS", s.replay_copy_wgs);
    s.host_merge = present("SX_HOST_MERGE");
    s.packed = on_unless_0("SX_PACKED");
    s.merge_part_mib = u64_at_least("SX_MERGE_PART_MIB", 1, s.merge_part_mib);
    s.merge_part_findings = u64_at_least("SX_MERGE_PART_FINDINGS", 1024, s.merge_part_findings);
    s.merge_copy_wgs = int_or("SX_MERGE_COPY_WGS", s.merge_copy_wgs);
    s.merge_copy_nt = int_or("SX_MERGE_COPY_NT", s.merge_copy_nt);
    s.merge_copy_threads = clamped_or("SX_MERGE_COPY_THREADS", 64, 1024, s.merge_copy_threads);
    s.host_merge_seg_bytes = u64_at_least("SX_HOST_MERGE_SEG_BYTES", 1, s.host_merge_seg_bytes);
    s.splice_seg_bytes = u64_at_least("SX_SPLICE_SEG_BYTES", 1, s.splice_seg_bytes);
    s.piece_mib = i64_or("SX_PIECE_MIB", s.piece_mib);
    s.seq_piece_kib = i64_or("SX_SEQ_PIECE_KIB", s.seq_piece_kib);
    s.seq_piece_mib = i64_or("SX_SEQ_PIECE_MIB", s.seq_piece_mib);
    s.debug_entry = present("SX_DEBUG_ENTRY");
    s.busiest_last = int_or("SX_BUSIEST_LAST", s.busiest_last);
    if (const char* e = getenv("SX_DEFER_MIN_BYTES")) s.defer_min_bytes = (uint64_t)atoll(e);
    s.wave_threads = on_unless_0("SX_WAVE_THREADS");
    s.timeline = int_or("SX_TIMELINE", s.timeline);
    s.timing = present("SX_TIMING");
    s.timing2 = present("SX_TIMING2");
    if (const char* e = getenv("SX_WAVE_REPLAY")) s.wave_replay = atoi(e) != 0;
    s.wave_keep_scan = present("SX_WAVE_KEEP_SCAN");
    if (const char* e = getenv("SX_WAVE_BYTES_PER_RUN")) s.wave_bytes_per_run = (uint64_t)atoll(e);
    s.wave_stream_prio = int_or("SX_WAVE_STREAM_PRIO", s.wave_stream_prio);
    s.wave_batches = clamped_or("SX_WAVE_BATCHES", 1, 64, s.wave_batches);
    s.wave_slabs = clamped_or("SX_WAVE_SLABS", 1, 64, s.wave_slabs);
    s.wave_lut = on_if_nonzero("SX_WAVE_LUT");
    s.wave_desc = on_unless_0("SX_WAVE_DESC");
    s.wave_desc_cap = clamped_or("SX_WAVE_DESC_CAP", 1, INT32_MAX, s.wave_desc_cap);
    s.wave_fail = present("SX_WAVE_FAIL");
    if (const char* e = getenv("SX_WAVE_REPAIR")) s.wave_repair = atoi(e) ? std::max(1, atoi(e)) : 0;
    s.wave_same = on_unless_0("SX_WAVE_SAME");
    if (const char* e = getenv("SX_SCAN_STREAM_MIB")) s.scan_stream_mib = (uint64_t)atoll(e);
    s.ingest_mmap = present("SX_INGEST_MMAP");
    return s;
}

}
```

stringsext_amd/csrc/sx_switches.hpp:

```cpp
#pragma once
#include <stdint.h>

namespace sx {

struct Switches {
    int64_t pin_flags = -1;
    bool small_copy = true;
    int replay_threads = 0;
    bool result_on_device = false;
    int scan_blocks_per_cu = -1;
    int64_t region_cap = -1;
    int scan_cus = 0;
    int prio_n = -1, prio_scan = 0, prio_post = 0;
    bool mission_streams = false;
    uint32_t scan_prio = 0;
    bool fused = true;
    int fused_prefilter = -1;
    int scan_warm = -1;
    bool no_large_regions = false;
    uint32_t device_join_min = 65536;
    bool no_pieces = false;
    uint32_t probe_rot = 0;
    bool host_replay = false;
    bool device_replay = false;
    bool host_stitch = false;
    bool no_replay_skip = false;
    bool no_grid_bound = false;
    bool no_replay_cache = false;
    uint32_t max_region_windows = 0;
    int64_t replay_cache_mib = -1;
    bool fast_replay = true;
    int count_waves = 4;
    int stitch_block = 0;
    int slabs = 0;
    int replay_copy_wgs = 0;
    bool host_merge = false;
    bool packed = true;
    uint64_t merge_part_mib = 0;
    uint64_t merge_part_findings = 0;
    int merge_copy_wgs = -1;
    int merge_copy_nt = 1;
    int merge_copy_threads = 512;
    uint64_t host_merge_seg_bytes = 0;
    uint64_t splice_seg_bytes = 0;
    int64_t piece_mib = -1;
    int64_t seq_piece_kib = -1;
    int64_t seq_piece_mib = -1;
    bool debug_entry = false;
    int busiest_last = 0;
    uint64_t defer_min_bytes = 256ull << 20;
    bool wave_threads = true;
    int timeline = 0;
    bool timing = false;
    bool timing2 = false;
    int wave_replay = -1;
    bool wave_keep_scan = false;
    uint64_t wave_bytes_per_run = 0;
    int wave_stream_prio = -1;
    int wave_batches = 0;
    int wave_slabs = 0;
    bool wave_lut = false;
    bool wave_desc = true;
    int wave_desc_cap = 0;
    bool wave_fail = false;
    int wave_repair = -1;
    bool wave_same = true;
    uint64_t scan_stream_mib = 0;
    bool ingest_mmap = false;

    static Switches from_env();
};

}
```

Baseline: 4100.

## Add device chain path fusing region scan, pack, join and piece splitting

Adds a chained device path for region-mode records. It runs a single-pass scan of region counts using last-block tickets, then a pack, then a join kernel that counts runs and pieces, then a placement kernel that writes runs and split pieces directly. This replaces the previous sequence of separate rocprim scans, join, host readbacks of the run count and a separate split count/write pass. It also adds a pinned counter gather and falls back to the old path on count mismatch or very long chains, which adds code paths and an extra readback whenever the fallback is taken.

```diff
diff --git a/stringsext_amd/csrc/sx_api.cpp b/stringsext_amd/csrc/sx_api.cpp
--- a/stringsext_amd/csrc/sx_api.cpp
+++ b/stringsext_amd/csrc/sx_api.cpp
@@ -448,6 +448,8 @@
         if (ctx->ev_interleaved) (void)hipEventDestroy(ctx->ev_interleaved);
         if (ctx->d_input) (void)hipFree(ctx->d_input);
         if (ctx->d_scratch) (void)hipFree(ctx->d_scratch);
+        if (ctx->chain_tickets.d) (void)hipFree(ctx->chain_tickets.d);
+        if (ctx->h_counters) (void)hipHostFree(ctx->h_counters);
         if (ctx->h_pin) (void)hipHostFree(ctx->h_pin);
         if (ctx->h_pin2) (void)hipHostFree(ctx->h_pin2);
     }
diff --git a/stringsext_amd/csrc/sx_chain.hpp b/stringsext_amd/csrc/sx_chain.hpp
--- /dev/null
+++ b/stringsext_amd/csrc/sx_chain.hpp
@@ -0,0 +1,30 @@
+#pragma once
+#include "sx_device.hpp"
+
+namespace sx {
+
+struct ChainResult {
+    uint32_t nrec;
+    uint32_t nruns;
+    uint64_t pieces;
+    uint32_t flags;
+    uint32_t pad[3];
+};
+constexpr uint32_t kChainPieceOverflow = 1u;
+constexpr uint32_t kChainCountMismatch = 2u;
+constexpr uint32_t kChainLongWalk = 4u;
+constexpr uint32_t kChainWalkMax = 64;
+
+bool chain_takes_encoding(uint32_t encoding);
+
+struct ChainTickets { uint32_t* d = nullptr; uint32_t base[2] = { 0, 0 }; };
+
+size_t chain_scratch_bytes(uint64_t n_regions, uint32_t nrec);
+hipError_t launch_chain(const DevRun* recs, const uint32_t* counts, uint64_t n_regions, uint32_t region_cap, DevRun* packed, uint32_t nrec,
+                        const ReplayParams& P, uint64_t min_chars, bool cut, sx_run* runs, sx_run* pieces, uint64_t piece_cap,
+                        void* scratch, size_t scratch_bytes, ChainTickets* tickets, hipStream_t stream);
+const ChainResult* chain_result_of(const void* scratch);
+
+hipError_t launch_gather_counters(uint32_t* pinned_dst, const uint32_t* const* src, int n, hipStream_t stream);
+
+}
diff --git a/stringsext_amd/csrc/sx_chain_core.hpp b/stringsext_amd/csrc/sx_chain_core.hpp
--- /dev/null
+++ b/stringsext_amd/csrc/sx_chain_core.hpp
@@ -0,0 +1,55 @@
+#pragma once
+#include <stdint.h>
+
+#include "sx_chain.hpp"
+#include "sx_replay_core.hpp"
+
+namespace sx {
+
+struct ChainEnt {
+    u64 start, end, chars;
+    u64 pieces;
+};
+SXD bool chain_rec_valid(const DevRun& r) { return r.start != ~0ull; }
+SXD bool chain_continues(const DevRun& p, const DevRun& r) {
+    return chain_rec_valid(r) && (p.chars_flags & kRecEndOpen) && (r.chars_flags & kRecStartOpen) && p.start + p.len == r.start;
+}
+SXD bool chain_is_head(const DevRun* v, u32 i) {
+    if (!chain_rec_valid(v[i])) return false;
+    return i == 0 || !chain_continues(v[i - 1], v[i]);
+}
+SXD bool chain_join(const DevRun* v, u32 n, u32 i, sx_run& o) {
+    DevRun p = v[i];
+    o.start = p.start; o.end = p.start + p.len; o.chars = p.chars_flags & kRecCharsMask;
+    for (u32 k = i + 1, steps = 1; k < n && (p.chars_flags & kRecEndOpen); k++, steps++) {
+        const DevRun r = v[k];
+        if (!chain_continues(p, r)) break;
+        if (steps >= kChainWalkMax) return false;
+        o.end = r.start + r.len;
+        o.chars += r.chars_flags & kRecCharsMask;
+        p = r;
+    }
+    return true;
+}
+template <int ENC>
+SXD ChainEnt chain_entry(const ReplayParams& P, const DevRun* v, u32 n, u32 i, u64 min_chars, bool cut, bool* long_walk) {
+    ChainEnt e;
+    e.start = 0; e.end = 0; e.chars = 0; e.pieces = 0;
+    if (!chain_is_head(v, i)) return e;
+    sx_run r;
+    if (!chain_join(v, n, i, r)) { *long_walk = true; return e; }
+    e.start = r.start; e.end = r.end; e.chars = r.chars;
+    if (r.chars < min_chars) return e;
+    e.pieces = cut ? split_count_of<ENC>(P, r.start, r.end) : 1;
+    return e;
+}
+SXD void chain_place(const ChainEnt& e, u32 W, u64 at_run, u64 at_piece, sx_run* runs, sx_run* pieces, u64 piece_cap) {
+    if (!e.pieces) return;
+    sx_run r;
+    r.start = e.start; r.end = e.end; r.chars = e.chars;
+    runs[at_run] = r;
+    if (!pieces) return;
+    for (u64 k = 0; k < e.pieces && at_piece + k < piece_cap; k++) pieces[at_piece + k] = split_piece_of(r, W, k, e.pieces);
+}
+
+}
diff --git a/stringsext_amd/csrc/sx_ctx.hpp b/stringsext_amd/csrc/sx_ctx.hpp
--- a/stringsext_amd/csrc/sx_ctx.hpp
+++ b/stringsext_amd/csrc/sx_ctx.hpp
@@ -23,6 +23,7 @@
 
 #include "sx_host.hpp"
 #include "sx_switches.hpp"
+#include "sx_chain.hpp"
 
 namespace sx {
 
@@ -89,6 +90,8 @@
     uint32_t region_cap = 0;
     uint64_t n_regions = 0;
     bool fused = false, fused_first = false;
+    std::vector<int> fused_group;
+    std::vector<uint32_t> counters_read;
 };
 struct MissionDev {
     hipStream_t stream = nullptr;
@@ -109,6 +112,7 @@
     uint8_t* h_small = nullptr;
     std::vector<hipEvent_t> wave_ev;
     uint64_t last_out_runs = 0, last_out_bytes = 0;
+    uint64_t chain_pieces = 0;
 };
 
 
@@ -182,6 +186,8 @@
     uint8_t* h_pin = nullptr;   uint64_t h_pin_cap = 0;
     uint8_t* h_pin2 = nullptr;  uint64_t h_pin2_cap = 0;
     uint8_t* d_scratch = nullptr; uint64_t d_scratch_cap = 0;
+    sx::ChainTickets chain_tickets;
+    uint32_t* h_counters = nullptr;
 };
 
 #define HIP_TRY(ctx, expr)                                                                     \
diff --git a/stringsext_amd/csrc/sx_replay_core.hpp b/stringsext_amd/csrc/sx_replay_core.hpp
--- a/stringsext_amd/csrc/sx_replay_core.hpp
+++ b/stringsext_amd/csrc/sx_replay_core.hpp
@@ -189,9 +189,8 @@
 }
 
 template <int ENC>
-SXD u64 split_count(const ReplayParams& P, u64 i) {
+SXD u64 split_count_of(const ReplayParams& P, u64 rs, u64 re) {
     if (!mission_splittable(P)) return 1;
-    const u64 rs = P.runs[i].start, re = P.runs[i].end;
     const u64 inside = win_starts_below(re, P.W) - win_starts_below(rs + 1, P.W);
     if (inside == 0) return 1;
     const u64 fe = rs + char_len_at<ENC>(P, rs) - 1;
@@ -199,16 +198,18 @@
     if (ENC == 4 && enc_is_gb((int)P.encoding)) return gb_run_is_exact(P, rs, re) ? inside + 1 : 1;
     return valid_char_before<ENC>(P, rs) ? inside + 1 : 1;
 }
-SXD sx_run split_piece(const ReplayParams& P, u64 i, u64 k, u64 count) {
-    const sx_run r = P.runs[i];
+template <int ENC>
+SXD u64 split_count(const ReplayParams& P, u64 i) { return split_count_of<ENC>(P, P.runs[i].start, P.runs[i].end); }
+SXD sx_run split_piece_of(const sx_run& r, u32 W, u64 k, u64 count) {
     if (count <= 1) return r;
-    const u64 first = win_starts_below(r.start + 1, P.W);
+    const u64 first = win_starts_below(r.start + 1, W);
     sx_run o;
-    o.start = k == 0 ? r.start : win_start_no(first + k - 1, P.W);
-    o.end = k + 1 == count ? r.end : win_start_no(first + k, P.W);
+    o.start = k == 0 ? r.start : win_start_no(first + k - 1, W);
+    o.end = k + 1 == count ? r.end : win_start_no(first + k, W);
     o.chars = k == 0 ? r.chars : (kPieceCont | (o.start - r.start));
     return o;
 }
+SXD sx_run split_piece(const ReplayParams& P, u64 i, u64 k, u64 count) { return split_piece_of(P.runs[i], P.W, k, count); }
 template <int ENC> SXD bool run_is_piece(const sx_run& r) { return (r.chars & kPieceCont) != 0; }
 
 template <int ENC>
diff --git a/stringsext_amd/csrc/sx_sort.hip b/stringsext_amd/csrc/sx_sort.hip
--- a/stringsext_amd/csrc/sx_sort.hip
+++ b/stringsext_amd/csrc/sx_sort.hip
@@ -9,6 +9,12 @@
 #include <rocprim/iterator/transform_iterator.hpp>
 
 #include "sx_device.hpp"
+
+namespace sx {
+#define SXD __device__ __forceinline__
+#define SXD_NOINLINE __device__ __attribute__((noinline))
+}
+#include "sx_chain_core.hpp"
 
 namespace sx {
 
@@ -229,6 +235,192 @@
     e = rocprim::exclusive_scan(rp_tmp, rp_bytes, flags, pos, 0u, (size_t)n, rocprim::plus<uint32_t>(), stream);
     if (e != hipSuccess) return e;
     hipLaunchKernelGGL(scatter_long_runs_kernel, dim3((n + 255) / 256), dim3(256), 0, stream, tmp, n, minc, pos, out, out_count);
+    return hipGetLastError();
+}
+
+__device__ __forceinline__ bool chain_drew_last_ticket(uint32_t* ticket, uint32_t base, uint32_t* s_last) {
+    asm volatile("s_waitcnt vmcnt(0)" ::: "memory");
+    __syncthreads();
+    if (threadIdx.x == 0) {
+        const uint32_t t = __hip_atomic_fetch_add(ticket, 1u, __ATOMIC_RELAXED, __HIP_MEMORY_SCOPE_AGENT);
+        *s_last = t - base == gridDim.x - 1u ? 1u : 0u;
+    }
+    __syncthreads();
+    return *s_last != 0u;
+}
+__global__ __launch_bounds__(256) void chain_region_scan_kernel(const uint32_t* counts, uint64_t n, uint32_t* local_off, uint32_t* block_sum,
+                                                                uint32_t n_blocks, uint32_t* total, uint32_t* ticket, uint32_t ticket_base) {
+    __shared__ uint32_t wsum[4];
+    __shared__ uint32_t last_s;
+    const uint64_t i0 = ((uint64_t)blockIdx.x * 256 + threadIdx.x) * 4;
+    const uint32_t lane = threadIdx.x & 63;
+    {
+        uint32_t c[4], t = 0;
+        for (int j = 0; j < 4; j++) { c[j] = i0 + j < n ? counts[i0 + j] : 0u; t += c[j]; }
+        uint32_t inc = t;
+        for (int o = 1; o < 64; o <<= 1) { const uint32_t v = __shfl_up(inc, o); if ((int)lane >= o) inc += v; }
+        if (lane == 63) wsum[threadIdx.x >> 6] = inc;
+        __syncthreads();
+        uint32_t before = 0;
+        for (uint32_t w = 0; w < (threadIdx.x >> 6); w++) before += wsum[w];
+        uint32_t run = before + inc - t;
+        for (int j = 0; j < 4; j++) { if (i0 + j < n) local_off[i0 + j] = run; run += c[j]; }
+        if (threadIdx.x == 255) __hip_atomic_store(block_sum + blockIdx.x, before + inc, __ATOMIC_RELAXED, __HIP_MEMORY_SCOPE_AGENT);
+    }
+    if (!chain_drew_last_ticket(ticket, ticket_base, &last_s)) return;
+    uint32_t carry = 0;
+    for (uint32_t base = 0; base < n_blocks; base += 256) {
+        const uint32_t i = base + threadIdx.x;
+        const uint32_t v = i < n_blocks ? __hip_atomic_load(block_sum + i, __ATOMIC_RELAXED, __HIP_MEMORY_SCOPE_AGENT) : 0u;
+        uint32_t inc = v;
+        for (int o = 1; o < 64; o <<= 1) { const uint32_t u = __shfl_up(inc, o); if ((int)lane >= o) inc += u; }
+        __syncthreads();
+        if (lane == 63) wsum[threadIdx.x >> 6] = inc;
+        __syncthreads();
+        uint32_t before = carry;
+        for (uint32_t w = 0; w < (threadIdx.x >> 6); w++) before += wsum[w];
+        if (i < n_blocks) block_sum[i] = before + inc - v;
+        carry += wsum[0] + wsum[1] + wsum[2] + wsum[3];
+    }
+    if (threadIdx.x == 0) *total = carry;
+}
+struct ChainSum { uint64_t runs, pieces, flags, pad; };
+__device__ __forceinline__ void chain_block_scan(uint64_t a, uint64_t b, uint64_t* s_w, uint64_t& ex_a, uint64_t& ex_b, uint64_t& tot_a, uint64_t& tot_b) {
+    const uint32_t lane = threadIdx.x & 63, w = threadIdx.x >> 6;
+    uint64_t ia = a, ib = b;
+    for (int o = 1; o < 64; o <<= 1) {
+        const uint64_t ua = __shfl_up((unsigned long long)ia, o), ub = __shfl_up((unsigned long long)ib, o);
+        if ((int)lane >= o) { ia += ua; ib += ub; }
+    }
+    __syncthreads();
+    if (lane == 63) { s_w[w] = ia; s_w[4 + w] = ib; }
+    __syncthreads();
+    uint64_t fa = 0, fb = 0;
+    tot_a = 0; tot_b = 0;
+    for (uint32_t k = 0; k < 4; k++) {
+        if (k < w) { fa += s_w[k]; fb += s_w[4 + k]; }
+        tot_a += s_w[k]; tot_b += s_w[4 + k];
+    }
+    ex_a = fa + ia - a; ex_b = fb + ib - b;
+}
+template <int ENC>
+__global__ __launch_bounds__(256) void chain_join_kernel(const ReplayParams P, const DevRun* v, uint32_t n, const uint32_t* d_nrec, uint64_t min_chars,
+                                                         uint32_t cut, uint64_t piece_cap, ChainEnt* ent, ChainSum* bsum, uint32_t n_blocks,
+                                                         ChainResult* result, uint32_t* ticket, uint32_t ticket_base) {
+    __shared__ uint64_t s_w[8];
+    __shared__ uint32_t last_s;
+    const uint32_t nrec = *d_nrec;
+    const uint32_t n_eff = nrec < n ? nrec : n;
+    const uint32_t i = blockIdx.x * 256u + threadIdx.x;
+    bool long_walk = false;
+    ChainEnt e;
+    e.start = 0; e.end = 0; e.chars = 0; e.pieces = 0;
+    if (i < n_eff) e = chain_entry<ENC>(P, v, n_eff, i, min_chars, cut != 0u, &long_walk);
+    if (i < n) ent[i] = e;
+    uint64_t ex_r, ex_p, tot_r, tot_p;
+    chain_block_scan(e.pieces ? 1u : 0u, e.pieces, s_w, ex_r, ex_p, tot_r, tot_p);
+    const int any_long = __syncthreads_or(long_walk ? 1 : 0);
+    if (threadIdx.x == 0) {
+        ChainSum* const s = bsum + blockIdx.x;
+        __hip_atomic_store(&s->runs, tot_r, __ATOMIC_RELAXED, __HIP_MEMORY_SCOPE_AGENT);
+        __hip_atomic_store(&s->pieces, tot_p, __ATOMIC_RELAXED, __HIP_MEMORY_SCOPE_AGENT);
+        __hip_atomic_store(&s->flags, (uint64_t)(any_long ? kChainLongWalk : 0u), __ATOMIC_RELAXED, __HIP_MEMORY_SCOPE_AGENT);
+    }
+    if (!chain_drew_last_ticket(ticket, ticket_base, &last_s)) return;
+    uint64_t carry_r = 0, carry_p = 0;
+    int flags = 0;
+    for (uint32_t base = 0; base < n_blocks; base += 256) {
+        const uint32_t k = base + threadIdx.x;
+        uint64_t r = 0, p = 0, f = 0;
+        if (k < n_blocks) {
+            r = __hip_atomic_load(&bsum[k].runs, __ATOMIC_RELAXED, __HIP_MEMORY_SCOPE_AGENT);
+            p = __hip_atomic_load(&bsum[k].pieces, __ATOMIC_RELAXED, __HIP_MEMORY_SCOPE_AGENT);
+            f = __hip_atomic_load(&bsum[k].flags, __ATOMIC_RELAXED, __HIP_MEMORY_SCOPE_AGENT);
+        }
+        chain_block_scan(r, p, s_w, ex_r, ex_p, tot_r, tot_p);
+        if (k < n_blocks) { bsum[k].runs = carry_r + ex_r; bsum[k].pieces = carry_p + ex_p; }
+        carry_r += tot_r; carry_p += tot_p;
+        flags |= (int)f;
+    }
+    flags = __syncthreads_or(flags & (int)kChainLongWalk) ? (int)kChainLongWalk : 0;
+    if (threadIdx.x == 0) {
+        ChainResult o;
+        o.nrec = nrec; o.nruns = (uint32_t)carry_r; o.pieces = carry_p;
+        o.flags = (uint32_t)flags | (nrec != n ? kChainCountMismatch : 0u) | (cut && carry_p > piece_cap ? kChainPieceOverflow : 0u);
+        o.pad[0] = 0; o.pad[1] = 0; o.pad[2] = 0;
+        *result = o;
+    }
+}
+__global__ __launch_bounds__(256) void chain_place_kernel(const ChainEnt* ent, uint32_t n, const ChainSum* bsum, uint32_t W, sx_run* runs,
+                                                          sx_run* pieces, uint64_t piece_cap) {
+    __shared__ uint64_t s_w[8];
+    const uint32_t i = blockIdx.x * 256u + threadIdx.x;
+    ChainEnt e;
+    e.start = 0; e.end = 0; e.chars = 0; e.pieces = 0;
+    if (i < n) e = ent[i];
+    uint64_t ex_r, ex_p, tot_r, tot_p;
+    chain_block_scan(e.pieces ? 1u : 0u, e.pieces, s_w, ex_r, ex_p, tot_r, tot_p);
+    chain_place(e, W, bsum[blockIdx.x].runs + ex_r, bsum[blockIdx.x].pieces + ex_p, runs, pieces, piece_cap);
+}
+
+bool chain_takes_encoding(uint32_t encoding) { return enc_family(encoding) <= 3; }
+static size_t chain_up(size_t x) { return (x + 255) / 256 * 256; }
+size_t chain_scratch_bytes(uint64_t n_regions, uint32_t nrec) {
+    const size_t nb1 = (size_t)((n_regions + kScanPerBlock - 1) / kScanPerBlock), nb3 = ((size_t)nrec + 255) / 256;
+    return 256 + chain_up(n_regions * 4) + chain_up(nb1 * 4) + chain_up((size_t)nrec * sizeof(ChainEnt)) + chain_up(nb3 * sizeof(ChainSum)) + 512;
+}
+const ChainResult* chain_result_of(const void* scratch) { return (const ChainResult*)(((uintptr_t)scratch + 255) & ~(uintptr_t)255); }
+hipError_t launch_chain(const DevRun* recs, const uint32_t* counts, uint64_t n_regions, uint32_t region_cap, DevRun* packed, uint32_t nrec,
+                        const ReplayParams& P, uint64_t min_chars, bool cut, sx_run* runs, sx_run* pieces, uint64_t piece_cap,
+                        void* scratch, size_t scratch_bytes, ChainTickets* tickets, hipStream_t stream) {
+    if (n_regions == 0 || nrec == 0 || !tickets || !tickets->d || scratch_bytes < chain_scratch_bytes(n_regions, nrec)) return hipErrorInvalidValue;
+    if (!chain_takes_encoding(P.encoding) || (cut && !pieces)) return hipErrorInvalidValue;
+    const uint32_t nb1 = (uint32_t)((n_regions + kScanPerBlock - 1) / kScanPerBlock), nb3 = (nrec + 255u) / 256u;
+    uint8_t* at = (uint8_t*)chain_result_of(scratch);
+    ChainResult* result = (ChainResult*)at;
+    uint32_t* d_nrec = (uint32_t*)(at + 64);
+    at += 256;
+    uint32_t* local_off = (uint32_t*)at; at += chain_up(n_regions * 4);
+    uint32_t* block_sum = (uint32_t*)at; at += chain_up((size_t)nb1 * 4);
+    ChainEnt* ent = (ChainEnt*)at; at += chain_up((size_t)nrec * sizeof(ChainEnt));
+    ChainSum* bsum = (ChainSum*)at;
+    hipLaunchKernelGGL(chain_region_scan_kernel, dim3(nb1), dim3(256), 0, stream, counts, n_regions, local_off, block_sum, nb1, d_nrec,
+                       tickets->d, tickets->base[0]);
+    hipError_t e = hipGetLastError();
+    if (e != hipSuccess) return e;
+    tickets->base[0] += nb1;
+    const uint64_t threads = n_regions * kPackLanes;
+    hipLaunchKernelGGL(region_pack_kernel, dim3((unsigned)((threads + 255) / 256)), dim3(256), 0, stream, recs, counts, local_off, block_sum,
+                       n_regions, region_cap, packed);
+    const uint64_t minc = min_chars ? min_chars : 1;
+    const uint32_t c = cut ? 1u : 0u;
+    const uint64_t cap = cut ? piece_cap : 0;
+    switch (enc_family(P.encoding)) {
+        case 1: hipLaunchKernelGGL(chain_join_kernel<1>, dim3(nb3), dim3(256), 0, stream, P, packed, nrec, d_nrec, minc, c, cap, ent, bsum, nb3, result, tickets->d + 1, tickets->base[1]); break;
+        case 2: hipLaunchKernelGGL(chain_join_kernel<2>, dim3(nb3), dim3(256), 0, stream, P, packed, nrec, d_nrec, minc, c, cap, ent, bsum, nb3, result, tickets->d + 1, tickets->base[1]); break;
+        case 3: hipLaunchKernelGGL(chain_join_kernel<3>, dim3(nb3), dim3(256), 0, stream, P, packed, nrec, d_nrec, minc, c, cap, ent, bsum, nb3, result, tickets->d + 1, tickets->base[1]); break;
+        default: hipLaunchKernelGGL(chain_join_kernel<0>, dim3(nb3), dim3(256), 0, stream, P, packed, nrec, d_nrec, minc, c, cap, ent, bsum, nb3, result, tickets->d + 1, tickets->base[1]); break;
+    }
+    e = hipGetLastError();
+    if (e != hipSuccess) return e;
+    tickets->base[1] += nb3;
+    hipLaunchKernelGGL(chain_place_kernel, dim3(nb3), dim3(256), 0, stream, ent, nrec, bsum, P.W, runs, cut ? pieces : nullptr, cap);
+    return hipGetLastError();
+}
+
+struct CounterSrc { const uint32_t* p[3]; };
+__global__ __launch_bounds__(64) void gather_counters_kernel(uint32_t* dst, CounterSrc s, int n) {
+    constexpr uint32_t n4 = kCounterWords / 4;
+    static_assert(kCounterWords % 4 == 0, "counter blocks are copied 16 bytes at a time");
+    for (int b = 0; b < n; b++)
+        for (uint32_t i = threadIdx.x; i < n4; i += 64) ((uint4*)dst)[b * n4 + i] = ((const uint4*)s.p[b])[i];
+}
+hipError_t launch_gather_counters(uint32_t* pinned_dst, const uint32_t* const* src, int n, hipStream_t stream) {
+    if (n < 1 || n > 3) return hipErrorInvalidValue;
+    CounterSrc s{ { nullptr, nullptr, nullptr } };
+    for (int b = 0; b < n; b++) { if (((uintptr_t)src[b] & 15) != 0) return hipErrorInvalidValue; s.p[b] = src[b]; }
+    if (((uintptr_t)pinned_dst & 15) != 0) return hipErrorInvalidValue;
+    hipLaunchKernelGGL(gather_counters_kernel, dim3(1), dim3(64), 0, stream, pinned_dst, s, n);
     return hipGetLastError();
 }
 
diff --git a/stringsext_amd/csrc/sx_stage_a.cpp b/stringsext_amd/csrc/sx_stage_a.cpp
--- a/stringsext_amd/csrc/sx_stage_a.cpp
+++ b/stringsext_amd/csrc/sx_stage_a.cpp
@@ -120,10 +120,13 @@
             for (int sl = 0; sl < kFusedMax; sl++) if ((used >> sl) & 1u) HIP_TRY(ctx, hipEventRecord(ctx->dev[(size_t)which[member[sl]]].slot[si].ev0, st));
             HIP_TRY(ctx, launch_scan_fused(fp, used, st, ctx->sw.fused_prefilter));
             bool first = true;
+            std::vector<int> group;
+            for (int sl = 0; sl < kFusedMax; sl++) if ((used >> sl) & 1u) group.push_back(which[member[sl]]);
             for (int sl = 0; sl < kFusedMax; sl++) if ((used >> sl) & 1u) {
                 ScanSlot& s = ctx->dev[(size_t)which[member[sl]]].slot[si];
                 HIP_TRY(ctx, hipEventRecord(s.ev1, st));
                 s.fused = true; s.fused_first = first; first = false;
+                s.fused_group = group; s.counters_read.clear();
                 fused[member[sl]] = 1;
             }
             ctx->stats.fused_launches++;
@@ -134,6 +137,7 @@
         MissionDev& d = ctx->dev[(size_t)which[k]];
         ScanSlot& s = d.slot[si];
         s.fused = false; s.fused_first = false;
+        s.fused_group.clear(); s.counters_read.clear();
         const bool dbcs = ctx->missions[(size_t)which[k]].is_dbcs();
         const ScanParams& p = params[k];
         const uint64_t n_sub = (len + p.subchunk - 1) / p.subchunk;
@@ -152,12 +156,34 @@
     return SX_OK;
 }
 
+static int read_group_counters(sx_ctx* ctx, MissionDev& d, ScanSlot& s, int si, std::vector<uint32_t>* hc) {
+    if (!ctx->h_counters) HIP_TRY(ctx, hipHostMalloc((void**)&ctx->h_counters, (size_t)kFusedMax * kCounterWords * sizeof(uint32_t), hipHostMallocDefault));
+    const uint32_t* src[kFusedMax];
+    ScanSlot* slots[kFusedMax];
+    int n = 0;
+    for (int m : s.fused_group) {
+        ScanSlot& o = ctx->dev[(size_t)m].slot[si];
+        if (n < kFusedMax && (&o == &s || (o.fused && o.fused_group == s.fused_group))) { src[n] = o.d_counters; slots[n] = &o; n++; }
+    }
+    HIP_TRY(ctx, launch_gather_counters(ctx->h_counters, src, n, d.stream_b));
+    HIP_TRY(ctx, hipStreamSynchronize(d.stream_b));
+    bool mine = false;
+    for (int b = 0; b < n; b++) {
+        const uint32_t* from = ctx->h_counters + (size_t)b * kCounterWords;
+        if (slots[b] == &s) { hc->assign(from, from + kCounterWords); mine = true; }
+        else slots[b]->counters_read.assign(from, from + kCounterWords);
+    }
+    if (!mine) { ctx->err = "fused launch: a Mission is not in its own group"; return SX_E_STATE; }
+    return SX_OK;
+}
+
 int stage_a_finish(sx_ctx* ctx, const std::vector<int>& which, const uint8_t* d_bytes, uint64_t len,
                    const std::vector<uint32_t>& parity, const std::vector<uint64_t>& min_chars, int si,
                    std::vector<RunList>* out, bool cut_into_pieces, const ReplayJob* wave_job) {
     out->assign(which.size(), RunList{});
     if (len == 0) return SX_OK;
     const double t0 = now_ms();
+    const bool chain = ctx->sw.stage_a_chain;
     for (size_t k = 0; k < which.size(); k++) {
         MissionDev& d = ctx->dev[(size_t)which[k]];
         ScanSlot& s = d.slot[si];
@@ -173,7 +199,15 @@
         std::vector<uint32_t> hc(kCounterWords);
         bool skip_runs = false;
         for (int round = 0;; round++) {
-            { const int rb = read_back_sync(ctx, d, d.stream_b, hc.data(), s.d_counters, kCounterWords * sizeof(uint32_t)); if (rb != SX_OK) return rb; }
+            if (round == 0 && chain && s.counters_read.size() == kCounterWords) {
+                hc.swap(s.counters_read);
+                s.counters_read.clear();
+            } else if (round == 0 && chain && s.fused && s.fused_group.size() > 1 && ctx->sw.small_copy) {
+                const int rb = read_group_counters(ctx, d, s, si, &hc); if (rb != SX_OK) return rb;
+            } else {
+                s.counters_read.clear();
+                const int rb = read_back_sync(ctx, d, d.stream_b, hc.data(), s.d_counters, kCounterWords * sizeof(uint32_t)); if (rb != SX_OK) return rb;
+            }
             counters[0] = hc[0]; counters[3] = hc[3];
             {
                 uint64_t heavy = 0, recs = 0;
@@ -237,6 +271,8 @@
         const DevRun* d_records = s.d_recs;
         const bool large_regions = s.region_cap > ctx->region_cap && ctx->region_cap;
         const bool regions = s.region_cap != 0 && !large_regions;
+        bool chain_full = false;
+        const char* how = nullptr;
         if (large_regions) {
             HIP_TRY(ctx, invalidate_region_slack(s.d_recs, s.d_cnt, s.n_regions, s.region_cap, d.stream_b));
             nrec = (uint32_t)(s.n_regions * s.region_cap);
@@ -249,10 +285,20 @@
                 HIP_TRY(ctx, hipMalloc((void**)&s.d_packed, (slots + slots / 8 + 64) * sizeof(DevRun)));
                 s.packed_cap = slots + slots / 8 + 64;
             }
-            int rc = ensure_scratch(ctx, compact_scratch_bytes(s.n_regions)); if (rc != SX_OK) return rc;
-            HIP_TRY(ctx, compact_regions(s.d_recs, s.d_cnt, s.n_regions, s.region_cap, s.d_packed, s.d_counters + 1, ctx->d_scratch,
-                                         ctx->d_scratch_cap, d.stream_b));
-            { const int rb = read_back_sync(ctx, d, d.stream_b, &nrec, s.d_counters + 1, 4); if (rb != SX_OK) return rb; }
+            if (chain) {
+                nrec = counters[2];
+                chain_full = nrec >= ctx->sw.device_join_min && chain_takes_encoding((uint32_t)ctx->missions[(size_t)which[k]].c.encoding) && !ctx->sw.timing2;
+                if (nrec && !chain_full) {
+                    int rc = ensure_scratch(ctx, compact_scratch_bytes(s.n_regions)); if (rc != SX_OK) return rc;
+                    HIP_TRY(ctx, compact_regions(s.d_recs, s.d_cnt, s.n_regions, s.region_cap, s.d_packed, s.d_counters + 1, ctx->d_scratch,
+                                                 ctx->d_scratch_cap, d.stream_b));
+                }
+            } else {
+                int rc = ensure_scratch(ctx, compact_scratch_bytes(s.n_regions)); if (rc != SX_OK) return rc;
+                HIP_TRY(ctx, compact_regions(s.d_recs, s.d_cnt, s.n_regions, s.region_cap, s.d_packed, s.d_counters + 1, ctx->d_scratch,
+                                             ctx->d_scratch_cap, d.stream_b));
+                { const int rb = read_back_sync(ctx, d, d.stream_b, &nrec, s.d_counters + 1, 4); if (rb != SX_OK) return rb; }
+            }
             d_records = s.d_packed;
             SX_TL("mission %d: regions packed (%u)", which[k], nrec);
         } else if (ctx->region_cap && !large_regions && nrec < s.n_regions * ctx->region_cap / 4)
@@ -262,9 +308,55 @@
         double tc1 = tc0;
         RunList& rl = (*out)[k];
         if (dev_sorted) {
+            const Mission& mm = ctx->missions[(size_t)which[k]];
+            const bool cut = cut_into_pieces && !ctx->sw.no_pieces && mm.c.grep_char < 0 && !mm.c.require_same_unicode_block
+                && mm.c.chars_min_nb >= 1 && mm.c.chars_min_nb <= mm.q && mm.q <= 255;
+            ReplayParams SP{};
+            SP.data = d_bytes; SP.len = len; SP.encoding = mm.c.encoding; SP.table = d.d_table;
+            SP.chars_min_nb = mm.c.chars_min_nb; SP.same_block = 0; SP.q = (uint32_t)mm.q; SP.W = (uint32_t)mm.window; SP.grep_char = -1;
+            int rc = SX_OK;
+            bool have_runs = false, have_pieces = false;
+            uint64_t chain_nruns = 0, chain_npieces = 0;
+            if (d.ev_runs) HIP_TRY(ctx, hipEventSynchronize(d.ev_runs));
+            if (chain_full) {
+                uint64_t piece_cap = std::max<uint64_t>(d.chain_pieces + d.chain_pieces / 4, nrec);
+                if (ctx->sw.chain_piece_cap) piece_cap = std::min<uint64_t>(piece_cap, ctx->sw.chain_piece_cap);
+                rc = ensure_scratch(ctx, chain_scratch_bytes(s.n_regions, nrec)); if (rc != SX_OK) return rc;
+                rc = ensure_rp(ctx, d, 0, (uint64_t)nrec * sizeof(sx_run)); if (rc != SX_OK) return rc;
+                if (cut) { rc = ensure_rp(ctx, d, 9, piece_cap * sizeof(sx_run)); if (rc != SX_OK) return rc; }
+                if (!ctx->chain_tickets.d) {
+                    HIP_TRY(ctx, hipMalloc((void**)&ctx->chain_tickets.d, 256));
+                    HIP_TRY(ctx, hipMemsetAsync(ctx->chain_tickets.d, 0, 256, d.stream_b));
+                    HIP_TRY(ctx, hipStreamSynchronize(d.stream_b));
+                    ctx->chain_tickets.base[0] = ctx->chain_tickets.base[1] = 0;
+                }
+                HIP_TRY(ctx, launch_chain(s.d_recs, s.d_cnt, s.n_regions, s.region_cap, s.d_packed, nrec, SP, min_chars[k], cut, (sx_run*)d.d_rp[0],
+                                          cut ? (sx_run*)d.d_rp[9] : nullptr, piece_cap, ctx->d_scratch, ctx->d_scratch_cap, &ctx->chain_tickets, d.stream_b));
+                HIP_TRY(ctx, hipEventRecord(s.ev_free, d.stream_b));
+                s.free_pending = true;
+                ChainResult res{};
+                { const int rb = read_back_sync(ctx, d, d.stream_b, &res, chain_result_of(ctx->d_scratch), sizeof res); if (rb != SX_OK) return rb; }
+                SX_TL("mission %d: chain done (%u records, %u runs, %llu pieces, flags %u)", which[k], res.nrec, res.nruns, (unsigned long long)res.pieces, res.flags);
+                if (res.flags & (kChainCountMismatch | kChainLongWalk)) {
+                    rc = ensure_scratch(ctx, compact_scratch_bytes(s.n_regions)); if (rc != SX_OK) return rc;
+                    HIP_TRY(ctx, compact_regions(s.d_recs, s.d_cnt, s.n_regions, s.region_cap, s.d_packed, s.d_counters + 1, ctx->d_scratch,
+                                                 ctx->d_scratch_cap, d.stream_b));
+                    { const int rb = read_back_sync(ctx, d, d.stream_b, &nrec, s.d_counters + 1, 4); if (rb != SX_OK) return rb; }
+                    how = (res.flags & kChainLongWalk) ? "device pack+join (after a chain that gave up: a run of very many records)"
+                                                       : "device pack+join (after a chain that gave up: the records are not the statistic's number)";
+                } else {
+                    have_runs = true; chain_nruns = res.nruns; how = "device chain";
+                    if (cut) {
+                        d.chain_pieces = res.pieces;
+                        if (!(res.flags & kChainPieceOverflow)) { have_pieces = true; chain_npieces = res.pieces; }
+                        else how = "device chain, pieces step by step";
+                    }
+                }
+            }
+            uint64_t nruns = chain_nruns;
+            if (!have_runs) {
             const size_t sb = std::max(sort_scratch_bytes(nrec), merge_scratch_bytes(nrec));
-            int rc = ensure_scratch(ctx, sb); if (rc != SX_OK) return rc;
-            if (d.ev_runs) HIP_TRY(ctx, hipEventSynchronize(d.ev_runs));
+            rc = ensure_scratch(ctx, sb); if (rc != SX_OK) return rc;
             rc = ensure_rp(ctx, d, 0, (uint64_t)nrec * sizeof(sx_run)); if (rc != SX_OK) return rc;
             if (!regions) HIP_TRY(ctx, sort_records(s.d_recs, nrec, len, ctx->d_scratch, ctx->d_scratch_cap, d.stream_b, ctx->sw.timing2));
             if (ctx->sw.timing2) { HIP_TRY(ctx, hipStreamSynchronize(d.stream_b)); fprintf(stderr, "[sx]   sort done +%.2f ms\n", now_ms() - tc0); }
@@ -275,20 +367,20 @@
             if (ctx->sw.timing2) { HIP_TRY(ctx, hipStreamSynchronize(d.stream_b)); fprintf(stderr, "[sx]   join done +%.2f ms\n", now_ms() - tc0); }
             uint32_t nruns32 = 0;
             { const int rb = read_back_sync(ctx, d, d.stream_b, &nruns32, s.d_counters + 2, 4); if (rb != SX_OK) return rb; }
-            uint64_t nruns = nruns32;
+            nruns = nruns32;
             SX_TL("mission %d: joined (%u runs)", which[k], nruns32);
+            }
             const sx_run* d_list = (const sx_run*)d.d_rp[0];
-            const Mission& mm = ctx->missions[(size_t)which[k]];
-            if (cut_into_pieces && nruns && !ctx->sw.no_pieces && mm.c.grep_char < 0 && !mm.c.require_same_unicode_block
-                && mm.c.chars_min_nb >= 1 && mm.c.chars_min_nb <= mm.q && mm.q <= 255) {
-                ReplayParams SP{};
-                SP.data = d_bytes; SP.len = len; SP.runs = d_list; SP.n_runs = nruns; SP.encoding = mm.c.encoding; SP.table = d.d_table;
-                SP.chars_min_nb = mm.c.chars_min_nb; SP.same_block = 0; SP.q = (uint32_t)mm.q; SP.W = (uint32_t)mm.window; SP.grep_char = -1;
+            if (cut && nruns && have_pieces) {
+                if (chain_npieces > nruns) { d_list = (const sx_run*)d.d_rp[9]; nruns = chain_npieces; }
+            } else if (cut && nruns) {
+                SP.runs = d_list; SP.n_runs = nruns;
                 rc = ensure_scratch(ctx, split_scratch_bytes(nruns) + 64); if (rc != SX_OK) return rc;
                 uint64_t* d_total = (uint64_t*)ctx->d_scratch;
                 HIP_TRY(ctx, launch_split_count(SP, ctx->d_scratch + 64, ctx->d_scratch_cap - 64, d_total, d.stream_b));
                 uint64_t total = 0;
                 { const int rb = read_back_sync(ctx, d, d.stream_b, &total, d_total, 8); if (rb != SX_OK) return rb; }
+                d.chain_pieces = total;
                 if (total > nruns && total < (1ull << 32) && ensure_rp(ctx, d, 9, total * sizeof(sx_run)) == SX_OK) {
                     HIP_TRY(ctx, launch_split_write(SP, ctx->d_scratch + 64, total, (sx_run*)d.d_rp[9], d.stream_b));
                     HIP_TRY(ctx, hipStreamSynchronize(d.stream_b));
@@ -328,7 +420,7 @@
         }
         if (ctx->sw.timing)
             fprintf(stderr, "[sx] mission %d: kernel %.2f ms, %u %s, %s %.2f ms, %s %.2f ms -> %zu runs\n", which[k], ms, nrec,
-                    regions ? "records (regions)" : (large_regions ? "record slots (large regions)" : "record slots (pool)"), dev_sorted ? (regions ? "device pack+join" : "device sort+join") : "d2h",
+                    regions ? "records (regions)" : (large_regions ? "record slots (large regions)" : "record slots (pool)"), dev_sorted ? (how ? how : regions ? "device pack+join" : "device sort+join") : "d2h",
                     tc1 - tc0, dev_sorted ? "d2h runs" : "host join", now_ms() - tc1, rl.size());
         ctx->stats.run_records += rl.size();
         ctx->stats.bytes_scanned += len;
diff --git a/stringsext_amd/csrc/sx_switches.cpp b/stringsext_amd/csrc/sx_switches.cpp
--- a/stringsext_amd/csrc/sx_switches.cpp
+++ b/stringsext_amd/csrc/sx_switches.cpp
@@ -33,6 +33,8 @@
     s.no_large_regions = present("SX_NO_LARGE_REGIONS");
     s.device_join_min = (uint32_t)int_or("SX_DEVICE_JOIN_MIN", (int)s.device_join_min);
     s.no_pieces = present("SX_NO_PIECES");
+    s.stage_a_chain = on_unless_0("SX_STAGE_A_CHAIN");
+    s.chain_piece_cap = u64_at_least("SX_CHAIN_PIECE_CAP", 1, s.chain_piece_cap);
     s.probe_rot = (uint32_t)int_or("SX_PROBE_ROT", (int)s.probe_rot);
     s.host_replay = present("SX_HOST_REPLAY");
     s.device_replay = present("SX_DEVICE_REPLAY");
diff --git a/stringsext_amd/csrc/sx_switches.hpp b/stringsext_amd/csrc/sx_switches.hpp
--- a/stringsext_amd/csrc/sx_switches.hpp
+++ b/stringsext_amd/csrc/sx_switches.hpp
@@ -20,6 +20,8 @@
     bool no_large_regions = false;
     uint32_t device_join_min = 65536;
     bool no_pieces = false;
+    bool stage_a_chain = true;
+    uint64_t chain_piece_cap = 0;
     uint32_t probe_rot = 0;
     bool host_replay = false;
     bool device_replay = false;
```

Result: no change. 4134, median of 6 (+0.8%).
